# linkedin/spark-tfrecord

Hardware: AMD Instinct MI355X
Metric: rows/sec read+write (1M-row Example round-trip) (higher is better)
Workload: dtype wire(int64/float32/bytes); 1 GPU; model=Example{id:int64, ints:Int64List[8], floats:FloatList[16], tokens:BytesList[2]}, global_batch=1000000, parallelism=dp1, rows_per_rank=1000000, engine=gpu, storage=/dev/shm, crc_verify=True

## Files before the change

csrc/codec_core.h:

```cpp
#pragma once

#include <cstdint>
#include <cstring>

#include "crc32c.h"

namespace tfrec {

using i64 = int64_t;
using u64 = uint64_t;
using u32 = uint32_t;
using u8 = uint8_t;

enum Kind : int32_t { KIND_BYTES = 1, KIND_FLOAT = 2, KIND_INT64 = 3 };

enum RecordFormat : int32_t { FMT_EXAMPLE = 0, FMT_SEQUENCE = 1, FMT_BYTE_ARRAY = 2 };

enum CodecErr : int32_t {
  ERR_OK = 0,
  ERR_TRUNCATED = -1,
  ERR_BAD_VARINT = -2,
  ERR_KIND_MISMATCH = -3,
  ERR_BAD_WIRETYPE = -4,
  ERR_OVERFLOW = -5,
  ERR_NAME_TOO_LONG = -6,
};


TFR_HOSTDEV inline int popcount64(u64 x) { return __builtin_popcountll(x); }

TFR_HOSTDEV inline int ctz64(u64 x) { return __builtin_ctzll(x); }

constexpr u64 kMsbMask = 0x8080808080808080ull;

TFR_HOSTDEV inline const u8* read_varint(const u8* p, const u8* end, u64* out) {
  if (end - p >= 8) {
    u64 w;
    __builtin_memcpy(&w, p, 8);
    u64 stops = ~w & kMsbMask;
    if (stops) {
      int nb = (ctz64(stops) >> 3) + 1;
      u64 v = 0;
      for (int i = 0; i < nb; ++i)
        v |= ((w >> (8 * i)) & 0x7F) << (7 * i);
      *out = v;
      return p + nb;
    }
    u64 v = 0;
    for (int i = 0; i < 8; ++i) v |= ((w >> (8 * i)) & 0x7F) << (7 * i);
    const u8* q = p + 8;
    for (int shift = 56; q < end && shift < 64; shift += 7) {
      u8 b = *q++;
      v |= static_cast<u64>(b & 0x7F) << shift;
      if (!(b & 0x80)) {
        *out = v;
        return q;
      }
    }
    return nullptr;
  }
  u64 v = 0;
  int shift = 0;
  while (p < end) {
    u8 b = *p++;
    v |= static_cast<u64>(b & 0x7F) << shift;
    if (!(b & 0x80)) {
      *out = v;
      return p;
    }
    shift += 7;
    if (shift >= 64) return nullptr;
  }
  return nullptr;
}

TFR_HOSTDEV inline int varint_size(u64 v) {
  int n = 1;
  while (v >= 0x80) {
    v >>= 7;
    ++n;
  }
  return n;
}

TFR_HOSTDEV inline u8* write_varint(u8* p, u64 v) {
  while (v >= 0x80) {
    *p++ = static_cast<u8>(v) | 0x80;
    v >>= 7;
  }
  *p++ = static_cast<u8>(v);
  return p;
}


struct FieldDescRaw {
  int32_t kind;
  int32_t is_seq;
  int32_t name_off;
  int32_t name_len;
};

struct SchemaView {
  int32_t nfields;
  const FieldDescRaw* fields;
  const u8* names;

  TFR_HOSTDEV const u8* name(int f) const { return names + fields[f].name_off; }
  TFR_HOSTDEV int name_len(int f) const { return fields[f].name_len; }
};

TFR_HOSTDEV inline SchemaView schema_view(const u8* blob) {
  SchemaView v;
  int32_t n;
  __builtin_memcpy(&n, blob, 4);
  v.nfields = n;
  v.fields = reinterpret_cast<const FieldDescRaw*>(blob + 4);
  v.names = blob + 4 + n * static_cast<int>(sizeof(FieldDescRaw));
  return v;
}

TFR_HOSTDEV inline bool name_eq(const u8* a, const u8* b, int n) {
  while (n >= 8) {
    u64 x, y;
    __builtin_memcpy(&x, a, 8);
    __builtin_memcpy(&y, b, 8);
    if (x != y) return false;
    a += 8;
    b += 8;
    n -= 8;
  }
  for (int i = 0; i < n; ++i)
    if (a[i] != b[i]) return false;
  return true;
}

TFR_HOSTDEV inline int schema_find(const SchemaView& s, const u8* name, int len,
                                   int want_seq) {
  for (int f = 0; f < s.nfields; ++f) {
    if (s.fields[f].is_seq == want_seq && s.fields[f].name_len == len &&
        name_eq(s.name(f), name, len))
      return f;
  }
  return -1;
}


struct FieldStat {
  i64 pos;
  i64 len;
  i64 nvals;
  i64 nbytes;
  i64 nlists;
  int32_t kind_found;
  int32_t err;
};

TFR_HOSTDEV inline void field_stat_clear(FieldStat* st) {
  st->pos = -1;
  st->len = 0;
  st->nvals = 0;
  st->nbytes = 0;
  st->nlists = 0;
  st->kind_found = 0;
  st->err = 0;
}

TFR_HOSTDEV inline const u8* skip_field(const u8* p, const u8* end, u32 wiretype) {
  u64 tmp;
  switch (wiretype) {
    case 0:
      return read_varint(p, end, &tmp);
    case 1:
      return (end - p >= 8) ? p + 8 : nullptr;
    case 2:
      p = read_varint(p, end, &tmp);
      if (!p || static_cast<u64>(end - p) < tmp) return nullptr;
      return p + tmp;
    case 5:
      return (end - p >= 4) ? p + 4 : nullptr;
    default:
      return nullptr;
  }
}

TFR_HOSTDEV inline int32_t count_list_body(const u8* p, const u8* end, int32_t kind,
                                           i64* nvals, i64* nbytes) {
  while (p < end) {
    u64 tag;
    p = read_varint(p, end, &tag);
    if (!p) return ERR_BAD_VARINT;
    u32 fieldno = static_cast<u32>(tag >> 3);
    u32 wt = static_cast<u32>(tag & 7);
    if (fieldno != 1) {
      p = skip_field(p, end, wt);
      if (!p) return ERR_TRUNCATED;
      continue;
    }
    if (kind == KIND_BYTES) {
      if (wt != 2) return ERR_BAD_WIRETYPE;
      u64 len;
      p = read_varint(p, end, &len);
      if (!p || static_cast<u64>(end - p) < len) return ERR_TRUNCATED;
      *nvals += 1;
      *nbytes += static_cast<i64>(len);
      p += len;
    } else if (kind == KIND_FLOAT) {
      if (wt == 2) {
        u64 len;
        p = read_varint(p, end, &len);
        if (!p || static_cast<u64>(end - p) < len) return ERR_TRUNCATED;
        *nvals += static_cast<i64>(len / 4);
        p += len;
      } else if (wt == 5) {
        if (end - p < 4) return ERR_TRUNCATED;
        *nvals += 1;
        p += 4;
      } else {
        return ERR_BAD_WIRETYPE;
      }
    } else {
      if (wt == 2) {
        u64 len;
        p = read_varint(p, end, &len);
        if (!p || static_cast<u64>(end - p) < len) return ERR_TRUNCATED;
        const u8* q = p;
        const u8* qe = p + len;
        if (len && (qe[-1] & 0x80)) return ERR_BAD_VARINT;
        i64 cnt = 0;
        while (qe - q >= 8) {
          u64 w;
          __builtin_memcpy(&w, q, 8);
          cnt += popcount64(~w & kMsbMask);
          q += 8;
        }
        for (; q < qe; ++q) cnt += !(*q & 0x80);
        *nvals += cnt;
        p = qe;
      } else if (wt == 0) {
        u64 v;
        p = read_varint(p, end, &v);
        if (!p) return ERR_BAD_VARINT;
        *nvals += 1;
      } else {
        return ERR_BAD_WIRETYPE;
      }
    }
  }
  return ERR_OK;
}

TFR_HOSTDEV inline int32_t scan_feature_body(const u8* p, const u8* end,
                                             int32_t expect_kind, int32_t* kind_found,
                                             i64* nvals, i64* nbytes) {
  while (p < end) {
    u64 tag;
    p = read_varint(p, end, &tag);
    if (!p) return ERR_BAD_VARINT;
    u32 fieldno = static_cast<u32>(tag >> 3);
    u32 wt = static_cast<u32>(tag & 7);
    if (fieldno >= 1 && fieldno <= 3 && wt == 2) {
      u64 len;
      p = read_varint(p, end, &len);
      if (!p || static_cast<u64>(end - p) < len) return ERR_TRUNCATED;
      *kind_found = static_cast<int32_t>(fieldno);
      if (expect_kind >= 0 && static_cast<int32_t>(fieldno) != expect_kind)
        return ERR_KIND_MISMATCH;
      int32_t rc = count_list_body(p, p + len, static_cast<int32_t>(fieldno), nvals,
                                   nbytes);
      if (rc != ERR_OK) return rc;
      p += len;
    } else {
      p = skip_field(p, end, wt);
      if (!p) return ERR_TRUNCATED;
    }
  }
  return ERR_OK;
}

TFR_HOSTDEV inline int32_t scan_features_body(const u8* p, const u8* end, i64 base,
                                              const SchemaView& schema, int want_seq,
                                              FieldStat* stats) {
  const u8* body_start = p;
  while (p < end) {
    u64 tag;
    p = read_varint(p, end, &tag);
    if (!p) return ERR_BAD_VARINT;
    u32 fieldno = static_cast<u32>(tag >> 3);
    u32 wt = static_cast<u32>(tag & 7);
    if (fieldno != 1 || wt != 2) {
      p = skip_field(p, end, wt);
      if (!p) return ERR_TRUNCATED;
      continue;
    }
    u64 entry_len;
    p = read_varint(p, end, &entry_len);
    if (!p || static_cast<u64>(end - p) < entry_len) return ERR_TRUNCATED;
    const u8* ep = p;
    const u8* ee = p + entry_len;
    p = ee;
    const u8* key = nullptr;
    u64 key_len = 0;
    const u8* val = nullptr;
    u64 val_len = 0;
    while (ep < ee) {
      u64 etag;
      ep = read_varint(ep, ee, &etag);
      if (!ep) return ERR_BAD_VARINT;
      u32 efn = static_cast<u32>(etag >> 3);
      u32 ewt = static_cast<u32>(etag & 7);
      if (efn == 1 && ewt == 2) {
        ep = read_varint(ep, ee, &key_len);
        if (!ep || static_cast<u64>(ee - ep) < key_len) return ERR_TRUNCATED;
        key = ep;
        ep += key_len;
      } else if (efn == 2 && ewt == 2) {
        ep = read_varint(ep, ee, &val_len);
        if (!ep || static_cast<u64>(ee - ep) < val_len) return ERR_TRUNCATED;
        val = ep;
        ep += val_len;
      } else {
        ep = skip_field(ep, ee, ewt);
        if (!ep) return ERR_TRUNCATED;
      }
    }
    if (!key) continue;
    int f = schema_find(schema, key, static_cast<int>(key_len), want_seq);
    if (f < 0) continue;
    FieldStat* st = &stats[f];
    st->nvals = 0;
    st->nbytes = 0;
    st->nlists = 0;
    st->kind_found = 0;
    st->err = 0;
    st->pos = base + (val ? (val - body_start) : 0);
    st->len = static_cast<i64>(val_len);
    if (!want_seq) {
      int32_t rc = scan_feature_body(val, val + val_len, schema.fields[f].kind,
                                     &st->kind_found, &st->nvals, &st->nbytes);
      if (rc != ERR_OK) st->err = rc;
    } else {
      const u8* lp = val;
      const u8* le = val + val_len;
      while (lp < le) {
        u64 ltag;
        lp = read_varint(lp, le, &ltag);
        if (!lp) {
          st->err = ERR_BAD_VARINT;
          break;
        }
        u32 lfn = static_cast<u32>(ltag >> 3);
        u32 lwt = static_cast<u32>(ltag & 7);
        if (lfn == 1 && lwt == 2) {
          u64 flen;
          lp = read_varint(lp, le, &flen);
          if (!lp || static_cast<u64>(le - lp) < flen) {
            st->err = ERR_TRUNCATED;
            break;
          }
          st->nlists += 1;
          int32_t kf = 0;
          int32_t rc = scan_feature_body(lp, lp + flen, schema.fields[f].kind, &kf,
                                         &st->nvals, &st->nbytes);
          if (rc != ERR_OK) {
            st->err = rc;
            break;
          }
          if (kf) st->kind_found = kf;
          lp += flen;
        } else {
          lp = skip_field(lp, le, lwt);
          if (!lp) {
            st->err = ERR_TRUNCATED;
            break;
          }
        }
      }
    }
  }
  return ERR_OK;
}

TFR_HOSTDEV inline int32_t scan_record(const u8* data, i64 abs_off, i64 rec_len,
                                       int32_t fmt, const SchemaView& schema,
                                       FieldStat* stats) {
  const u8* p = data + abs_off;
  const u8* end = p + rec_len;
  while (p < end) {
    u64 tag;
    p = read_varint(p, end, &tag);
    if (!p) return ERR_BAD_VARINT;
    u32 fieldno = static_cast<u32>(tag >> 3);
    u32 wt = static_cast<u32>(tag & 7);
    bool is_features =
        (fmt == FMT_EXAMPLE && fieldno == 1) || (fmt == FMT_SEQUENCE && fieldno == 1);
    bool is_feature_lists = (fmt == FMT_SEQUENCE && fieldno == 2);
    if ((is_features || is_feature_lists) && wt == 2) {
      u64 len;
      p = read_varint(p, end, &len);
      if (!p || static_cast<u64>(end - p) < len) return ERR_TRUNCATED;
      i64 base = (p - data);
      if (is_features) {
        int32_t rc = scan_features_body(p, p + len, base, schema, 0, stats);
        if (rc != ERR_OK) return rc;
      } else {
        int32_t rc = scan_features_body(p, p + len, base, schema, 1, stats);
        if (rc != ERR_OK) return rc;
      }
      p += len;
    } else {
      p = skip_field(p, end, wt);
      if (!p) return ERR_TRUNCATED;
    }
  }
  return ERR_OK;
}


constexpr int32_t ERR_RETRY_UNFUSED = -100;

TFR_HOSTDEV inline u32 crc32c_step8(u32 crc, u64 w, const uint32_t (*tab)[256]) {
  w ^= crc;
  return tab[7][w & 0xFF] ^ tab[6][(w >> 8) & 0xFF] ^ tab[5][(w >> 16) & 0xFF] ^
         tab[4][(w >> 24) & 0xFF] ^ tab[3][(w >> 32) & 0xFF] ^
         tab[2][(w >> 40) & 0xFF] ^ tab[1][(w >> 48) & 0xFF] ^
         tab[0][(w >> 56) & 0xFF];
}

struct ScanCur {
  const u8* base;
  i64 len;
  i64 pos;
  i64 wpos;
  u64 w0, w1;
  u32 crc;
  const uint32_t (*tab)[256];
};

TFR_HOSTDEV inline u64 cur_load(const ScanCur& c, i64 at) {
  if (at + 8 <= c.len) {
    u64 w;
    __builtin_memcpy(&w, c.base + at, 8);
    return w;
  }
  u64 w = 0;
  for (i64 b = at; b < c.len; ++b) w |= (u64)c.base[b] << (8 * (b - at));
  return w;
}

TFR_HOSTDEV inline void cur_init(ScanCur& c, const u8* base, i64 len,
                                 const uint32_t (*tab)[256]) {
  c.base = base;
  c.len = len;
  c.pos = 0;
  c.wpos = 0;
  c.tab = tab;
  c.crc = 0xFFFFFFFFu;
  c.w0 = cur_load(c, 0);
  c.w1 = cur_load(c, 8);
}

TFR_HOSTDEV inline u64 cur_peek(const ScanCur& c) {
  int sh = (int)(c.pos - c.wpos) * 8;
  if (sh == 0) return c.w0;
  if (sh == 64) return c.w1;
  return (c.w0 >> sh) | (c.w1 << (64 - sh));
}

TFR_HOSTDEV inline void cur_advance(ScanCur& c, i64 k) {
  c.pos += k;
  while (c.pos > c.wpos + 8) {
    if (c.wpos + 8 <= c.len) c.crc = crc32c_step8(c.crc, c.w0, c.tab);
    c.w0 = c.w1;
    c.wpos += 8;
    c.w1 = cur_load(c, c.wpos + 8);
  }
}

TFR_HOSTDEV inline u32 cur_finish_crc(ScanCur& c) {
  while (c.wpos + 8 <= c.len) {
    c.crc = crc32c_step8(c.crc, c.w0, c.tab);
    c.w0 = c.w1;
    c.wpos += 8;
    c.w1 = cur_load(c, c.wpos + 8);
  }
  u32 crc = c.crc;
  for (i64 b = c.wpos; b < c.len; ++b)
    crc = c.tab[0][(crc ^ c.base[b]) & 0xFF] ^ (crc >> 8);
  return ~crc;
}

TFR_HOSTDEV inline bool cur_varint(ScanCur& c, i64 end, u64* out) {
  i64 avail = end - c.pos;
  if (avail <= 0) return false;
  u64 w = cur_peek(c);
  u64 stops = ~w & kMsbMask;
  if (stops) {
    int nb = (ctz64(stops) >> 3) + 1;
    if (nb > avail) return false;
    u64 v = 0;
    for (int i = 0; i < nb; ++i) v |= ((w >> (8 * i)) & 0x7F) << (7 * i);
    *out = v;
    cur_advance(c, nb);
    return true;
  }
  if (avail < 9) return false;
  u64 v = 0;
  for (int i = 0; i < 8; ++i) v |= ((w >> (8 * i)) & 0x7F) << (7 * i);
  cur_advance(c, 8);
  for (int shift = 56; shift < 64 && c.pos < end; shift += 7) {
    u8 b = (u8)cur_peek(c);
    v |= (u64)(b & 0x7F) << shift;
    cur_advance(c, 1);
    if (!(b & 0x80)) {
      *out = v;
      return true;
    }
  }
  return false;
}

TFR_HOSTDEV inline int32_t cur_skip_field(ScanCur& c, i64 end, u32 wt) {
  u64 tmp;
  switch (wt) {
    case 0:
      return cur_varint(c, end, &tmp) ? ERR_OK : ERR_BAD_VARINT;
    case 1:
      if (end - c.pos < 8) return ERR_TRUNCATED;
      cur_advance(c, 8);
      return ERR_OK;
    case 2:
      if (!cur_varint(c, end, &tmp)) return ERR_BAD_VARINT;
      if ((u64)(end - c.pos) < tmp) return ERR_TRUNCATED;
      cur_advance(c, (i64)tmp);
      return ERR_OK;
    case 5:
      if (end - c.pos < 4) return ERR_TRUNCATED;
      cur_advance(c, 4);
      return ERR_OK;
    default:
      return ERR_BAD_WIRETYPE;
  }
}

TFR_HOSTDEV inline i64 cur_count_terms(ScanCur& c, i64 n) {
  i64 cnt = 0;
  while (n >= 8) {
    cnt += popcount64(~cur_peek(c) & kMsbMask);
    cur_advance(c, 8);
    n -= 8;
  }
  if (n > 0) {
    u64 mask = kMsbMask >> (8 * (8 - n));
    cnt += popcount64(~cur_peek(c) & mask);
    cur_advance(c, n);
  }
  return cnt;
}

TFR_HOSTDEV inline int32_t cur_count_list_body(ScanCur& c, i64 end, int32_t kind,
                                               i64* nvals, i64* nbytes) {
  while (c.pos < end) {
    u64 tag;
    if (!cur_varint(c, end, &tag)) return ERR_BAD_VARINT;
    u32 fieldno = (u32)(tag >> 3), wt = (u32)(tag & 7);
    if (fieldno != 1) {
      int32_t rc = cur_skip_field(c, end, wt);
      if (rc != ERR_OK) return rc;
      continue;
    }
    if (kind == KIND_BYTES) {
      if (wt != 2) return ERR_BAD_WIRETYPE;
      u64 blen;
      if (!cur_varint(c, end, &blen)) return ERR_BAD_VARINT;
      if ((u64)(end - c.pos) < blen) return ERR_TRUNCATED;
      *nvals += 1;
      *nbytes += (i64)blen;
      cur_advance(c, (i64)blen);
    } else if (kind == KIND_FLOAT) {
      if (wt == 2) {
        u64 blen;
        if (!cur_varint(c, end, &blen)) return ERR_BAD_VARINT;
        if ((u64)(end - c.pos) < blen) return ERR_TRUNCATED;
        *nvals += (i64)(blen / 4);
        cur_advance(c, (i64)blen);
      } else if (wt == 5) {
        if (end - c.pos < 4) return ERR_TRUNCATED;
        *nvals += 1;
        cur_advance(c, 4);
      } else {
        return ERR_BAD_WIRETYPE;
      }
    } else {
      if (wt == 2) {
        u64 blen;
        if (!cur_varint(c, end, &blen)) return ERR_BAD_VARINT;
        if ((u64)(end - c.pos) < blen) return ERR_TRUNCATED;
        if (blen && (c.base[c.pos + (i64)blen - 1] & 0x80))
          return ERR_BAD_VARINT;
        *nvals += cur_count_terms(c, (i64)blen);
      } else if (wt == 0) {
        u64 v;
        if (!cur_varint(c, end, &v)) return ERR_BAD_VARINT;
        *nvals += 1;
      } else {
        return ERR_BAD_WIRETYPE;
      }
    }
  }
  return ERR_OK;
}

TFR_HOSTDEV inline int32_t cur_scan_feature_body(ScanCur& c, i64 end,
                                                 int32_t expect_kind,
                                                 int32_t* kind_found, i64* nvals,
                                                 i64* nbytes) {
  while (c.pos < end) {
    u64 tag;
    if (!cur_varint(c, end, &tag)) return ERR_BAD_VARINT;
    u32 fieldno = (u32)(tag >> 3), wt = (u32)(tag & 7);
    if (fieldno >= 1 && fieldno <= 3 && wt == 2) {
      u64 blen;
      if (!cur_varint(c, end, &blen)) return ERR_BAD_VARINT;
      if ((u64)(end - c.pos) < blen) return ERR_TRUNCATED;
      *kind_found = (int32_t)fieldno;
      if (expect_kind >= 0 && (int32_t)fieldno != expect_kind)
        return ERR_KIND_MISMATCH;
      int32_t rc = cur_count_list_body(c, c.pos + (i64)blen, (int32_t)fieldno,
                                       nvals, nbytes);
      if (rc != ERR_OK) return rc;
    } else {
      int32_t rc = cur_skip_field(c, end, wt);
      if (rc != ERR_OK) return rc;
    }
  }
  return ERR_OK;
}

TFR_HOSTDEV inline int32_t cur_scan_features_body(ScanCur& c, i64 end, i64 data_rel,
                                                  const SchemaView& schema,
                                                  int want_seq, FieldStat* stats) {
  i64 body_start = c.pos;
  while (c.pos < end) {
    u64 tag;
    if (!cur_varint(c, end, &tag)) return ERR_BAD_VARINT;
    u32 fieldno = (u32)(tag >> 3), wt = (u32)(tag & 7);
    if (fieldno != 1 || wt != 2) {
      int32_t rc = cur_skip_field(c, end, wt);
      if (rc != ERR_OK) return rc;
      continue;
    }
    u64 entry_len;
    if (!cur_varint(c, end, &entry_len)) return ERR_BAD_VARINT;
    if ((u64)(end - c.pos) < entry_len) return ERR_TRUNCATED;
    i64 ee = c.pos + (i64)entry_len;
    int f = -1;
    bool key_seen = false;
    bool val_seen = false;
    while (c.pos < ee) {
      u64 etag;
      if (!cur_varint(c, ee, &etag)) return ERR_BAD_VARINT;
      u32 efn = (u32)(etag >> 3), ewt = (u32)(etag & 7);
      if (efn == 1 && ewt == 2) {
        if (val_seen) return ERR_RETRY_UNFUSED;
        u64 klen;
        if (!cur_varint(c, ee, &klen)) return ERR_BAD_VARINT;
        if ((u64)(ee - c.pos) < klen) return ERR_TRUNCATED;
        f = schema_find(schema, c.base + c.pos, (int)klen, want_seq);
        key_seen = true;
        cur_advance(c, (i64)klen);
      } else if (efn == 2 && ewt == 2) {
        if (!key_seen) return ERR_RETRY_UNFUSED;
        val_seen = true;
        u64 vlen;
        if (!cur_varint(c, ee, &vlen)) return ERR_BAD_VARINT;
        if ((u64)(ee - c.pos) < vlen) return ERR_TRUNCATED;
        i64 ve = c.pos + (i64)vlen;
        if (f < 0) {
          cur_advance(c, (i64)vlen);
          continue;
        }
        FieldStat* st = &stats[f];
        st->nvals = 0;
        st->nbytes = 0;
        st->nlists = 0;
        st->kind_found = 0;
        st->err = 0;
        st->pos = data_rel + c.pos;
        st->len = (i64)vlen;
        if (!want_seq) {
          int32_t rc = cur_scan_feature_body(c, ve, schema.fields[f].kind,
                                             &st->kind_found, &st->nvals,
                                             &st->nbytes);
          if (rc == ERR_RETRY_UNFUSED) return rc;
          if (rc != ERR_OK) st->err = rc;
        } else {
          while (c.pos < ve && st->err == ERR_OK) {
            u64 ltag;
            if (!cur_varint(c, ve, &ltag)) {
              st->err = ERR_BAD_VARINT;
              break;
            }
            u32 lfn = (u32)(ltag >> 3), lwt = (u32)(ltag & 7);
            if (lfn == 1 && lwt == 2) {
              u64 flen;
              if (!cur_varint(c, ve, &flen) || (u64)(ve - c.pos) < flen) {
                st->err = ERR_TRUNCATED;
                break;
              }
              st->nlists += 1;
              int32_t kf = 0;
              int32_t rc = cur_scan_feature_body(c, c.pos + (i64)flen,
                                                 schema.fields[f].kind, &kf,
                                                 &st->nvals, &st->nbytes);
              if (rc == ERR_RETRY_UNFUSED) return rc;
              if (rc != ERR_OK) {
                st->err = rc;
                break;
              }
              if (kf) st->kind_found = kf;
            } else {
              int32_t rc = cur_skip_field(c, ve, lwt);
              if (rc != ERR_OK) {
                st->err = ERR_TRUNCATED;
                break;
              }
            }
          }
        }
        if (c.pos < ve) cur_advance(c, ve - c.pos);
      } else {
        int32_t rc = cur_skip_field(c, ee, ewt);
        if (rc != ERR_OK) return rc;
      }
    }
    if (f >= 0 && !val_seen) {
      FieldStat* st = &stats[f];
      st->pos = data_rel + body_start;
      st->len = 0;
      st->nvals = 0;
      st->nbytes = 0;
      st->nlists = 0;
      st->kind_found = 0;
      st->err = 0;
    }
  }
  return ERR_OK;
}

TFR_HOSTDEV inline int32_t scan_record_fused(const u8* data, i64 abs_off,
                                             i64 rec_len, int32_t fmt,
                                             const SchemaView& schema,
                                             FieldStat* stats, u32* crc_out,
                                             const uint32_t (*tab)[256]) {
  ScanCur c;
  cur_init(c, data + abs_off, rec_len, tab);
  while (c.pos < rec_len) {
    u64 tag;
    if (!cur_varint(c, rec_len, &tag)) return ERR_BAD_VARINT;
    u32 fieldno = (u32)(tag >> 3), wt = (u32)(tag & 7);
    bool is_features = fieldno == 1;
    bool is_fl = (fmt == FMT_SEQUENCE && fieldno == 2);
    if ((is_features || is_fl) && wt == 2) {
      u64 blen;
      if (!cur_varint(c, rec_len, &blen)) return ERR_BAD_VARINT;
      if ((u64)(rec_len - c.pos) < blen) return ERR_TRUNCATED;
      int32_t rc = cur_scan_features_body(c, c.pos + (i64)blen, abs_off, schema,
                                          is_fl ? 1 : 0, stats);
      if (rc != ERR_OK) return rc;
    } else {
      int32_t rc = cur_skip_field(c, rec_len, wt);
      if (rc != ERR_OK) return rc;
    }
  }
  *crc_out = cur_finish_crc(c);
  return ERR_OK;
}


struct DecodeDst {
  i64* i64_vals;
  float* f32_vals;
  u8* bytes_data;
  i64* elem_len;
  i64* sub_count;
};

TFR_HOSTDEV inline int32_t extract_list_body(const u8* p, const u8* end, int32_t kind,
                                             const DecodeDst& dst, i64* vi, i64* bi) {
  while (p < end) {
    u64 tag;
    p = read_varint(p, end, &tag);
    if (!p) return ERR_BAD_VARINT;
    u32 fieldno = static_cast<u32>(tag >> 3);
    u32 wt = static_cast<u32>(tag & 7);
    if (fieldno != 1) {
      p = skip_field(p, end, wt);
      if (!p) return ERR_TRUNCATED;
      continue;
    }
    if (kind == KIND_BYTES) {
      u64 len;
      p = read_varint(p, end, &len);
      if (!p || static_cast<u64>(end - p) < len) return ERR_TRUNCATED;
      u8* d = dst.bytes_data + *bi;
      u64 i = 0;
      for (; i + 8 <= len; i += 8) {
        u64 w;
        __builtin_memcpy(&w, p + i, 8);
        __builtin_memcpy(d + i, &w, 8);
      }
      for (; i < len; ++i) d[i] = p[i];
      dst.elem_len[*vi] = static_cast<i64>(len);
      *bi += static_cast<i64>(len);
      *vi += 1;
      p += len;
    } else if (kind == KIND_FLOAT) {
      if (wt == 2) {
        u64 len;
        p = read_varint(p, end, &len);
        if (!p || static_cast<u64>(end - p) < len) return ERR_TRUNCATED;
        u64 n = len / 4;
        __builtin_memcpy(dst.f32_vals + *vi, p, n * 4);
        *vi += static_cast<i64>(n);
        p += len;
      } else {
        if (end - p < 4) return ERR_TRUNCATED;
        float v;
        __builtin_memcpy(&v, p, 4);
        dst.f32_vals[(*vi)++] = v;
        p += 4;
      }
    } else {
      if (wt == 2) {
        u64 len;
        p = read_varint(p, end, &len);
        if (!p || static_cast<u64>(end - p) < len) return ERR_TRUNCATED;
        const u8* q = p;
        const u8* qe = p + len;
        while (q < qe) {
          u64 v;
          q = read_varint(q, qe, &v);
          if (!q) return ERR_BAD_VARINT;
          dst.i64_vals[(*vi)++] = static_cast<i64>(v);
        }
        p = qe;
      } else {
        u64 v;
        p = read_varint(p, end, &v);
        if (!p) return ERR_BAD_VARINT;
        dst.i64_vals[(*vi)++] = static_cast<i64>(v);
      }
    }
  }
  return ERR_OK;
}

TFR_HOSTDEV inline int32_t extract_feature_body(const u8* p, const u8* end,
                                                int32_t kind, const DecodeDst& dst,
                                                i64* vi, i64* bi) {
  while (p < end) {
    u64 tag;
    p = read_varint(p, end, &tag);
    if (!p) return ERR_BAD_VARINT;
    u32 fieldno = static_cast<u32>(tag >> 3);
    u32 wt = static_cast<u32>(tag & 7);
    if (fieldno >= 1 && fieldno <= 3 && wt == 2) {
      u64 len;
      p = read_varint(p, end, &len);
      if (!p || static_cast<u64>(end - p) < len) return ERR_TRUNCATED;
      int32_t rc = extract_list_body(p, p + len, kind, dst, vi, bi);
      if (rc != ERR_OK) return rc;
      p += len;
    } else {
      p = skip_field(p, end, wt);
      if (!p) return ERR_TRUNCATED;
    }
  }
  return ERR_OK;
}

TFR_HOSTDEV inline int32_t extract_field(const u8* data, i64 pos, i64 len,
                                         int32_t kind, int32_t is_seq,
                                         const DecodeDst& dst, i64 val_base,
                                         i64 byte_base, i64 list_base) {
  if (pos < 0) return ERR_OK;
  const u8* p = data + pos;
  const u8* end = p + len;
  i64 vi = val_base;
  i64 bi = byte_base;
  if (!is_seq) return extract_feature_body(p, end, kind, dst, &vi, &bi);
  i64 li = list_base;
  while (p < end) {
    u64 tag;
    p = read_varint(p, end, &tag);
    if (!p) return ERR_BAD_VARINT;
    u32 fieldno = static_cast<u32>(tag >> 3);
    u32 wt = static_cast<u32>(tag & 7);
    if (fieldno == 1 && wt == 2) {
      u64 flen;
      p = read_varint(p, end, &flen);
      if (!p || static_cast<u64>(end - p) < flen) return ERR_TRUNCATED;
      i64 v_before = vi;
      int32_t rc = extract_feature_body(p, p + flen, kind, dst, &vi, &bi);
      if (rc != ERR_OK) return rc;
      dst.sub_count[li++] = vi - v_before;
      p += flen;
    } else {
      p = skip_field(p, end, wt);
      if (!p) return ERR_TRUNCATED;
    }
  }
  return ERR_OK;
}


struct FieldColumn {
  int32_t kind;
  int32_t is_seq;
  const u8* presence;
  const i64* row_off;
  const i64* list_off;
  const i64* sub_off;
  const i64* elem_off;
  const u8* bytes_data;
  const i64* i64_vals;
  const float* f32_vals;
};

TFR_HOSTDEV inline i64 list_body_size(const FieldColumn& c, i64 v0, i64 v1) {
  if (c.kind == KIND_FLOAT) {
    i64 n = v1 - v0;
    return n ? (1 + varint_size(static_cast<u64>(4 * n)) + 4 * n) : 0;
  }
  if (c.kind == KIND_INT64) {
    i64 packed = 0;
    for (i64 v = v0; v < v1; ++v)
      packed += varint_size(static_cast<u64>(c.i64_vals[v]));
    return packed ? (1 + varint_size(static_cast<u64>(packed)) + packed) : 0;
  }
  i64 sz = 0;
  for (i64 v = v0; v < v1; ++v) {
    i64 blen = c.elem_off[v + 1] - c.elem_off[v];
    sz += 1 + varint_size(static_cast<u64>(blen)) + blen;
  }
  return sz;
}

TFR_HOSTDEV inline i64 feature_body_size(const FieldColumn& c, i64 v0, i64 v1) {
  i64 body = list_body_size(c, v0, v1);
  return 1 + varint_size(static_cast<u64>(body)) + body;
}

TFR_HOSTDEV inline u8* emit_list_body(u8* o, const FieldColumn& c, i64 v0, i64 v1) {
  if (c.kind == KIND_FLOAT) {
    i64 n = v1 - v0;
    if (n) {
      *o++ = 0x0A;
      o = write_varint(o, static_cast<u64>(4 * n));
      __builtin_memcpy(o, c.f32_vals + v0, static_cast<size_t>(4 * n));
      o += 4 * n;
    }
  } else if (c.kind == KIND_INT64) {
    i64 packed = 0;
    for (i64 v = v0; v < v1; ++v)
      packed += varint_size(static_cast<u64>(c.i64_vals[v]));
    if (packed) {
      *o++ = 0x0A;
      o = write_varint(o, static_cast<u64>(packed));
      for (i64 v = v0; v < v1; ++v)
        o = write_varint(o, static_cast<u64>(c.i64_vals[v]));
    }
  } else {
    for (i64 v = v0; v < v1; ++v) {
      i64 b0 = c.elem_off[v];
      i64 blen = c.elem_off[v + 1] - b0;
      *o++ = 0x0A;
      o = write_varint(o, static_cast<u64>(blen));
      for (i64 i = 0; i < blen; ++i) o[i] = c.bytes_data[b0 + i];
      o += blen;
    }
  }
  return o;
}

TFR_HOSTDEV inline u8* emit_feature_body(u8* o, const FieldColumn& c, i64 v0, i64 v1) {
  i64 body = list_body_size(c, v0, v1);
  *o++ = static_cast<u8>((c.kind << 3) | 2);
  o = write_varint(o, static_cast<u64>(body));
  return emit_list_body(o, c, v0, v1);
}

TFR_HOSTDEV inline i64 features_entry_size(const FieldColumn& c, const SchemaView& s,
                                           int f, i64 v0, i64 v1) {
  i64 fb = feature_body_size(c, v0, v1);
  i64 klen = s.name_len(f);
  return (1 + varint_size(static_cast<u64>(klen)) + klen) +
         (1 + varint_size(static_cast<u64>(fb)) + fb);
}

TFR_HOSTDEV inline u8* emit_features_entry(u8* o, const FieldColumn& c,
                                           const SchemaView& s, int f, i64 v0, i64 v1) {
  i64 fb = feature_body_size(c, v0, v1);
  i64 klen = s.name_len(f);
  *o++ = 0x0A;
  o = write_varint(o, static_cast<u64>(klen));
  const u8* nm = s.name(f);
  for (i64 i = 0; i < klen; ++i) o[i] = nm[i];
  o += klen;
  *o++ = 0x12;
  o = write_varint(o, static_cast<u64>(fb));
  return emit_feature_body(o, c, v0, v1);
}

TFR_HOSTDEV inline i64 feature_list_body_size(const FieldColumn& c, i64 r) {
  i64 sz = 0;
  for (i64 j = c.list_off[r]; j < c.list_off[r + 1]; ++j) {
    i64 fb = feature_body_size(c, c.sub_off[j], c.sub_off[j + 1]);
    sz += 1 + varint_size(static_cast<u64>(fb)) + fb;
  }
  return sz;
}

TFR_HOSTDEV inline u8* emit_feature_list_body(u8* o, const FieldColumn& c, i64 r) {
  for (i64 j = c.list_off[r]; j < c.list_off[r + 1]; ++j) {
    i64 fb = feature_body_size(c, c.sub_off[j], c.sub_off[j + 1]);
    *o++ = 0x0A;
    o = write_varint(o, static_cast<u64>(fb));
    o = emit_feature_body(o, c, c.sub_off[j], c.sub_off[j + 1]);
  }
  return o;
}

TFR_HOSTDEV inline i64 feature_lists_entry_size(const FieldColumn& c,
                                                const SchemaView& s, int f, i64 r) {
  i64 flb = feature_list_body_size(c, r);
  i64 klen = s.name_len(f);
  return (1 + varint_size(static_cast<u64>(klen)) + klen) +
         (1 + varint_size(static_cast<u64>(flb)) + flb);
}

TFR_HOSTDEV inline u8* emit_feature_lists_entry(u8* o, const FieldColumn& c,
                                                const SchemaView& s, int f, i64 r) {
  i64 flb = feature_list_body_size(c, r);
  i64 klen = s.name_len(f);
  *o++ = 0x0A;
  o = write_varint(o, static_cast<u64>(klen));
  const u8* nm = s.name(f);
  for (i64 i = 0; i < klen; ++i) o[i] = nm[i];
  o += klen;
  *o++ = 0x12;
  o = write_varint(o, static_cast<u64>(flb));
  return emit_feature_list_body(o, c, r);
}

TFR_HOSTDEV inline i64 record_payload_size(const FieldColumn* cols,
                                           const SchemaView& s, int32_t fmt, i64 r) {
  i64 ctx_body = 0;
  i64 fl_body = 0;
  for (int f = 0; f < s.nfields; ++f) {
    const FieldColumn& c = cols[f];
    if (!c.presence[r]) continue;
    if (!c.is_seq) {
      i64 e = features_entry_size(c, s, f, c.row_off[r], c.row_off[r + 1]);
      ctx_body += 1 + varint_size(static_cast<u64>(e)) + e;
    } else {
      i64 e = feature_lists_entry_size(c, s, f, r);
      fl_body += 1 + varint_size(static_cast<u64>(e)) + e;
    }
  }
  i64 total = 0;
  if (fmt == FMT_EXAMPLE) {
    total += 1 + varint_size(static_cast<u64>(ctx_body)) + ctx_body;
  } else {
    if (ctx_body) total += 1 + varint_size(static_cast<u64>(ctx_body)) + ctx_body;
    total += 1 + varint_size(static_cast<u64>(fl_body)) + fl_body;
  }
  return total;
}

TFR_HOSTDEV inline u8* emit_record_payload(u8* o, const FieldColumn* cols,
                                           const SchemaView& s, int32_t fmt, i64 r) {
  i64 ctx_body = 0, fl_body = 0;
  for (int f = 0; f < s.nfields; ++f) {
    const FieldColumn& c = cols[f];
    if (!c.presence[r]) continue;
    if (!c.is_seq) {
      i64 e = features_entry_size(c, s, f, c.row_off[r], c.row_off[r + 1]);
      ctx_body += 1 + varint_size(static_cast<u64>(e)) + e;
    } else {
      i64 e = feature_lists_entry_size(c, s, f, r);
      fl_body += 1 + varint_size(static_cast<u64>(e)) + e;
    }
  }
  auto emit_ctx = [&](u8* oo) {
    for (int f = 0; f < s.nfields; ++f) {
      const FieldColumn& c = cols[f];
      if (!c.presence[r] || c.is_seq) continue;
      i64 e = features_entry_size(c, s, f, c.row_off[r], c.row_off[r + 1]);
      *oo++ = 0x0A;
      oo = write_varint(oo, static_cast<u64>(e));
      oo = emit_features_entry(oo, c, s, f, c.row_off[r], c.row_off[r + 1]);
    }
    return oo;
  };
  auto emit_fl = [&](u8* oo) {
    for (int f = 0; f < s.nfields; ++f) {
      const FieldColumn& c = cols[f];
      if (!c.presence[r] || !c.is_seq) continue;
      i64 e = feature_lists_entry_size(c, s, f, r);
      *oo++ = 0x0A;
      oo = write_varint(oo, static_cast<u64>(e));
      oo = emit_feature_lists_entry(oo, c, s, f, r);
    }
    return oo;
  };
  if (fmt == FMT_EXAMPLE) {
    *o++ = 0x0A;
    o = write_varint(o, static_cast<u64>(ctx_body));
    o = emit_ctx(o);
  } else {
    if (ctx_body) {
      *o++ = 0x0A;
      o = write_varint(o, static_cast<u64>(ctx_body));
      o = emit_ctx(o);
    }
    *o++ = 0x12;
    o = write_varint(o, static_cast<u64>(fl_body));
    o = emit_fl(o);
  }
  return o;
}



struct WriteCur {
  u8* base;
  i64 pos;
  i64 wpos;
  u64 win;
  u32 crc;
  const uint32_t (*tab)[256];
};

TFR_HOSTDEV inline void wcur_init(WriteCur& w, u8* base,
                                  const uint32_t (*tab)[256]) {
  w.base = base;
  w.pos = 0;
  w.wpos = 0;
  w.win = 0;
  w.crc = 0xFFFFFFFFu;
  w.tab = tab;
}

TFR_HOSTDEV inline void wcur_flush8(WriteCur& w) {
  __builtin_memcpy(w.base + w.wpos, &w.win, 8);
  w.crc = crc32c_step8(w.crc, w.win, w.tab);
  w.wpos += 8;
  w.win = 0;
}

TFR_HOSTDEV inline void wcur_put(WriteCur& w, u8 b) {
  w.win |= (u64)b << (8 * (w.pos - w.wpos));
  if (++w.pos - w.wpos == 8) wcur_flush8(w);
}

TFR_HOSTDEV inline void wcur_varint(WriteCur& w, u64 v) {
  while (v >= 0x80) {
    wcur_put(w, (u8)(v | 0x80));
    v >>= 7;
  }
  wcur_put(w, (u8)v);
}

TFR_HOSTDEV inline void wcur_bytes(WriteCur& w, const u8* src, i64 n) {
  while (n > 0 && (w.pos - w.wpos) != 0) {
    wcur_put(w, *src++);
    --n;
  }
  while (n >= 8) {
    __builtin_memcpy(&w.win, src, 8);
    w.pos += 8;
    wcur_flush8(w);
    src += 8;
    n -= 8;
  }
  while (n-- > 0) wcur_put(w, *src++);
}

TFR_HOSTDEV inline u32 wcur_finish(WriteCur& w) {
  int rem = (int)(w.pos - w.wpos);
  if (!rem) return ~w.crc;
  __builtin_memcpy(w.base + w.wpos, &w.win, (size_t)rem);
  u32 crc = w.crc;
  for (int i = 0; i < rem; ++i)
    crc = w.tab[0][(crc ^ (u8)(w.win >> (8 * i))) & 0xFF] ^ (crc >> 8);
  return ~crc;
}

TFR_HOSTDEV inline void wcur_list_body(WriteCur& w, const FieldColumn& c,
                                       i64 v0, i64 v1) {
  if (c.kind == KIND_FLOAT) {
    i64 n = v1 - v0;
    if (n) {
      wcur_put(w, 0x0A);
      wcur_varint(w, (u64)(4 * n));
      wcur_bytes(w, (const u8*)(c.f32_vals + v0), 4 * n);
    }
  } else if (c.kind == KIND_INT64) {
    i64 packed = 0;
    for (i64 v = v0; v < v1; ++v)
      packed += varint_size((u64)c.i64_vals[v]);
    if (packed) {
      wcur_put(w, 0x0A);
      wcur_varint(w, (u64)packed);
      for (i64 v = v0; v < v1; ++v) wcur_varint(w, (u64)c.i64_vals[v]);
    }
  } else {
    for (i64 v = v0; v < v1; ++v) {
      i64 b0 = c.elem_off[v];
      i64 blen = c.elem_off[v + 1] - b0;
      wcur_put(w, 0x0A);
      wcur_varint(w, (u64)blen);
      wcur_bytes(w, c.bytes_data + b0, blen);
    }
  }
}

TFR_HOSTDEV inline void wcur_feature_body(WriteCur& w, const FieldColumn& c,
                                          i64 v0, i64 v1) {
  i64 body = list_body_size(c, v0, v1);
  wcur_put(w, (u8)((c.kind << 3) | 2));
  wcur_varint(w, (u64)body);
  wcur_list_body(w, c, v0, v1);
}

TFR_HOSTDEV inline void wcur_features_entry(WriteCur& w, const FieldColumn& c,
                                            const SchemaView& s, int f, i64 v0,
                                            i64 v1) {
  i64 fb = feature_body_size(c, v0, v1);
  i64 klen = s.name_len(f);
  wcur_put(w, 0x0A);
  wcur_varint(w, (u64)klen);
  wcur_bytes(w, s.name(f), klen);
  wcur_put(w, 0x12);
  wcur_varint(w, (u64)fb);
  wcur_feature_body(w, c, v0, v1);
}

TFR_HOSTDEV inline void wcur_feature_list_body(WriteCur& w,
                                               const FieldColumn& c, i64 r) {
  for (i64 j = c.list_off[r]; j < c.list_off[r + 1]; ++j) {
    i64 fb = feature_body_size(c, c.sub_off[j], c.sub_off[j + 1]);
    wcur_put(w, 0x0A);
    wcur_varint(w, (u64)fb);
    wcur_feature_body(w, c, c.sub_off[j], c.sub_off[j + 1]);
  }
}

TFR_HOSTDEV inline void wcur_feature_lists_entry(WriteCur& w,
                                                 const FieldColumn& c,
                                                 const SchemaView& s, int f,
                                                 i64 r) {
  i64 flb = feature_list_body_size(c, r);
  i64 klen = s.name_len(f);
  wcur_put(w, 0x0A);
  wcur_varint(w, (u64)klen);
  wcur_bytes(w, s.name(f), klen);
  wcur_put(w, 0x12);
  wcur_varint(w, (u64)flb);
  wcur_feature_list_body(w, c, r);
}

TFR_HOSTDEV inline i64 emit_record_payload_fused(u8* o, const FieldColumn* cols,
                                                 const SchemaView& s, int32_t fmt,
                                                 i64 r, u32* crc_out,
                                                 const uint32_t (*tab)[256]) {
  i64 ctx_body = 0, fl_body = 0;
  for (int f = 0; f < s.nfields; ++f) {
    const FieldColumn& c = cols[f];
    if (!c.presence[r]) continue;
    if (!c.is_seq) {
      i64 e = features_entry_size(c, s, f, c.row_off[r], c.row_off[r + 1]);
      ctx_body += 1 + varint_size((u64)e) + e;
    } else {
      i64 e = feature_lists_entry_size(c, s, f, r);
      fl_body += 1 + varint_size((u64)e) + e;
    }
  }
  WriteCur w;
  wcur_init(w, o, tab);
  auto emit_ctx = [&]() {
    for (int f = 0; f < s.nfields; ++f) {
      const FieldColumn& c = cols[f];
      if (!c.presence[r] || c.is_seq) continue;
      i64 e = features_entry_size(c, s, f, c.row_off[r], c.row_off[r + 1]);
      wcur_put(w, 0x0A);
      wcur_varint(w, (u64)e);
      wcur_features_entry(w, c, s, f, c.row_off[r], c.row_off[r + 1]);
    }
  };
  auto emit_fl = [&]() {
    for (int f = 0; f < s.nfields; ++f) {
      const FieldColumn& c = cols[f];
      if (!c.presence[r] || !c.is_seq) continue;
      i64 e = feature_lists_entry_size(c, s, f, r);
      wcur_put(w, 0x0A);
      wcur_varint(w, (u64)e);
      wcur_feature_lists_entry(w, c, s, f, r);
    }
  };
  if (fmt == FMT_EXAMPLE) {
    wcur_put(w, 0x0A);
    wcur_varint(w, (u64)ctx_body);
    emit_ctx();
  } else {
    if (ctx_body) {
      wcur_put(w, 0x0A);
      wcur_varint(w, (u64)ctx_body);
      emit_ctx();
    }
    wcur_put(w, 0x12);
    wcur_varint(w, (u64)fl_body);
    emit_fl();
  }
  *crc_out = wcur_finish(w);
  return w.pos;
}

constexpr i64 kFrameOverhead = 16;

TFR_HOSTDEV inline void write_frame_header_footer(u8* file, i64 frame_off,
                                                  i64 payload_len,
                                                  const u32 (*tab)[256]) {
  u8* h = file + frame_off;
  u64 len_le = static_cast<u64>(payload_len);
  __builtin_memcpy(h, &len_le, 8);
  u32 lc = mask_crc(crc32c_sw(h, 8, 0, tab));
  __builtin_memcpy(h + 8, &lc, 4);
  u32 dc = mask_crc(crc32c_sw(h + 12, static_cast<size_t>(payload_len), 0, tab));
  __builtin_memcpy(h + 12 + payload_len, &dc, 4);
}

TFR_HOSTDEV inline void write_frame_header_footer_crc(u8* file, i64 frame_off,
                                                      i64 payload_len,
                                                      u32 payload_crc,
                                                      const u32 (*tab)[256]) {
  u8* h = file + frame_off;
  u64 len_le = static_cast<u64>(payload_len);
  __builtin_memcpy(h, &len_le, 8);
  u32 lc = mask_crc(crc32c_sw(h, 8, 0, tab));
  __builtin_memcpy(h + 8, &lc, 4);
  u32 dc = mask_crc(payload_crc);
  __builtin_memcpy(h + 12 + payload_len, &dc, 4);
}

}
```

csrc/hip/kernels.hip:

```cpp

#include <hip/hip_runtime.h>
#include <pybind11/pybind11.h>
#include <pybind11/stl.h>
#include <rocprim/rocprim.hpp>

#include <fcntl.h>
#include <sys/mman.h>
#include <sys/stat.h>
#include <unistd.h>

#include <cstdint>
#include <map>
#include <mutex>
#include <stdexcept>
#include <string>
#include <vector>

#include "../codec_core.h"

namespace py = pybind11;
using namespace tfrec;

#define HIP_CHECK(expr)                                                          \
  do {                                                                           \
    hipError_t _e = (expr);                                                      \
    if (_e != hipSuccess)                                                        \
      throw std::runtime_error(std::string("HIP error: ") +                      \
                               hipGetErrorString(_e) + " at " __FILE__ ":" +     \
                               std::to_string(__LINE__));                        \
  } while (0)

namespace {

constexpr int kBlock = 256;

__device__ inline void stage_crc_tables(uint32_t (*lds)[256]) {
  const uint32_t* src = &kCrcTables.t[0][0];
  uint32_t* dst = &lds[0][0];
  for (int i = threadIdx.x; i < 8 * 256; i += blockDim.x) dst[i] = src[i];
  __syncthreads();
}

__device__ inline void set_err(int32_t* err, int32_t code, i64 r) {
  err[0] = code;
  i64 v = r + 1;
  atomicMax(&err[1], v > 0x7FFFFFFF ? (int32_t)0x7FFFFFFF : (int32_t)v);
}


__global__ void crc_verify_kernel(const u8* __restrict__ data,
                                  const i64* __restrict__ off,
                                  const i64* __restrict__ len, i64 R,
                                  unsigned long long* err_out) {
  __shared__ uint32_t tab[8][256];
  stage_crc_tables(tab);
  for (i64 r = blockIdx.x * (i64)blockDim.x + threadIdx.x; r < R;
       r += (i64)gridDim.x * blockDim.x) {
    const u8* h = data + off[r] - 12;
    u32 len_crc, data_crc;
    __builtin_memcpy(&len_crc, h + 8, 4);
    __builtin_memcpy(&data_crc, h + 12 + len[r], 4);
    bool ok = mask_crc(crc32c_sw(h, 8, 0, tab)) == len_crc &&
              mask_crc(crc32c_sw(h + 12, (size_t)len[r], 0, tab)) == data_crc;
    if (!ok) atomicMin(err_out, (unsigned long long)(r + 1));
  }
}


static_assert(sizeof(FieldStat) == 48, "FieldStat layout shared with Python");

__global__ void scan_records_kernel(const u8* __restrict__ data,
                                    const i64* __restrict__ off,
                                    const i64* __restrict__ len, i64 R, int32_t fmt,
                                    const u8* __restrict__ schema_blob, int F,
                                    FieldStat* __restrict__ stats,
                                    int32_t* __restrict__ err,
                                    unsigned long long* crc_err,
                                    i64 rec_base) {
  __shared__ uint32_t tab[8][256];
  if (crc_err) stage_crc_tables(tab);
  SchemaView schema = schema_view(schema_blob);
  for (i64 r = blockIdx.x * (i64)blockDim.x + threadIdx.x; r < R;
       r += (i64)gridDim.x * blockDim.x) {
    FieldStat* st = stats + r * F;
    for (int f = 0; f < F; ++f) field_stat_clear(&st[f]);
    int32_t rc;
    if (crc_err) {
      u32 payload_crc = 0;
      rc = scan_record_fused(data, off[r], len[r], fmt, schema, st,
                             &payload_crc, tab);
      if (rc == ERR_RETRY_UNFUSED) {
        for (int f = 0; f < F; ++f) field_stat_clear(&st[f]);
        rc = scan_record(data, off[r], len[r], fmt, schema, st);
        payload_crc = crc32c_sw(data + off[r], (size_t)len[r], 0, tab);
      }
      if (rc != ERR_OK)
        payload_crc = crc32c_sw(data + off[r], (size_t)len[r], 0, tab);
      const u8* h = data + off[r] - 12;
      u32 len_crc, data_crc;
      __builtin_memcpy(&len_crc, h + 8, 4);
      __builtin_memcpy(&data_crc, h + 12 + len[r], 4);
      bool ok = mask_crc(crc32c_sw(h, 8, 0, tab)) == len_crc &&
                mask_crc(payload_crc) == data_crc;
      if (!ok) atomicMin(crc_err, (unsigned long long)(rec_base + r + 1));
    } else {
      rc = scan_record(data, off[r], len[r], fmt, schema, st);
    }
    if (rc != ERR_OK) set_err(err, rc, rec_base + r);
    for (int f = 0; f < F; ++f)
      if (st[f].err != ERR_OK) set_err(err, st[f].err, rec_base + r);
  }
}


struct DevFieldDst {
  int32_t kind;
  int32_t is_seq;
  i64* i64_vals;
  float* f32_vals;
  u8* bytes_data;
  i64* elem_len;
  i64* sub_count;
  const i64* val_base;
  const i64* byte_base;
  const i64* list_base;
};

__global__ void extract_fields_kernel(const u8* __restrict__ data, i64 R, int F,
                                      const FieldStat* __restrict__ stats,
                                      const DevFieldDst* __restrict__ metas,
                                      int32_t* __restrict__ err, i64 r0) {
  i64 total = R * F;
  for (i64 idx = blockIdx.x * (i64)blockDim.x + threadIdx.x; idx < total;
       idx += (i64)gridDim.x * blockDim.x) {
    i64 q = idx / F;
    int f = (int)(idx - q * F);
    i64 r = r0 + q;
    const DevFieldDst& m = metas[f];
    const FieldStat& st = stats[r * F + f];
    DecodeDst dst{m.i64_vals, m.f32_vals, m.bytes_data, m.elem_len, m.sub_count};
    int32_t rc = extract_field(data, st.pos, st.len, m.kind, m.is_seq, dst,
                               m.val_base ? m.val_base[r] : 0,
                               m.byte_base ? m.byte_base[r] : 0,
                               m.list_base ? m.list_base[r] : 0);
    if (rc != ERR_OK) set_err(err, rc, r);
  }
}



__global__ void size_records_kernel(const FieldColumn* __restrict__ cols,
                                    const u8* __restrict__ schema_blob, int32_t fmt,
                                    i64 R, i64* __restrict__ psize) {
  SchemaView schema = schema_view(schema_blob);
  for (i64 r = blockIdx.x * (i64)blockDim.x + threadIdx.x; r < R;
       r += (i64)gridDim.x * blockDim.x) {
    psize[r] = record_payload_size(cols, schema, fmt, r) + kFrameOverhead;
  }
}

__global__ void emit_records_kernel(const FieldColumn* __restrict__ cols,
                                    const u8* __restrict__ schema_blob, int32_t fmt,
                                    i64 r0, i64 R, const i64* __restrict__ frame_off,
                                    u8* __restrict__ file,
                                    int32_t* __restrict__ err) {
  __shared__ uint32_t tab[8][256];
  stage_crc_tables(tab);
  SchemaView schema = schema_view(schema_blob);
  for (i64 r = r0 + blockIdx.x * (i64)blockDim.x + threadIdx.x; r < R;
       r += (i64)gridDim.x * blockDim.x) {
    i64 payload = (frame_off[r + 1] - frame_off[r]) - kFrameOverhead;
    u8* o = file + frame_off[r] + 12;
    u32 crc = 0;
    i64 emitted = emit_record_payload_fused(o, cols, schema, fmt, r, &crc,
                                            tab);
    if (emitted != payload) set_err(err, ERR_OVERFLOW, r);
    write_frame_header_footer_crc(file, frame_off[r], payload, crc, tab);
  }
}


constexpr i64 kWaveRecordBytes = 8 << 10;

__device__ inline u32 crc32c_wave(const u8* p, i64 n,
                                  const uint32_t (*tab)[256]) {
  int lane = threadIdx.x & 63;
  i64 chunk = (n + 63) / 64;
  if (chunk < 64) chunk = 64;
  i64 s = (i64)lane * chunk;
  i64 e = s + chunk < n ? s + chunk : n;
  u32 my = (s < e) ? crc32c_sw(p + s, (size_t)(e - s), 0, tab) : 0;
  u32 acc = __shfl(my, 0);
  if (chunk < n) {
    u32 op = crc32c_shift_elem((u64)chunk);
    for (int i = 1; i < 64; ++i) {
      i64 si = (i64)i * chunk;
      if (si >= n) break;
      u32 ci = __shfl(my, i);
      i64 li = (si + chunk < n ? chunk : n - si);
      acc = (li == chunk) ? (crc_gfmul(acc, op) ^ ci)
                          : crc32c_combine_fast(acc, ci, (u64)li);
    }
  }
  return acc;
}

__device__ inline void copy_wave(u8* d, const u8* s, i64 n) {
  int lane = threadIdx.x & 63;
  i64 i = (i64)lane * 8;
  for (; i + 8 <= n; i += 64 * 8) {
    u64 w;
    __builtin_memcpy(&w, s + i, 8);
    __builtin_memcpy(d + i, &w, 8);
  }
  i64 tail = n & ~((i64)7);
  for (i64 b = tail + lane; b < n; b += 64) d[b] = s[b];
}

__global__ void crc_verify_wave_kernel(const u8* __restrict__ data,
                                       const i64* __restrict__ off,
                                       const i64* __restrict__ len, i64 R,
                                       unsigned long long* err_out) {
  __shared__ uint32_t tab[8][256];
  stage_crc_tables(tab);
  i64 wave = (blockIdx.x * (i64)blockDim.x + threadIdx.x) / 64;
  i64 nwaves = ((i64)gridDim.x * blockDim.x) / 64;
  for (i64 r = wave; r < R; r += nwaves) {
    const u8* h = data + off[r] - 12;
    u32 payload = crc32c_wave(h + 12, len[r], tab);
    if ((threadIdx.x & 63) == 0) {
      u32 len_crc, data_crc;
      __builtin_memcpy(&len_crc, h + 8, 4);
      __builtin_memcpy(&data_crc, h + 12 + len[r], 4);
      bool ok = mask_crc(crc32c_sw(h, 8, 0, tab)) == len_crc &&
                mask_crc(payload) == data_crc;
      if (!ok) atomicMin(err_out, (unsigned long long)(r + 1));
    }
  }
}

__global__ void frame_bytes_wave_kernel(const u8* __restrict__ src,
                                        const i64* __restrict__ elem_off,
                                        const i64* __restrict__ frame_off, i64 R,
                                        u8* __restrict__ file) {
  __shared__ uint32_t tab[8][256];
  stage_crc_tables(tab);
  i64 wave = (blockIdx.x * (i64)blockDim.x + threadIdx.x) / 64;
  i64 nwaves = ((i64)gridDim.x * blockDim.x) / 64;
  for (i64 r = wave; r < R; r += nwaves) {
    i64 n = elem_off[r + 1] - elem_off[r];
    const u8* s = src + elem_off[r];
    u8* d = file + frame_off[r] + 12;
    copy_wave(d, s, n);
    u32 crc = crc32c_wave(s, n, tab);
    if ((threadIdx.x & 63) == 0)
      write_frame_header_footer_crc(file, frame_off[r], n, crc, tab);
  }
}

__global__ void gather_payloads_wave_kernel(const u8* __restrict__ data,
                                            const i64* __restrict__ off,
                                            const i64* __restrict__ len,
                                            const i64* __restrict__ dst_off,
                                            i64 R, u8* __restrict__ out) {
  i64 wave = (blockIdx.x * (i64)blockDim.x + threadIdx.x) / 64;
  i64 nwaves = ((i64)gridDim.x * blockDim.x) / 64;
  for (i64 r = wave; r < R; r += nwaves)
    copy_wave(out + dst_off[r], data + off[r], len[r]);
}


__device__ inline i64 wave_incl_scan(i64 v) {
  int lane = threadIdx.x & 63;
  for (int d = 1; d < 64; d <<= 1) {
    i64 y = __shfl_up(v, d);
    if (lane >= d) v += y;
  }
  return v;
}

__device__ inline i64 wave_extract_i64_packed(const u8* __restrict__ p, i64 n,
                                              i64* __restrict__ out, i64 base) {
  int lane = threadIdx.x & 63;
  i64 chunk = (n + 63) / 64;
  i64 lo = (i64)lane * chunk;
  i64 hi = lo + chunk < n ? lo + chunk : n;
  i64 cnt = 0;
  for (i64 i = lo; i < hi; ++i) cnt += !(p[i] & 0x80);
  i64 incl = wave_incl_scan(cnt);
  i64 excl = incl - cnt;
  i64 total = __shfl(incl, 63);
  i64 q = lo;
  i64 pre = 0;
  if (lo > 0 && lo < hi) {
    if (p[lo - 1] & 0x80) {
      while (q < hi && (p[q] & 0x80)) ++q;
      if (q < hi) {
        ++q;
        pre = 1;
      }
    }
  }
  i64 idx = base + excl + pre;
  while (q < hi) {
    u64 v = 0;
    int shift = 0;
    i64 j = q;
    while (j < n && shift < 70) {
      u8 b = p[j++];
      v |= (u64)(b & 0x7F) << shift;
      shift += 7;
      if (!(b & 0x80)) break;
    }
    out[idx++] = (i64)v;
    q = j;
  }
  return total;
}

__device__ inline int32_t extract_list_body_wave(const u8* __restrict__ p,
                                                 const u8* end, int32_t kind,
                                                 const DecodeDst& dst, i64* vi,
                                                 i64* bi) {
  int lane = threadIdx.x & 63;
  while (p < end) {
    u64 tag;
    p = read_varint(p, end, &tag);
    if (!p) return ERR_BAD_VARINT;
    u32 fieldno = (u32)(tag >> 3), wt = (u32)(tag & 7);
    if (fieldno != 1) {
      p = skip_field(p, end, wt);
      if (!p) return ERR_TRUNCATED;
      continue;
    }
    if (kind == KIND_BYTES) {
      u64 len;
      p = read_varint(p, end, &len);
      if (!p || (u64)(end - p) < len) return ERR_TRUNCATED;
      copy_wave(dst.bytes_data + *bi, p, (i64)len);
      if (lane == 0) dst.elem_len[*vi] = (i64)len;
      *bi += (i64)len;
      *vi += 1;
      p += len;
    } else if (kind == KIND_FLOAT) {
      if (wt == 2) {
        u64 len;
        p = read_varint(p, end, &len);
        if (!p || (u64)(end - p) < len) return ERR_TRUNCATED;
        u64 nv = len / 4;
        copy_wave((u8*)(dst.f32_vals + *vi), p, (i64)(nv * 4));
        *vi += (i64)nv;
        p += len;
      } else {
        if (end - p < 4) return ERR_TRUNCATED;
        if (lane == 0) {
          float v;
          __builtin_memcpy(&v, p, 4);
          dst.f32_vals[*vi] = v;
        }
        (*vi)++;
        p += 4;
      }
    } else {
      if (wt == 2) {
        u64 len;
        p = read_varint(p, end, &len);
        if (!p || (u64)(end - p) < len) return ERR_TRUNCATED;
        *vi += wave_extract_i64_packed(p, (i64)len, dst.i64_vals, *vi);
        p += len;
      } else {
        u64 v;
        p = read_varint(p, end, &v);
        if (!p) return ERR_BAD_VARINT;
        if (lane == 0) dst.i64_vals[*vi] = (i64)v;
        (*vi)++;
      }
    }
  }
  return ERR_OK;
}

__device__ inline int32_t extract_feature_body_wave(const u8* __restrict__ p,
                                                    const u8* end, int32_t kind,
                                                    const DecodeDst& dst,
                                                    i64* vi, i64* bi) {
  while (p < end) {
    u64 tag;
    p = read_varint(p, end, &tag);
    if (!p) return ERR_BAD_VARINT;
    u32 fieldno = (u32)(tag >> 3), wt = (u32)(tag & 7);
    if (fieldno >= 1 && fieldno <= 3 && wt == 2) {
      u64 len;
      p = read_varint(p, end, &len);
      if (!p || (u64)(end - p) < len) return ERR_TRUNCATED;
      int32_t rc = extract_list_body_wave(p, p + len, kind, dst, vi, bi);
      if (rc != ERR_OK) return rc;
      p += len;
    } else {
      p = skip_field(p, end, wt);
      if (!p) return ERR_TRUNCATED;
    }
  }
  return ERR_OK;
}

__device__ inline int32_t extract_field_wave(const u8* __restrict__ data,
                                             i64 pos, i64 len, int32_t kind,
                                             int32_t is_seq, const DecodeDst& dst,
                                             i64 val_base, i64 byte_base,
                                             i64 list_base) {
  if (pos < 0) return ERR_OK;
  int lane = threadIdx.x & 63;
  const u8* p = data + pos;
  const u8* end = p + len;
  i64 vi = val_base;
  i64 bi = byte_base;
  if (!is_seq) return extract_feature_body_wave(p, end, kind, dst, &vi, &bi);
  i64 li = list_base;
  while (p < end) {
    u64 tag;
    p = read_varint(p, end, &tag);
    if (!p) return ERR_BAD_VARINT;
    u32 fieldno = (u32)(tag >> 3), wt = (u32)(tag & 7);
    if (fieldno == 1 && wt == 2) {
      u64 flen;
      p = read_varint(p, end, &flen);
      if (!p || (u64)(end - p) < flen) return ERR_TRUNCATED;
      i64 v_before = vi;
      int32_t rc = extract_feature_body_wave(p, p + flen, kind, dst, &vi, &bi);
      if (rc != ERR_OK) return rc;
      if (lane == 0) dst.sub_count[li] = vi - v_before;
      ++li;
      p += flen;
    } else {
      p = skip_field(p, end, wt);
      if (!p) return ERR_TRUNCATED;
    }
  }
  return ERR_OK;
}

__global__ void scan_records_wave_kernel(const u8* __restrict__ data,
                                         const i64* __restrict__ off,
                                         const i64* __restrict__ len, i64 R,
                                         int32_t fmt,
                                         const u8* __restrict__ schema_blob,
                                         int F, FieldStat* __restrict__ stats,
                                         int32_t* __restrict__ err,
                                         unsigned long long* crc_err,
                                         i64 rec_base) {
  __shared__ uint32_t tab[8][256];
  stage_crc_tables(tab);
  SchemaView schema = schema_view(schema_blob);
  i64 wave = (blockIdx.x * (i64)blockDim.x + threadIdx.x) / 64;
  i64 nwaves = ((i64)gridDim.x * blockDim.x) / 64;
  int lane = threadIdx.x & 63;
  for (i64 r = wave; r < R; r += nwaves) {
    if (lane == 0) {
      FieldStat* st = stats + r * F;
      for (int f = 0; f < F; ++f) field_stat_clear(&st[f]);
      int32_t rc = scan_record(data, off[r], len[r], fmt, schema, st);
      if (rc != ERR_OK) set_err(err, rc, rec_base + r);
      for (int f = 0; f < F; ++f)
        if (st[f].err != ERR_OK) set_err(err, st[f].err, rec_base + r);
    }
    if (crc_err) {
      const u8* h = data + off[r] - 12;
      u32 payload = crc32c_wave(h + 12, len[r], tab);
      if (lane == 0) {
        u32 len_crc, data_crc;
        __builtin_memcpy(&len_crc, h + 8, 4);
        __builtin_memcpy(&data_crc, h + 12 + len[r], 4);
        bool ok = mask_crc(crc32c_sw(h, 8, 0, tab)) == len_crc &&
                  mask_crc(payload) == data_crc;
        if (!ok) atomicMin(crc_err, (unsigned long long)(rec_base + r + 1));
      }
    }
  }
}

__global__ void extract_fields_wave_kernel(const u8* __restrict__ data, i64 R,
                                           int F,
                                           const FieldStat* __restrict__ stats,
                                           const DevFieldDst* __restrict__ metas,
                                           int32_t* __restrict__ err, i64 r0) {
  i64 total = R * F;
  i64 wave = (blockIdx.x * (i64)blockDim.x + threadIdx.x) / 64;
  i64 nwaves = ((i64)gridDim.x * blockDim.x) / 64;
  for (i64 idx = wave; idx < total; idx += nwaves) {
    i64 q = idx / F;
    int f = (int)(idx - q * F);
    i64 r = r0 + q;
    const DevFieldDst& m = metas[f];
    const FieldStat& st = stats[r * F + f];
    DecodeDst dst{m.i64_vals, m.f32_vals, m.bytes_data, m.elem_len, m.sub_count};
    int32_t rc = extract_field_wave(data, st.pos, st.len, m.kind, m.is_seq, dst,
                                    m.val_base ? m.val_base[r] : 0,
                                    m.byte_base ? m.byte_base[r] : 0,
                                    m.list_base ? m.list_base[r] : 0);
    if (rc != ERR_OK && (threadIdx.x & 63) == 0) set_err(err, rc, r);
  }
}


__device__ inline i64 wave_emit_i64_packed(u8* __restrict__ o,
                                           const i64* __restrict__ vals,
                                           i64 v0, i64 v1) {
  int lane = threadIdx.x & 63;
  i64 n = v1 - v0;
  i64 chunk = (n + 63) / 64;
  i64 lo = v0 + (i64)lane * chunk;
  i64 hi = lo + chunk < v1 ? lo + chunk : v1;
  i64 sz = 0;
  for (i64 v = lo; v < hi; ++v) sz += varint_size((u64)vals[v]);
  i64 incl = wave_incl_scan(sz);
  u8* q = o + (incl - sz);
  for (i64 v = lo; v < hi; ++v) q = write_varint(q, (u64)vals[v]);
  return __shfl(incl, 63);
}

struct WaveCur {
  u8* base;
  i64 pos;
};

__device__ inline void wvc_put(WaveCur& w, u8 b) {
  if ((threadIdx.x & 63) == 0) w.base[w.pos] = b;
  w.pos += 1;
}

__device__ inline void wvc_varint(WaveCur& w, u64 v) {
  if ((threadIdx.x & 63) == 0) write_varint(w.base + w.pos, v);
  w.pos += varint_size(v);
}

__device__ inline void wvc_bytes(WaveCur& w, const u8* s, i64 n) {
  copy_wave(w.base + w.pos, s, n);
  w.pos += n;
}

__device__ inline void wvc_list_body(WaveCur& w, const FieldColumn& c, i64 v0,
                                     i64 v1) {
  if (c.kind == KIND_FLOAT) {
    i64 n = v1 - v0;
    if (n) {
      wvc_put(w, 0x0A);
      wvc_varint(w, (u64)(4 * n));
      wvc_bytes(w, (const u8*)(c.f32_vals + v0), 4 * n);
    }
  } else if (c.kind == KIND_INT64) {
    i64 packed = 0;
    for (i64 v = v0; v < v1; ++v) packed += varint_size((u64)c.i64_vals[v]);
    if (packed) {
      wvc_put(w, 0x0A);
      wvc_varint(w, (u64)packed);
      w.pos += wave_emit_i64_packed(w.base + w.pos, c.i64_vals, v0, v1);
    }
  } else {
    for (i64 v = v0; v < v1; ++v) {
      i64 b0 = c.elem_off[v];
      i64 blen = c.elem_off[v + 1] - b0;
      wvc_put(w, 0x0A);
      wvc_varint(w, (u64)blen);
      wvc_bytes(w, c.bytes_data + b0, blen);
    }
  }
}

__device__ inline void wvc_feature_body(WaveCur& w, const FieldColumn& c,
                                        i64 v0, i64 v1) {
  i64 body = list_body_size(c, v0, v1);
  wvc_put(w, (u8)((c.kind << 3) | 2));
  wvc_varint(w, (u64)body);
  wvc_list_body(w, c, v0, v1);
}

__device__ inline void wvc_features_entry(WaveCur& w, const FieldColumn& c,
                                          const SchemaView& s, int f, i64 v0,
                                          i64 v1) {
  i64 fb = feature_body_size(c, v0, v1);
  i64 klen = s.name_len(f);
  wvc_put(w, 0x0A);
  wvc_varint(w, (u64)klen);
  wvc_bytes(w, s.name(f), klen);
  wvc_put(w, 0x12);
  wvc_varint(w, (u64)fb);
  wvc_feature_body(w, c, v0, v1);
}

__device__ inline void wvc_feature_lists_entry(WaveCur& w, const FieldColumn& c,
                                               const SchemaView& s, int f,
                                               i64 r) {
  i64 flb = feature_list_body_size(c, r);
  i64 klen = s.name_len(f);
  wvc_put(w, 0x0A);
  wvc_varint(w, (u64)klen);
  wvc_bytes(w, s.name(f), klen);
  wvc_put(w, 0x12);
  wvc_varint(w, (u64)flb);
  for (i64 j = c.list_off[r]; j < c.list_off[r + 1]; ++j) {
    i64 fb = feature_body_size(c, c.sub_off[j], c.sub_off[j + 1]);
    wvc_put(w, 0x0A);
    wvc_varint(w, (u64)fb);
    wvc_feature_body(w, c, c.sub_off[j], c.sub_off[j + 1]);
  }
}

__device__ inline i64 emit_record_payload_wave(u8* o, const FieldColumn* cols,
                                               const SchemaView& s, int32_t fmt,
                                               i64 r) {
  i64 ctx_body = 0, fl_body = 0;
  for (int f = 0; f < s.nfields; ++f) {
    const FieldColumn& c = cols[f];
    if (!c.presence[r]) continue;
    if (!c.is_seq) {
      i64 e = features_entry_size(c, s, f, c.row_off[r], c.row_off[r + 1]);
      ctx_body += 1 + varint_size((u64)e) + e;
    } else {
      i64 e = feature_lists_entry_size(c, s, f, r);
      fl_body += 1 + varint_size((u64)e) + e;
    }
  }
  WaveCur w{o, 0};
  auto emit_ctx = [&]() {
    for (int f = 0; f < s.nfields; ++f) {
      const FieldColumn& c = cols[f];
      if (!c.presence[r] || c.is_seq) continue;
      i64 e = features_entry_size(c, s, f, c.row_off[r], c.row_off[r + 1]);
      wvc_put(w, 0x0A);
      wvc_varint(w, (u64)e);
      wvc_features_entry(w, c, s, f, c.row_off[r], c.row_off[r + 1]);
    }
  };
  auto emit_fl = [&]() {
    for (int f = 0; f < s.nfields; ++f) {
      const FieldColumn& c = cols[f];
      if (!c.presence[r] || !c.is_seq) continue;
      i64 e = feature_lists_entry_size(c, s, f, r);
      wvc_put(w, 0x0A);
      wvc_varint(w, (u64)e);
      wvc_feature_lists_entry(w, c, s, f, r);
    }
  };
  if (fmt == FMT_EXAMPLE) {
    wvc_put(w, 0x0A);
    wvc_varint(w, (u64)ctx_body);
    emit_ctx();
  } else {
    if (ctx_body) {
      wvc_put(w, 0x0A);
      wvc_varint(w, (u64)ctx_body);
      emit_ctx();
    }
    wvc_put(w, 0x12);
    wvc_varint(w, (u64)fl_body);
    emit_fl();
  }
  return w.pos;
}

__global__ void emit_records_wave_kernel(const FieldColumn* __restrict__ cols,
                                         const u8* __restrict__ schema_blob,
                                         int32_t fmt, i64 r0, i64 R,
                                         const i64* __restrict__ frame_off,
                                         u8* __restrict__ file,
                                         int32_t* __restrict__ err) {
  __shared__ uint32_t tab[8][256];
  stage_crc_tables(tab);
  SchemaView schema = schema_view(schema_blob);
  i64 wave = (blockIdx.x * (i64)blockDim.x + threadIdx.x) / 64;
  i64 nwaves = ((i64)gridDim.x * blockDim.x) / 64;
  int lane = threadIdx.x & 63;
  for (i64 r = r0 + wave; r < R; r += nwaves) {
    i64 payload = (frame_off[r + 1] - frame_off[r]) - kFrameOverhead;
    u8* o = file + frame_off[r] + 12;
    i64 emitted = emit_record_payload_wave(o, cols, schema, fmt, r);
    if (emitted != payload && lane == 0) set_err(err, ERR_OVERFLOW, r);
    __threadfence_block();
    u32 crc = crc32c_wave(o, payload, tab);
    if (lane == 0)
      write_frame_header_footer_crc(file, frame_off[r], payload, crc, tab);
  }
}

__global__ void frame_bytes_kernel(const u8* __restrict__ src,
                                   const i64* __restrict__ elem_off,
                                   const i64* __restrict__ frame_off, i64 R,
                                   u8* __restrict__ file) {
  __shared__ uint32_t tab[8][256];
  stage_crc_tables(tab);
  for (i64 r = blockIdx.x * (i64)blockDim.x + threadIdx.x; r < R;
       r += (i64)gridDim.x * blockDim.x) {
    i64 n = elem_off[r + 1] - elem_off[r];
    WriteCur w;
    wcur_init(w, file + frame_off[r] + 12, tab);
    wcur_bytes(w, src + elem_off[r], n);
    u32 crc = wcur_finish(w);
    write_frame_header_footer_crc(file, frame_off[r], n, crc, tab);
  }
}

__device__ inline u32 crc8b_reg(u64 w, const uint32_t (*tab)[256]) {
  w ^= 0xFFFFFFFFull;
  u32 c = tab[7][w & 0xFF] ^ tab[6][(w >> 8) & 0xFF] ^ tab[5][(w >> 16) & 0xFF] ^
          tab[4][(w >> 24) & 0xFF] ^ tab[3][(w >> 32) & 0xFF] ^
          tab[2][(w >> 40) & 0xFF] ^ tab[1][(w >> 48) & 0xFF] ^
          tab[0][(w >> 56) & 0xFF];
  return ~c;
}

constexpr int kPosPerLane = 16;

template <typename F>
__device__ inline void eval_frame_chunk(const u8* __restrict__ data,
                                        const u64* __restrict__ wdata, i64 N,
                                        i64 c, i64 pos_start, i64 pos_end,
                                        const uint32_t (*tab)[256], F&& f) {
  i64 p0 = c * kPosPerLane;
  i64 w0 = p0 >> 3;
  u64 w[4];
  if (p0 + 32 <= N) {
#pragma unroll
    for (int j = 0; j < 4; ++j) w[j] = wdata[w0 + j];
  } else {
#pragma unroll
    for (int j = 0; j < 4; ++j) {
      u64 v = 0;
      i64 boff = (w0 + j) * 8;
      for (int b = 0; b < 8 && boff + b < N; ++b)
        v |= (u64)data[boff + b] << (8 * b);
      w[j] = v;
    }
  }
#pragma unroll
  for (int k = 0; k < kPosPerLane; ++k) {
    i64 i = p0 + k;
    if (i + 16 > N || i >= pos_end) break;
    if (i < pos_start) continue;
    constexpr int _ppl = kPosPerLane;
    static_assert(_ppl == 16, "index math below assumes 16 positions");
    const int wi = k >> 3;
    const int sh = (k & 7) * 8;
    u64 len = (sh == 0) ? w[wi] : (w[wi] >> sh) | (w[wi + 1] << (64 - sh));
    if (len > (u64)(N - i) - 16) continue;
    const int wi2 = (k + 8) >> 3;
    const int sh2 = sh;
    u64 hi = (sh2 == 0) ? w[wi2]
                        : (w[wi2] >> sh2) | (w[wi2 + 1] << (64 - sh2));
    u32 want = (u32)hi;
    if (mask_crc(crc8b_reg(len, tab)) != want) continue;
    f(i, (i64)len);
  }
}

template <bool EMIT>
__global__ void frame_scan_pass_kernel(const u8* __restrict__ data, i64 N,
                                       i64 pos_start, i64 pos_end,
                                       i64 block_base,
                                       i64* __restrict__ block_data,
                                       i64* __restrict__ cand_pos,
                                       i64* __restrict__ cand_len) {
  __shared__ uint32_t tab[8][256];
  __shared__ unsigned int cnt[256];
  stage_crc_tables(tab);
  const u64* wdata = reinterpret_cast<const u64*>(data);
  i64 c_lo = pos_start / kPosPerLane;
  i64 c_hi = (pos_end + kPosPerLane - 1) / kPosPerLane;
  i64 c = c_lo + (i64)blockIdx.x * blockDim.x + threadIdx.x;
  unsigned int my = 0;
  if (c < c_hi)
    eval_frame_chunk(data, wdata, N, c, pos_start, pos_end, tab,
                     [&](i64, i64) { ++my; });
  cnt[threadIdx.x] = my;
  __syncthreads();
  if (!EMIT) {
    for (int off = blockDim.x / 2; off; off >>= 1) {
      if ((int)threadIdx.x < off) cnt[threadIdx.x] += cnt[threadIdx.x + off];
      __syncthreads();
    }
    if (threadIdx.x == 0) block_data[block_base + blockIdx.x] = (i64)cnt[0];
    return;
  }
  for (int off = 1; off < (int)blockDim.x; off <<= 1) {
    unsigned int v = (int)threadIdx.x >= off ? cnt[threadIdx.x - off] : 0;
    __syncthreads();
    cnt[threadIdx.x] += v;
    __syncthreads();
  }
  i64 slot = block_data[block_base + blockIdx.x] + (i64)(cnt[threadIdx.x] - my);
  if (c < c_hi)
    eval_frame_chunk(data, wdata, N, c, pos_start, pos_end, tab,
                     [&](i64 i, i64 len) {
                       cand_pos[slot] = i;
                       cand_len[slot] = len;
                       ++slot;
                     });
}

__global__ void frame_chain_kernel(const i64* __restrict__ pos,
                                   const i64* __restrict__ len, i64 C,
                                   const i64* __restrict__ carry_in,
                                   i64* __restrict__ carry_out,
                                   i64* __restrict__ off,
                                   i64* __restrict__ broken) {
  for (i64 k = blockIdx.x * (i64)blockDim.x + threadIdx.x; k < C;
       k += (i64)gridDim.x * blockDim.x) {
    i64 p = pos[k];
    i64 want = k == 0 ? *carry_in : pos[k - 1] + 16 + len[k - 1];
    if (p != want) *broken = 1;
    off[k] = p + 12;
    if (k == C - 1) *carry_out = p + 16 + len[k];
  }
}


struct InferSlot {
  unsigned long long hash;
  long long nameref;
  long long code;
};
static_assert(sizeof(InferSlot) == 24, "layout shared with Python [S,3] i64");

__device__ inline u64 fnv1a64(const u8* s, u64 n) {
  u64 h = 1469598103934665603ull;
  for (u64 i = 0; i < n; ++i) h = (h ^ s[i]) * 1099511628211ull;
  return h ? h : 1ull;
}

constexpr int kLdsInfer = 64;

struct LdsInferSlot {
  unsigned long long hash;
  long long nameref;
  unsigned int code;
};

__device__ inline bool lds_infer_merge(LdsInferSlot* ltab, u64 hash,
                                       long long nameref, int code) {
  int idx = (int)(hash % (u64)kLdsInfer);
  for (int probe = 0; probe < kLdsInfer; ++probe) {
    LdsInferSlot& s = ltab[idx];
    unsigned long long seen =
        atomicCAS(&s.hash, 0ull, (unsigned long long)hash);
    if (seen == 0ull) s.nameref = nameref;
    if (seen == 0ull || seen == hash) {
      atomicMax(&s.code, (unsigned int)code);
      return true;
    }
    idx = (idx + 1) % kLdsInfer;
  }
  return false;
}

__device__ inline bool infer_slot_merge(InferSlot* table, int lo, int half,
                                        u64 hash, long long nameref, int code) {
  int idx = lo + (int)(hash % (u64)half);
  for (int probe = 0; probe < half; ++probe) {
    InferSlot& s = table[idx];
    unsigned long long seen =
        atomicCAS(&s.hash, 0ull, (unsigned long long)hash);
    if (seen == 0ull) s.nameref = nameref;
    if (seen == 0ull || seen == hash) {
      atomicMax((unsigned long long*)&s.code, (unsigned long long)code);
      return true;
    }
    idx = (idx + 1 - lo) % half + lo;
  }
  return false;
}

__device__ inline int32_t infer_features_body_dev(const u8* data, const u8* p,
                                                  const u8* end, bool seq,
                                                  LdsInferSlot* ltab,
                                                  InferSlot* table, int nslots) {
  int half = nslots / 2;
  int lo = seq ? half : 0;
  while (p < end) {
    u64 tag;
    p = read_varint(p, end, &tag);
    if (!p) return ERR_BAD_VARINT;
    u32 fieldno = (u32)(tag >> 3), wt = (u32)(tag & 7);
    if (fieldno != 1 || wt != 2) {
      p = skip_field(p, end, wt);
      if (!p) return ERR_TRUNCATED;
      continue;
    }
    u64 entry_len;
    p = read_varint(p, end, &entry_len);
    if (!p || (u64)(end - p) < entry_len) return ERR_TRUNCATED;
    const u8* ep = p;
    const u8* ee = p + entry_len;
    p = ee;
    const u8* key = nullptr;
    u64 key_len = 0;
    const u8* val = nullptr;
    u64 val_len = 0;
    while (ep < ee) {
      u64 etag;
      ep = read_varint(ep, ee, &etag);
      if (!ep) return ERR_BAD_VARINT;
      u32 efn = (u32)(etag >> 3), ewt = (u32)(etag & 7);
      if (efn == 1 && ewt == 2) {
        ep = read_varint(ep, ee, &key_len);
        if (!ep || (u64)(ee - ep) < key_len) return ERR_TRUNCATED;
        key = ep;
        ep += key_len;
      } else if (efn == 2 && ewt == 2) {
        ep = read_varint(ep, ee, &val_len);
        if (!ep || (u64)(ee - ep) < val_len) return ERR_TRUNCATED;
        val = ep;
        ep += val_len;
      } else {
        ep = skip_field(ep, ee, ewt);
        if (!ep) return ERR_TRUNCATED;
      }
    }
    if (!key) continue;
    int code = 0;
    if (val) {
      if (!seq) {
        int32_t kf = 0;
        i64 nvals = 0, nbytes = 0;
        int32_t rc = scan_feature_body(val, val + val_len, -1, &kf, &nvals, &nbytes);
        if (rc != ERR_OK) return rc;
        if (kf != 0 && nvals > 0) code = (4 - kf) + (nvals > 1 ? 3 : 0);
      } else {
        const u8* lp = val;
        const u8* le = val + val_len;
        int kind_seen = 0;
        while (lp < le) {
          u64 ltag;
          lp = read_varint(lp, le, &ltag);
          if (!lp) return ERR_BAD_VARINT;
          u32 lfn = (u32)(ltag >> 3), lwt = (u32)(ltag & 7);
          if (lfn == 1 && lwt == 2) {
            u64 flen;
            lp = read_varint(lp, le, &flen);
            if (!lp || (u64)(le - lp) < flen) return ERR_TRUNCATED;
            int32_t kf = 0;
            i64 nvals = 0, nbytes = 0;
            int32_t rc = scan_feature_body(lp, lp + flen, -1, &kf, &nvals, &nbytes);
            if (rc != ERR_OK) return rc;
            if (kf) {
              int r = 4 - kf;
              kind_seen = kind_seen > r ? kind_seen : r;
            }
            lp += flen;
          } else {
            lp = skip_field(lp, le, lwt);
            if (!lp) return ERR_TRUNCATED;
          }
        }
        if (kind_seen) code = 6 + kind_seen;
      }
    }
    if (key_len > 0xFFFF) return ERR_NAME_TOO_LONG;
    long long nameref = ((long long)(key - data) << 16) | (long long)key_len;
    u64 hash = fnv1a64(key, key_len);
    if (!lds_infer_merge(ltab, hash, nameref, code) &&
        !infer_slot_merge(table, lo, half, hash, nameref, code))
      return ERR_OVERFLOW;
  }
  return ERR_OK;
}

__global__ void infer_codes_kernel(const u8* __restrict__ data,
                                   const i64* __restrict__ off,
                                   const i64* __restrict__ len, i64 R, int32_t fmt,
                                   InferSlot* __restrict__ table, int nslots,
                                   int32_t* __restrict__ err) {
  __shared__ LdsInferSlot lctx[kLdsInfer];
  __shared__ LdsInferSlot lseq[kLdsInfer];
  for (int i = threadIdx.x; i < kLdsInfer; i += blockDim.x) {
    lctx[i].hash = 0;
    lctx[i].code = 0;
    lseq[i].hash = 0;
    lseq[i].code = 0;
  }
  __syncthreads();
  for (i64 r = blockIdx.x * (i64)blockDim.x + threadIdx.x; r < R;
       r += (i64)gridDim.x * blockDim.x) {
    const u8* p = data + off[r];
    const u8* end = p + len[r];
    while (p < end) {
      u64 tag;
      const u8* np = read_varint(p, end, &tag);
      if (!np) {
        set_err(err, ERR_BAD_VARINT, r);
        break;
      }
      p = np;
      u32 fieldno = (u32)(tag >> 3), wt = (u32)(tag & 7);
      bool is_features = fieldno == 1;
      bool is_fl = (fmt == FMT_SEQUENCE && fieldno == 2);
      if ((is_features || is_fl) && wt == 2) {
        u64 blen;
        p = read_varint(p, end, &blen);
        if (!p || (u64)(end - p) < blen) {
          set_err(err, ERR_TRUNCATED, r);
          break;
        }
        int32_t rc = infer_features_body_dev(data, p, p + blen, is_fl,
                                             is_fl ? lseq : lctx, table, nslots);
        if (rc != ERR_OK) {
          set_err(err, rc, r);
          break;
        }
        p += blen;
      } else {
        p = skip_field(p, end, wt);
        if (!p) {
          set_err(err, ERR_TRUNCATED, r);
          break;
        }
      }
    }
  }
  __syncthreads();
  int half = nslots / 2;
  for (int i = threadIdx.x; i < kLdsInfer; i += blockDim.x) {
    if (lctx[i].hash &&
        !infer_slot_merge(table, 0, half, lctx[i].hash, lctx[i].nameref,
                          (int)lctx[i].code))
      err[0] = ERR_OVERFLOW;
    if (lseq[i].hash &&
        !infer_slot_merge(table, half, half, lseq[i].hash, lseq[i].nameref,
                          (int)lseq[i].code))
      err[0] = ERR_OVERFLOW;
  }
}

__global__ void gather_payloads_kernel(const u8* __restrict__ data,
                                       const i64* __restrict__ off,
                                       const i64* __restrict__ len,
                                       const i64* __restrict__ dst_off, i64 R,
                                       u8* __restrict__ out) {
  for (i64 r = blockIdx.x * (i64)blockDim.x + threadIdx.x; r < R;
       r += (i64)gridDim.x * blockDim.x) {
    const u8* s = data + off[r];
    u8* d = out + dst_off[r];
    i64 n = len[r];
    i64 i = 0;
    for (; i + 8 <= n; i += 8) {
      u64 w;
      __builtin_memcpy(&w, s + i, 8);
      __builtin_memcpy(d + i, &w, 8);
    }
    for (; i < n; ++i) d[i] = s[i];
  }
}


inline int grid_for(i64 n, i64 max_blocks = 0) {
  i64 blocks = (n + kBlock - 1) / kBlock;
  i64 cap = max_blocks > 0 && max_blocks < 8192 ? max_blocks : 8192;
  if (blocks > cap) blocks = cap;
  if (blocks < 1) blocks = 1;
  return (int)blocks;
}

void gpu_crc_verify(uintptr_t data, uintptr_t off, uintptr_t len, i64 R,
                    uintptr_t err_out, uintptr_t stream, i64 avg_bytes) {
  if (avg_bytes > kWaveRecordBytes) {
    hipLaunchKernelGGL(crc_verify_wave_kernel, dim3(grid_for(R * 64)),
                       dim3(kBlock), 0, (hipStream_t)stream, (const u8*)data,
                       (const i64*)off, (const i64*)len, R,
                       (unsigned long long*)err_out);
  } else {
    hipLaunchKernelGGL(crc_verify_kernel, dim3(grid_for(R)), dim3(kBlock), 0,
                       (hipStream_t)stream, (const u8*)data, (const i64*)off,
                       (const i64*)len, R, (unsigned long long*)err_out);
  }
  HIP_CHECK(hipGetLastError());
}

void gpu_scan_records(uintptr_t data, uintptr_t off, uintptr_t len, i64 R,
                      int32_t fmt, uintptr_t schema_blob, int F, uintptr_t stats,
                      uintptr_t err, uintptr_t crc_err, uintptr_t stream,
                      i64 avg_bytes, i64 rec_base, i64 max_blocks) {
  if (R <= 0) return;
  if (avg_bytes > kWaveRecordBytes) {
    hipLaunchKernelGGL(scan_records_wave_kernel,
                       dim3(grid_for(R * 64, max_blocks)), dim3(kBlock), 0,
                       (hipStream_t)stream, (const u8*)data, (const i64*)off,
                       (const i64*)len, R, fmt, (const u8*)schema_blob, F,
                       (FieldStat*)stats, (int32_t*)err,
                       (unsigned long long*)crc_err, rec_base);
  } else {
    hipLaunchKernelGGL(scan_records_kernel, dim3(grid_for(R, max_blocks)),
                       dim3(kBlock), 0, (hipStream_t)stream, (const u8*)data,
                       (const i64*)off, (const i64*)len, R, fmt,
                       (const u8*)schema_blob, F, (FieldStat*)stats,
                       (int32_t*)err, (unsigned long long*)crc_err, rec_base);
  }
  HIP_CHECK(hipGetLastError());
}

void gpu_extract_fields(uintptr_t data, i64 R, int F, uintptr_t stats,
                        py::list metas, uintptr_t meta_dev, uintptr_t err,
                        uintptr_t stream, i64 avg_bytes, i64 r0,
                        i64 max_blocks) {
  if (R <= 0 || F <= 0) return;
  std::vector<DevFieldDst> host_metas(F);
  for (int f = 0; f < F; ++f) {
    py::dict d = metas[f].cast<py::dict>();
    DevFieldDst& m = host_metas[f];
    m.kind = d["kind"].cast<int32_t>();
    m.is_seq = d["is_seq"].cast<int32_t>();
    m.i64_vals = (i64*)d["i64_vals"].cast<uintptr_t>();
    m.f32_vals = (float*)d["f32_vals"].cast<uintptr_t>();
    m.bytes_data = (u8*)d["bytes_data"].cast<uintptr_t>();
    m.elem_len = (i64*)d["elem_len"].cast<uintptr_t>();
    m.sub_count = (i64*)d["sub_count"].cast<uintptr_t>();
    m.val_base = (const i64*)d["val_base"].cast<uintptr_t>();
    m.byte_base = (const i64*)d["byte_base"].cast<uintptr_t>();
    m.list_base = (const i64*)d["list_base"].cast<uintptr_t>();
  }
  HIP_CHECK(hipMemcpyAsync((void*)meta_dev, host_metas.data(),
                           sizeof(DevFieldDst) * F, hipMemcpyHostToDevice,
                           (hipStream_t)stream));
  if (avg_bytes > kWaveRecordBytes) {
    hipLaunchKernelGGL(extract_fields_wave_kernel,
                       dim3(grid_for(R * F * 64, max_blocks)), dim3(kBlock), 0,
                       (hipStream_t)stream, (const u8*)data, R, F,
                       (const FieldStat*)stats, (const DevFieldDst*)meta_dev,
                       (int32_t*)err, r0);
  } else {
    hipLaunchKernelGGL(extract_fields_kernel,
                       dim3(grid_for(R * F, max_blocks)), dim3(kBlock), 0,
                       (hipStream_t)stream, (const u8*)data, R, F,
                       (const FieldStat*)stats, (const DevFieldDst*)meta_dev,
                       (int32_t*)err, r0);
  }
  HIP_CHECK(hipGetLastError());
}

size_t gpu_devcols_bytes(int F) { return sizeof(FieldColumn) * (size_t)F; }

void fill_devcols(py::list cols, std::vector<FieldColumn>& out) {
  int F = (int)cols.size();
  out.resize(F);
  for (int f = 0; f < F; ++f) {
    py::dict d = cols[f].cast<py::dict>();
    FieldColumn& c = out[f];
    c.kind = d["kind"].cast<int32_t>();
    c.is_seq = d["is_seq"].cast<int32_t>();
    c.presence = (const u8*)d["presence"].cast<uintptr_t>();
    c.row_off = (const i64*)d["row_off"].cast<uintptr_t>();
    c.list_off = (const i64*)d["list_off"].cast<uintptr_t>();
    c.sub_off = (const i64*)d["sub_off"].cast<uintptr_t>();
    c.elem_off = (const i64*)d["elem_off"].cast<uintptr_t>();
    c.bytes_data = (const u8*)d["values_bytes"].cast<uintptr_t>();
    c.i64_vals = (const i64*)d["values_i64"].cast<uintptr_t>();
    c.f32_vals = (const float*)d["values_f32"].cast<uintptr_t>();
  }
}

void gpu_size_records(py::list cols, uintptr_t cols_dev, uintptr_t schema_blob,
                      int32_t fmt, i64 R, uintptr_t psize, uintptr_t stream) {
  static thread_local std::vector<FieldColumn> host_cols;
  fill_devcols(cols, host_cols);
  HIP_CHECK(hipMemcpyAsync((void*)cols_dev, host_cols.data(),
                           sizeof(FieldColumn) * host_cols.size(),
                           hipMemcpyHostToDevice, (hipStream_t)stream));
  hipLaunchKernelGGL(size_records_kernel, dim3(grid_for(R)), dim3(kBlock), 0,
                     (hipStream_t)stream, (const FieldColumn*)cols_dev,
                     (const u8*)schema_blob, fmt, R, (i64*)psize);
  HIP_CHECK(hipGetLastError());
}

void gpu_emit_records(uintptr_t cols_dev, uintptr_t schema_blob, int32_t fmt,
                      i64 r0, i64 R, uintptr_t frame_off, uintptr_t file,
                      uintptr_t err, uintptr_t stream, i64 avg_bytes) {
  if (avg_bytes > kWaveRecordBytes) {
    hipLaunchKernelGGL(emit_records_wave_kernel, dim3(grid_for((R - r0) * 64)),
                       dim3(kBlock), 0, (hipStream_t)stream,
                       (const FieldColumn*)cols_dev, (const u8*)schema_blob,
                       fmt, r0, R, (const i64*)frame_off, (u8*)file,
                       (int32_t*)err);
  } else {
    hipLaunchKernelGGL(emit_records_kernel, dim3(grid_for(R - r0)),
                       dim3(kBlock), 0, (hipStream_t)stream,
                       (const FieldColumn*)cols_dev, (const u8*)schema_blob,
                       fmt, r0, R, (const i64*)frame_off, (u8*)file,
                       (int32_t*)err);
  }
  HIP_CHECK(hipGetLastError());
}

void gpu_frame_bytes(uintptr_t src, uintptr_t elem_off, uintptr_t frame_off, i64 R,
                     uintptr_t file, uintptr_t stream, i64 avg_bytes) {
  if (avg_bytes > kWaveRecordBytes) {
    hipLaunchKernelGGL(frame_bytes_wave_kernel, dim3(grid_for(R * 64)),
                       dim3(kBlock), 0, (hipStream_t)stream, (const u8*)src,
                       (const i64*)elem_off, (const i64*)frame_off, R,
                       (u8*)file);
  } else {
    hipLaunchKernelGGL(frame_bytes_kernel, dim3(grid_for(R)), dim3(kBlock), 0,
                       (hipStream_t)stream, (const u8*)src, (const i64*)elem_off,
                       (const i64*)frame_off, R, (u8*)file);
  }
  HIP_CHECK(hipGetLastError());
}

i64 gpu_frame_scan_blocks(i64 pos_start, i64 pos_end) {
  i64 c_lo = pos_start / kPosPerLane;
  i64 c_hi = (pos_end + kPosPerLane - 1) / kPosPerLane;
  i64 n = c_hi - c_lo;
  return (n + kBlock - 1) / kBlock;
}

void gpu_frame_scan_count(uintptr_t data, i64 N, i64 pos_start, i64 pos_end,
                          i64 block_base, uintptr_t block_counts,
                          uintptr_t stream) {
  i64 B = gpu_frame_scan_blocks(pos_start, pos_end);
  if (B <= 0) return;
  hipLaunchKernelGGL(frame_scan_pass_kernel<false>, dim3((uint32_t)B),
                     dim3(kBlock), 0, (hipStream_t)stream, (const u8*)data, N,
                     pos_start, pos_end, block_base, (i64*)block_counts,
                     nullptr, nullptr);
  HIP_CHECK(hipGetLastError());
}

void gpu_frame_scan_emit(uintptr_t data, i64 N, i64 pos_start, i64 pos_end,
                         i64 block_base, uintptr_t block_off,
                         uintptr_t cand_pos, uintptr_t cand_len,
                         uintptr_t stream) {
  i64 B = gpu_frame_scan_blocks(pos_start, pos_end);
  if (B <= 0) return;
  hipLaunchKernelGGL(frame_scan_pass_kernel<true>, dim3((uint32_t)B),
                     dim3(kBlock), 0, (hipStream_t)stream, (const u8*)data, N,
                     pos_start, pos_end, block_base, (i64*)block_off,
                     (i64*)cand_pos, (i64*)cand_len);
  HIP_CHECK(hipGetLastError());
}

void gpu_frame_chain(uintptr_t pos, uintptr_t len, i64 C, uintptr_t carry_in,
                     uintptr_t carry_out, uintptr_t off, uintptr_t broken,
                     uintptr_t stream) {
  if (C <= 0) return;
  hipLaunchKernelGGL(frame_chain_kernel, dim3(grid_for(C)), dim3(kBlock), 0,
                     (hipStream_t)stream, (const i64*)pos, (const i64*)len, C,
                     (const i64*)carry_in, (i64*)carry_out, (i64*)off,
                     (i64*)broken);
  HIP_CHECK(hipGetLastError());
}

void gpu_infer_codes(uintptr_t data, uintptr_t off, uintptr_t len, i64 R,
                     int32_t fmt, uintptr_t table, int nslots, uintptr_t err,
                     uintptr_t stream) {
  hipLaunchKernelGGL(infer_codes_kernel, dim3(grid_for(R)), dim3(kBlock), 0,
                     (hipStream_t)stream, (const u8*)data, (const i64*)off,
                     (const i64*)len, R, fmt, (InferSlot*)table, nslots,
                     (int32_t*)err);
  HIP_CHECK(hipGetLastError());
}

void gpu_gather_payloads(uintptr_t data, uintptr_t off, uintptr_t len,
                         uintptr_t dst_off, i64 R, uintptr_t out,
                         uintptr_t stream, i64 avg_bytes) {
  if (avg_bytes > kWaveRecordBytes) {
    hipLaunchKernelGGL(gather_payloads_wave_kernel, dim3(grid_for(R * 64)),
                       dim3(kBlock), 0, (hipStream_t)stream, (const u8*)data,
                       (const i64*)off, (const i64*)len, (const i64*)dst_off,
                       R, (u8*)out);
  } else {
    hipLaunchKernelGGL(gather_payloads_kernel, dim3(grid_for(R)), dim3(kBlock),
                       0, (hipStream_t)stream, (const u8*)data,
                       (const i64*)off, (const i64*)len, (const i64*)dst_off,
                       R, (u8*)out);
  }
  HIP_CHECK(hipGetLastError());
}


struct StridedLoadI64 {
  const i64* p;
  i64 stride;
  __host__ __device__ i64 operator()(i64 i) const { return p[i * stride]; }
};

size_t gpu_scan_temp_bytes(i64 n) {
  size_t bytes = 0;
  auto it = rocprim::make_transform_iterator(
      rocprim::make_counting_iterator<i64>(0), StridedLoadI64{nullptr, 1});
  (void)rocprim::inclusive_scan(nullptr, bytes, it, (i64*)nullptr, (size_t)n,
                                rocprim::plus<i64>());
  return bytes;
}


struct Seg3 {
  i64 v0, v1, v2;
  u32 flag;
};

struct Seg3Combine {
  __host__ __device__ Seg3 operator()(const Seg3& a, const Seg3& b) const {
    if (b.flag) return b;
    return Seg3{a.v0 + b.v0, a.v1 + b.v1, a.v2 + b.v2, a.flag};
  }
};

struct Seg3Load {
  const i64* stats;
  i64 n;
  int F;
  i64 r0;
  i64 stride;
  const i64* b0;
  const i64* b1;
  const i64* b2;
  __host__ __device__ Seg3 operator()(i64 idx) const {
    i64 f = idx / n;
    i64 q = idx - f * n;
    const i64* st = stats + ((r0 + q) * F + f) * 6;
    if (q != 0) return Seg3{st[2], st[3], st[4], 0u};
    i64 at = f * stride + r0;
    return Seg3{st[2] + b0[at], st[3] + b1[at], st[4] + b2[at], 1u};
  }
};

struct Seg3OutRef {
  i64* o0;
  i64* o1;
  i64* o2;
  __host__ __device__ Seg3OutRef& operator=(const Seg3& v) {
    *o0 = v.v0;
    *o1 = v.v1;
    *o2 = v.v2;
    return *this;
  }
};

struct Seg3OutIt {
  using value_type = Seg3;
  using reference = Seg3OutRef;
  using pointer = Seg3OutRef*;
  using difference_type = i64;
  using iterator_category = std::random_access_iterator_tag;
  i64* b0;
  i64* b1;
  i64* b2;
  i64 n;
  i64 r0;
  i64 stride;
  i64 pos;
  __host__ __device__ Seg3OutRef operator*() const { return (*this)[0]; }
  __host__ __device__ Seg3OutRef operator[](i64 k) const {
    i64 idx = pos + k;
    i64 f = idx / n;
    i64 q = idx - f * n;
    i64 at = f * stride + r0 + q + 1;
    return Seg3OutRef{b0 + at, b1 + at, b2 + at};
  }
  __host__ __device__ Seg3OutIt operator+(i64 k) const {
    return Seg3OutIt{b0, b1, b2, n, r0, stride, pos + k};
  }
  __host__ __device__ Seg3OutIt& operator+=(i64 k) {
    pos += k;
    return *this;
  }
  __host__ __device__ Seg3OutIt& operator++() {
    ++pos;
    return *this;
  }
};

size_t gpu_stat_scan_temp_bytes(i64 R, int F) {
  size_t bytes = 0;
  auto in = rocprim::make_transform_iterator(
      rocprim::make_counting_iterator<i64>(0),
      Seg3Load{nullptr, R, F, 0, R + 1, nullptr, nullptr, nullptr});
  Seg3OutIt out{nullptr, nullptr, nullptr, R, 0, R + 1, 0};
  (void)rocprim::inclusive_scan(nullptr, bytes, in, out, (size_t)(R * F),
                                Seg3Combine());
  return bytes;
}

void gpu_stat_scans(uintptr_t temp, size_t temp_bytes, uintptr_t stats, i64 R,
                    int F, uintptr_t val_base, uintptr_t byte_base,
                    uintptr_t list_base, uintptr_t stream, i64 r0, i64 r1,
                    i64 stride) {
  auto s = (hipStream_t)stream;
  if (r1 < 0) r1 = R;
  if (stride <= 0) stride = R + 1;
  if (r0 < 0 || r1 > R || r1 >= stride)
    throw std::runtime_error("gpu_stat_scans: range outside the planes");
  i64 n = r1 - r0;
  if (n <= 0 || F <= 0) return;
  auto in = rocprim::make_transform_iterator(
      rocprim::make_counting_iterator<i64>(0),
      Seg3Load{(const i64*)stats, n, F, r0, stride, (const i64*)val_base,
               (const i64*)byte_base, (const i64*)list_base});
  Seg3OutIt out{(i64*)val_base, (i64*)byte_base, (i64*)list_base, n, r0,
                stride, 0};
  size_t tb = temp_bytes;
  HIP_CHECK(rocprim::inclusive_scan((void*)temp, tb, in, out,
                                    (size_t)(n * F), Seg3Combine(), s));
}

void gpu_excl_sum_strided(uintptr_t temp, size_t temp_bytes, uintptr_t in,
                          i64 stride, uintptr_t out, i64 n, uintptr_t stream) {
  auto s = (hipStream_t)stream;
  HIP_CHECK(hipMemsetAsync((void*)out, 0, sizeof(i64), s));
  if (n <= 0) return;
  auto it = rocprim::make_transform_iterator(
      rocprim::make_counting_iterator<i64>(0), StridedLoadI64{(const i64*)in, stride});
  size_t tb = temp_bytes;
  hipError_t e = rocprim::inclusive_scan((void*)temp, tb, it, (i64*)out + 1,
                                         (size_t)n, rocprim::plus<i64>(), s);
  HIP_CHECK(e);
}


struct MappedFile {
  void* ptr = nullptr;
  size_t n = 0;
  dev_t dev = 0;
  ino_t ino = 0;
  bool pinned = false;
  bool writable = false;
};

std::map<std::string, MappedFile> g_mmap_cache;
std::mutex g_mmap_mu;
size_t g_mmap_bytes = 0;
constexpr size_t kMmapCacheCap = 4ull << 30;

void drop_mapping_locked(const std::string& key) {
  auto it = g_mmap_cache.find(key);
  if (it == g_mmap_cache.end()) return;
  if (it->second.pinned) {
    (void)hipDeviceSynchronize();
    (void)hipHostUnregister(it->second.ptr);
  }
  munmap(it->second.ptr, it->second.n);
  g_mmap_bytes -= it->second.n;
  g_mmap_cache.erase(it);
}

void sweep_stale_locked() {
  for (auto it = g_mmap_cache.begin(); it != g_mmap_cache.end();) {
    struct stat st {};
    bool live = stat(it->first.c_str(), &st) == 0 &&
                st.st_dev == it->second.dev && st.st_ino == it->second.ino &&
                (size_t)st.st_size >= it->second.n;
    if (live) {
      ++it;
    } else {
      auto key = it->first;
      ++it;
      drop_mapping_locked(key);
    }
  }
}

py::tuple file_mmap_pinned(const std::string& path, i64 n, bool writable) {
  if (n <= 0) return py::make_tuple((uintptr_t)0, true);
  std::lock_guard<std::mutex> lk(g_mmap_mu);
  sweep_stale_locked();
  int flags = writable ? (O_RDWR | O_CREAT) : O_RDWR;
  int fd = ::open(path.c_str(), flags, 0644);
  bool rdonly = false;
  if (fd < 0 && !writable) {
    fd = ::open(path.c_str(), O_RDONLY);
    rdonly = true;
  }
  if (fd < 0)
    throw std::runtime_error("open failed: " + path + ": " + strerror(errno));
  struct stat st {};
  if (fstat(fd, &st) != 0) {
    ::close(fd);
    throw std::runtime_error("stat failed: " + path);
  }
  auto it = g_mmap_cache.find(path);
  if (it != g_mmap_cache.end()) {
    MappedFile& m = it->second;
    if (m.dev == st.st_dev && m.ino == st.st_ino && m.n == (size_t)n &&
        st.st_size >= (off_t)n && (m.writable || !writable)) {
      ::close(fd);
      return py::make_tuple((uintptr_t)m.ptr, m.pinned);
    }
    drop_mapping_locked(path);
  }
  if (writable && st.st_size != (off_t)n && ftruncate(fd, (off_t)n) != 0) {
    int e = errno;
    ::close(fd);
    throw std::runtime_error("ftruncate failed: " + path + ": " + strerror(e));
  }
  if (!writable && st.st_size < (off_t)n) {
    ::close(fd);
    throw std::runtime_error("short file: " + path);
  }
  while (g_mmap_bytes + (size_t)n > kMmapCacheCap && !g_mmap_cache.empty())
    drop_mapping_locked(g_mmap_cache.begin()->first);
  int prot = PROT_READ | ((writable || !rdonly) ? PROT_WRITE : 0);
  void* p = mmap(nullptr, (size_t)n, prot, MAP_SHARED, fd, 0);
  ::close(fd);
  if (p == MAP_FAILED)
    throw std::runtime_error("mmap failed: " + path + ": " + strerror(errno));
  bool pinned = hipHostRegister(p, (size_t)n, hipHostRegisterDefault) == hipSuccess;
  if (!pinned) (void)hipGetLastError();
  MappedFile m{p, (size_t)n, st.st_dev, st.st_ino, pinned,
               writable || !rdonly};
  g_mmap_cache[path] = m;
  g_mmap_bytes += (size_t)n;
  return py::make_tuple((uintptr_t)p, pinned);
}

void file_mmap_drop(const std::string& path) {
  std::lock_guard<std::mutex> lk(g_mmap_mu);
  drop_mapping_locked(path);
}

void file_mmap_sync(const std::string& path) {
  std::lock_guard<std::mutex> lk(g_mmap_mu);
  auto it = g_mmap_cache.find(path);
  if (it != g_mmap_cache.end() && it->second.ptr) {
    if (msync(it->second.ptr, it->second.n, MS_SYNC) != 0)
      throw std::runtime_error("msync failed: " + path + ": " +
                               strerror(errno));
  }
  int fd = ::open(path.c_str(), O_RDONLY);
  if (fd >= 0) {
    (void)fsync(fd);
    ::close(fd);
  }
}


void gpu_memcpy_d2h(uintptr_t dst, uintptr_t src, i64 n, uintptr_t stream) {
  HIP_CHECK(hipMemcpyAsync((void*)dst, (const void*)src, (size_t)n,
                           hipMemcpyDeviceToHost, (hipStream_t)stream));
}

void gpu_memcpy_h2d(uintptr_t dst, uintptr_t src, i64 n, uintptr_t stream) {
  HIP_CHECK(hipMemcpyAsync((void*)dst, (const void*)src, (size_t)n,
                           hipMemcpyHostToDevice, (hipStream_t)stream));
}

}

void register_gpu(py::module_& m) {
  m.def("gpu_device_count", []() {
    int n = 0;
    hipError_t e = hipGetDeviceCount(&n);
    return (e == hipSuccess) ? n : -static_cast<int>(e);
  });
  m.def("gpu_crc_verify", &gpu_crc_verify, py::arg("data"), py::arg("off"),
        py::arg("len"), py::arg("R"), py::arg("err_out"), py::arg("stream"),
        py::arg("avg_bytes") = 0);
  m.def("gpu_scan_records", &gpu_scan_records, py::arg("data"), py::arg("off"),
        py::arg("len"), py::arg("R"), py::arg("fmt"), py::arg("schema_blob"),
        py::arg("F"), py::arg("stats"), py::arg("err"), py::arg("crc_err"),
        py::arg("stream"), py::arg("avg_bytes") = 0, py::arg("rec_base") = 0,
        py::arg("max_blocks") = 0);
  m.def("gpu_extract_fields", &gpu_extract_fields, py::arg("data"),
        py::arg("R"), py::arg("F"), py::arg("stats"), py::arg("metas"),
        py::arg("meta_dev"), py::arg("err"), py::arg("stream"),
        py::arg("avg_bytes") = 0, py::arg("r0") = 0,
        py::arg("max_blocks") = 0);
  m.def("gpu_size_records", &gpu_size_records);
  m.def("gpu_emit_records", &gpu_emit_records, py::arg("cols_dev"),
        py::arg("schema_blob"), py::arg("fmt"), py::arg("r0"), py::arg("R"),
        py::arg("frame_off"), py::arg("file"), py::arg("err"),
        py::arg("stream"), py::arg("avg_bytes") = 0);
  m.def("gpu_frame_bytes", &gpu_frame_bytes, py::arg("src"),
        py::arg("elem_off"), py::arg("frame_off"), py::arg("R"),
        py::arg("file"), py::arg("stream"), py::arg("avg_bytes") = 0);
  m.def("gpu_frame_scan_blocks", &gpu_frame_scan_blocks);
  m.def("gpu_frame_scan_count", &gpu_frame_scan_count);
  m.def("gpu_frame_scan_emit", &gpu_frame_scan_emit);
  m.def("gpu_frame_chain", &gpu_frame_chain);
  m.def("gpu_gather_payloads", &gpu_gather_payloads, py::arg("data"),
        py::arg("off"), py::arg("len"), py::arg("dst_off"), py::arg("R"),
        py::arg("out"), py::arg("stream"), py::arg("avg_bytes") = 0);
  m.def("gpu_infer_codes", &gpu_infer_codes);
  m.def("gpu_scan_temp_bytes", &gpu_scan_temp_bytes);
  m.def("gpu_stat_scan_temp_bytes", &gpu_stat_scan_temp_bytes);
  m.def("gpu_stat_scans", &gpu_stat_scans, py::arg("temp"),
        py::arg("temp_bytes"), py::arg("stats"), py::arg("R"), py::arg("F"),
        py::arg("val_base"), py::arg("byte_base"), py::arg("list_base"),
        py::arg("stream"), py::arg("r0") = 0, py::arg("r1") = -1,
        py::arg("stride") = 0);
  m.def("gpu_excl_sum_strided", &gpu_excl_sum_strided);
  m.def("file_mmap_pinned", &file_mmap_pinned, py::arg("path"), py::arg("n"),
        py::arg("writable"));
  m.def("file_mmap_drop", &file_mmap_drop);
  m.def("file_mmap_sync", &file_mmap_sync);
  m.def("gpu_memcpy_d2h", &gpu_memcpy_d2h);
  m.def("gpu_memcpy_h2d", &gpu_memcpy_h2d);
  m.def("gpu_devcols_bytes", &gpu_devcols_bytes);
  m.def("gpu_devmeta_bytes", []() { return sizeof(DevFieldDst); });
  m.def("gpu_fieldstat_words", []() { return sizeof(FieldStat) / 8; });
}
```

spark_tfrecord_amd/engine/gpu.py:

```python

from __future__ import annotations

import os
import threading
import warnings
from typing import List, Optional

import numpy as np
import torch

from .. import _native
from . import stream_plan
from ..columnar import RecordBatch, WireColumn, schema_blob, wire_fields
from ..schema import KIND_BYTES, KIND_FLOAT, KIND_INT64, StructType, is_sequence_field, wire_kind_of

FMT = {"Example": _native.FMT_EXAMPLE, "SequenceExample": _native.FMT_SEQUENCE}


def _stream() -> int:
    return torch.cuda.current_stream().cuda_stream


def _dev(x, dtype, device="cuda") -> torch.Tensor:
    if isinstance(x, torch.Tensor):
        return x.to(device=device, dtype=dtype).contiguous()
    arr = np.ascontiguousarray(x)
    with warnings.catch_warnings():
        warnings.simplefilter("ignore", UserWarning)
        return torch.as_tensor(arr, dtype=dtype).to(device)


def check_native():
    if not getattr(_native, "HAS_GPU_KERNELS", False):
        raise RuntimeError("_native was built without HIP kernels; rebuild "
                           "with build_native.py before using the GPU engine")



_pinned_tls = threading.local()


def pinned_buffer(tag: str, nbytes: int) -> torch.Tensor:
    pool = getattr(_pinned_tls, "pool", None)
    if pool is None:
        pool = _pinned_tls.pool = {}
    buf = pool.get(tag)
    if buf is None or buf.numel() < nbytes:
        cap = max(nbytes, int((buf.numel() if buf is not None else 1 << 20) * 1.5))
        buf = torch.empty(cap, dtype=torch.uint8, pin_memory=True)
        pool[tag] = buf
    return buf


_CHUNK = 64 << 20
_READ_SLICE = int(os.environ.get("TFREC_READ_SLICE", 32 << 20))
_SPLIT_SLICES = os.environ.get("TFREC_READ_SPLIT", "1") != "0"
_WRITE_SLICES = int(os.environ.get("TFREC_WRITE_SLICES", 8))
_STREAM_DECODE = os.environ.get("TFREC_STREAM_DECODE", "1") != "0"
_STREAM_HEADROOM = float(os.environ.get("TFREC_STREAM_HEADROOM", 1.125))
_STREAM_EXTRACT = os.environ.get("TFREC_STREAM_EXTRACT", "1") != "0"
_SYNC_WRITES = os.environ.get("TFREC_SYNC", "1") != "0"


def read_file_to_device(path: str, device="cuda") -> torch.Tensor:
    n = os.path.getsize(path)
    dev_t = torch.empty(max(n, 1), dtype=torch.uint8, device=device)[:n]
    if n:
        ptr, pinned = _native.file_mmap_pinned(path, n, False)
        if pinned:
            _multi_dma(dev_t.data_ptr(), ptr, n, _native.gpu_memcpy_h2d,
                       after_main=True)
            return dev_t
    return _read_file_staged(path, dev_t)


_copy_streams: Optional[list] = None


def _dma_streams() -> list:
    global _copy_streams
    if _copy_streams is None:
        _copy_streams = [torch.cuda.Stream() for _ in range(2)]
    return _copy_streams


def _multi_dma(dst: int, src: int, n: int, fn, after_main: bool):
    streams = _dma_streams()
    main = torch.cuda.current_stream()
    k = min(len(streams), max(1, n // (16 << 20)))
    span = (n + k - 1) // k
    for i in range(k):
        o = i * span
        m = min(span, n - o)
        s = streams[i]
        s.wait_stream(main)
        fn(dst + o, src + o, m, s.cuda_stream)
    if after_main:
        for i in range(k):
            main.wait_stream(streams[i])
    else:
        for i in range(k):
            streams[i].synchronize()


def _read_file_staged(path: str, dev: torch.Tensor) -> torch.Tensor:
    n = dev.numel()
    buf = pinned_buffer("fread", min(n, 2 * _CHUNK) or 1)
    ev = [torch.cuda.Event(), torch.cuda.Event()]
    fd = os.open(path, os.O_RDONLY)
    try:
        pos = 0
        which = 0
        while pos < n:
            m = min(_CHUNK, n - pos)
            ev[which].synchronize()
            _native.pread_parallel(fd, buf.data_ptr() + which * _CHUNK, m, pos)
            dev[pos:pos + m].copy_(buf[which * _CHUNK:which * _CHUNK + m],
                                   non_blocking=True)
            ev[which].record()
            pos += m
            which ^= 1 if n > _CHUNK else 0
    finally:
        os.close(fd)
    return dev


def device_to_file(img: torch.Tensor, path: str):
    n = img.numel()
    if n == 0:
        open(path, "wb").close()
        return
    ptr, pinned = _native.file_mmap_pinned(path, n, True)
    if pinned:
        _multi_dma(ptr, img.data_ptr(), n, _native.gpu_memcpy_d2h,
                   after_main=False)
        if _SYNC_WRITES:
            _native.file_mmap_sync(path)
        return
    _write_file_staged(img, path)


def _write_file_staged(img: torch.Tensor, path: str):
    n = img.numel()
    buf = pinned_buffer("fwrite", min(n, 2 * _CHUNK) or 1)
    ev = [torch.cuda.Event(), torch.cuda.Event()]
    fd = os.open(path, os.O_RDWR | os.O_CREAT, 0o644)
    try:
        pos = 0
        which = 0
        m0 = min(_CHUNK, n)
        if n:
            buf[0:m0].copy_(img[0:m0], non_blocking=True)
            ev[0].record()
        while pos < n:
            m = min(_CHUNK, n - pos)
            nxt = pos + m
            nwhich = which ^ (1 if n > _CHUNK else 0)
            if nxt < n:
                m2 = min(_CHUNK, n - nxt)
                buf[nwhich * _CHUNK:nwhich * _CHUNK + m2].copy_(
                    img[nxt:nxt + m2], non_blocking=True)
                ev[nwhich].record()
            ev[which].synchronize()
            _native.pwrite_parallel(fd, buf.data_ptr() + which * _CHUNK, m, pos)
            pos = nxt
            which = nwhich
        os.ftruncate(fd, n)
        if _SYNC_WRITES:
            os.fsync(fd)
    finally:
        os.close(fd)



_scan_ws = {}


def _scan_workspace(n: int, device) -> torch.Tensor:
    key = (device.index if hasattr(device, "index") else 0)
    need = _native.gpu_scan_temp_bytes(max(n, 1))
    ws = _scan_ws.get(key)
    if ws is None or ws.numel() < need:
        ws = torch.empty(int(need * 2), dtype=torch.uint8, device=device)
        _scan_ws[key] = ws
    return ws


def _excl_sum_into(out_ptr: int, in_ptr: int, stride: int, n: int, device):
    ws = _scan_workspace(n, device)
    _native.gpu_excl_sum_strided(ws.data_ptr(), ws.numel(), in_ptr, stride,
                                 out_ptr, n, _stream())


def _stat_scan_workspace(R: int, F: int, device) -> torch.Tensor:
    key = ("stat", device.index if hasattr(device, "index") else 0)
    need = _native.gpu_stat_scan_temp_bytes(R, F)
    ws = _scan_ws.get(key)
    if ws is None or ws.numel() < need:
        ws = torch.empty(int(need * 2) or 1, dtype=torch.uint8, device=device)
        _scan_ws[key] = ws
    return ws


def excl_sum(t: torch.Tensor) -> torch.Tensor:
    n = t.numel()
    out = torch.empty(n + 1, dtype=torch.int64, device=t.device)
    _excl_sum_into(out.data_ptr(), t.data_ptr(), 1, n, t.device)
    return out


def device_to_bytes(img: torch.Tensor) -> bytes:
    n = img.numel()
    buf = pinned_buffer("d2h", n)
    buf[:n].copy_(img, non_blocking=True)
    torch.cuda.synchronize()
    return buf.numpy()[:n].tobytes()


def device_to_pinned_view(img: torch.Tensor, tag: str = "d2h_img") -> np.ndarray:
    n = img.numel()
    buf = pinned_buffer(tag, n)
    buf[:n].copy_(img, non_blocking=True)
    torch.cuda.synchronize()
    return buf.numpy()[:n]



def scan_frames_device(data: torch.Tensor):
    check_native()
    N = data.numel()
    device = data.device
    if N == 0:
        z = torch.zeros(0, dtype=torch.int64, device=device)
        return z, z.clone()
    B = _native.gpu_frame_scan_blocks(0, N)
    block_counts = torch.empty(B, dtype=torch.int64, device=device)
    _native.gpu_frame_scan_count(data.data_ptr(), N, 0, N, 0,
                                 block_counts.data_ptr(), _stream())
    off, lens, _ = _emit_and_chain(data, [(0, N)], block_counts, N)
    return off, lens


def _emit_and_chain(data, ranges, block_counts, N):
    device = data.device
    block_off = excl_sum(block_counts)
    C = int(block_off[-1].item())
    if C == 0:
        raise RuntimeError("corrupt TFRecord: no valid frame header found")
    pos = torch.empty(C, dtype=torch.int64, device=device)
    lens = torch.empty(C, dtype=torch.int64, device=device)
    base = 0
    for s, e in ranges:
        _native.gpu_frame_scan_emit(data.data_ptr(), N, s, e, base,
                                    block_off.data_ptr(), pos.data_ptr(),
                                    lens.data_ptr(), _stream())
        base += _native.gpu_frame_scan_blocks(s, e)
    expect_next = pos + 16 + lens
    ok = bool(((pos[0] == 0) & (expect_next[-1] == N)
               & (expect_next[:-1] == pos[1:]).all()).item())
    if not ok:
        pos_h = pos.cpu().numpy()
        len_h = lens.cpu().numpy()
        keep = []
        cur = 0
        pmap = {int(p): i for i, p in enumerate(pos_h)}
        while cur < N:
            i = pmap.get(cur)
            if i is None:
                raise RuntimeError(
                    f"corrupt TFRecord: broken frame chain at offset {cur}")
            keep.append(i)
            cur = int(pos_h[i] + 16 + len_h[i])
        sel = torch.as_tensor(np.asarray(keep, np.int64), device=device)
        pos = pos[sel]
        lens = lens[sel]
    return pos + 12, lens, ok



def crc_verify_device(data: torch.Tensor, off: torch.Tensor, lens: torch.Tensor,
                      avg_bytes: int = 0):
    R = off.numel()
    if R == 0:
        return
    if not avg_bytes:
        avg_bytes = max(0, (data.numel() // R) - 16)
    err = torch.full((1,), -1, dtype=torch.int64, device=data.device)
    _native.gpu_crc_verify(data.data_ptr(), off.data_ptr(), lens.data_ptr(), R,
                           err.data_ptr(), _stream(), avg_bytes)
    bad = int(err.item())
    if bad != -1:
        raise RuntimeError(
            f"corrupt TFRecord: bad CRC in record {bad - 1 if bad > 0 else bad}")


def decode_device(data: torch.Tensor, off: torch.Tensor, lens: torch.Tensor,
                  schema: StructType, record_type: str,
                  verify_crc: bool = True) -> RecordBatch:
    check_native()
    device = data.device
    R = off.numel()
    fields = wire_fields(schema)
    F = len(fields)
    if verify_crc and record_type == "ByteArray":
        crc_verify_device(data, off, lens)

    if record_type == "ByteArray":
        dst_off = excl_sum(lens.contiguous())
        total = int(dst_off[-1].item())
        out = torch.empty(total, dtype=torch.uint8, device=device)
        if R:
            _native.gpu_gather_payloads(data.data_ptr(), off.data_ptr(),
                                        lens.data_ptr(), dst_off.data_ptr(), R,
                                        out.data_ptr(), _stream(), total // R)
        col = WireColumn(kind=KIND_BYTES, is_seq=False,
                         presence=torch.ones(R, dtype=torch.uint8, device=device),
                         row_off=torch.arange(R + 1, dtype=torch.int64, device=device),
                         values=out, elem_off=dst_off)
        return RecordBatch(schema, [col], R)

    if F == 0 or R == 0:
        cols = [WireColumn(wire_kind_of(f.dataType), is_sequence_field(f.dataType),
                           torch.zeros(R, dtype=torch.uint8, device=device),
                           torch.zeros(R + 1, dtype=torch.int64, device=device),
                           torch.zeros(0, dtype=torch.int64, device=device))
                for f in fields]
        return RecordBatch(schema, cols, R)

    blob = _schema_blob_device(schema, device)
    stats = torch.empty((R, F, 6), dtype=torch.int64, device=device)
    err = torch.zeros(2, dtype=torch.int32, device=device)
    crc_err = None
    fuse_crc = verify_crc
    if fuse_crc:
        crc_err = torch.full((1,), -1, dtype=torch.int64, device=device)
    avg_bytes = max(0, (data.numel() // R) - 16) if R else 0
    _native.gpu_scan_records(data.data_ptr(), off.data_ptr(), lens.data_ptr(),
                             R, FMT[record_type], blob.data_ptr(), F,
                             stats.data_ptr(), err.data_ptr(),
                             crc_err.data_ptr() if fuse_crc else 0,
                             _stream(), avg_bytes)

    val_base = torch.empty((F, R + 1), dtype=torch.int64, device=device)
    byte_base = torch.empty((F, R + 1), dtype=torch.int64, device=device)
    list_base = torch.empty((F, R + 1), dtype=torch.int64, device=device)
    val_base[:, 0] = 0
    byte_base[:, 0] = 0
    list_base[:, 0] = 0
    ws = _stat_scan_workspace(R, F, device)
    _native.gpu_stat_scans(ws.data_ptr(), ws.numel(), stats.data_ptr(), R, F,
                           val_base.data_ptr(), byte_base.data_ptr(),
                           list_base.data_ptr(), _stream())
    totals = torch.stack([val_base[:, -1], byte_base[:, -1], list_base[:, -1]])
    totals_h = totals.cpu()
    _raise_scan_errors(int(crc_err.item()) if fuse_crc else -1,
                       int(err[0].item()), int(err[1].item()))
    vals = _FieldValues(fields, data.numel(), device)
    meta_dev = torch.empty(F * _native.gpu_devmeta_bytes(), dtype=torch.uint8,
                           device=device)
    vals.extract(data, stats, (val_base, byte_base, list_base), 0, R, totals_h,
                 data.numel(), meta_dev, err, avg_bytes)
    cols = vals.columns(stats, val_base, list_base, R)
    if int(err[0].item()) != 0:
        _raise_extract_error(int(err[0].item()), int(err[1].item()))
    return RecordBatch(schema, cols, R)


_schema_blobs = {}


def _schema_blob_device(schema: StructType, device) -> torch.Tensor:
    raw = bytes(schema_blob(schema))
    key = (raw, str(torch.device(device)))
    blob = _schema_blobs.get(key)
    if blob is None:
        if len(_schema_blobs) >= 64:
            _schema_blobs.clear()
        blob = torch.frombuffer(bytearray(raw), dtype=torch.uint8).to(device)
        _schema_blobs[key] = blob
    return blob


def _raise_scan_errors(crc_bad: int, rc: int, rec1: int):
    if crc_bad != -1:
        raise RuntimeError(f"corrupt TFRecord: bad CRC in record {crc_bad - 1}")
    if rc != 0:
        rec = rec1 - 1
        where = f" in record {rec}" if rec >= 0 else ""
        raise RuntimeError(f"TFRecord decode failed{where} (native error "
                           f"{rc}; kind mismatch or malformed record)")


def _raise_extract_error(rc: int, rec1: int):
    rec = rec1 - 1
    where = f" (record {rec})" if rec >= 0 else ""
    raise RuntimeError(f"TFRecord decode failed in value extraction"
                       f"{where} (native error {rc})")


class _FieldValues:

    _BUFS = {"i64_vals": (torch.int64, 0, KIND_INT64),
             "f32_vals": (torch.float32, 0, KIND_FLOAT),
             "elem_len": (torch.int64, 0, KIND_BYTES),
             "bytes_data": (torch.uint8, 1, None),
             "sub_count": (torch.int64, 2, None)}

    def __init__(self, fields, total_bytes: int, device):
        self.total_bytes = total_bytes
        self.device = device
        self.kinds = [wire_kind_of(f.dataType) for f in fields]
        self.seqs = [is_sequence_field(f.dataType) for f in fields]
        self.filled = [[0] * len(fields) for _ in range(3)]
        self.bufs = [{k: torch.empty(0, dtype=d, device=device)
                      for k, (d, _, _) in self._BUFS.items()} for _ in fields]

    def _reserve(self, totals, bytes_seen: int):
        for i, bufs in enumerate(self.bufs):
            for name, (_, dim, kind) in self._BUFS.items():
                if kind not in (None, self.kinds[i]):
                    continue
                need = int(totals[dim][i])
                old = bufs[name]
                cap = stream_plan.grown_capacity(
                    old.numel(), need, bytes_seen, self.total_bytes,
                    _STREAM_HEADROOM, min_unit=1)
                if cap == old.numel():
                    continue
                new = torch.empty(cap, dtype=old.dtype, device=self.device)
                k = self.filled[dim][i]
                if k:
                    new[:k].copy_(old[:k])
                if old.numel():
                    last_read["regrows"] = last_read.get("regrows", 0) + 1
                bufs[name] = new

    def extract(self, data, stats, planes, r0: int, r1: int, totals,
                bytes_seen: int, meta_dev, err, avg_bytes: int):
        self._reserve(totals, bytes_seen)
        v, b, l = planes
        metas = []
        for i, bufs in enumerate(self.bufs):
            metas.append({
                "kind": self.kinds[i], "is_seq": 1 if self.seqs[i] else 0,
                **{name: t.data_ptr() for name, t in bufs.items()},
                "val_base": v[i].data_ptr(),
                "byte_base": b[i].data_ptr(),
                "list_base": l[i].data_ptr() if self.seqs[i] else 0,
            })
        _native.gpu_extract_fields(data.data_ptr(), r1 - r0, len(self.bufs),
                                   stats.data_ptr(), metas,
                                   meta_dev.data_ptr(), err.data_ptr(),
                                   _stream(), avg_bytes, r0=r0)
        self.filled = [[int(totals[d][i]) for i in range(len(self.bufs))]
                       for d in range(3)]

    def columns(self, stats, val_base, list_base, R: int) -> List[WireColumn]:
        cols = []
        for i, bufs in enumerate(self.bufs):
            kind, seq = self.kinds[i], self.seqs[i]
            nv, nb, nl = (self.filled[d][i] for d in range(3))
            presence = (stats[:, i, 0] >= 0).to(torch.uint8)
            elem_off = None
            if kind == KIND_BYTES:
                elem_off = excl_sum(bufs["elem_len"][:nv])
            sub_off = None
            if seq:
                sub_off = excl_sum(bufs["sub_count"][:nl])
            values = (bufs["i64_vals"][:nv] if kind == KIND_INT64 else
                      bufs["f32_vals"][:nv] if kind == KIND_FLOAT else
                      bufs["bytes_data"][:nb])
            cols.append(WireColumn(kind, seq, presence, val_base[i][:R + 1],
                                   values, elem_off,
                                   list_base[i][:R + 1] if seq else None,
                                   sub_off))
        return cols


def decode_buffer_device(data_np: np.ndarray, schema: StructType, record_type: str,
                         verify_crc: bool = True, device="cuda") -> RecordBatch:
    data_np = np.ascontiguousarray(data_np, np.uint8)
    n = data_np.size
    stage = pinned_buffer("h2d", n)
    stage.numpy()[:n] = data_np
    data = torch.empty(n, dtype=torch.uint8, device=device)
    data.copy_(stage[:n], non_blocking=True)
    off, lens = scan_frames_device(data)
    return decode_device(data, off, lens, schema, record_type, verify_crc)


def read_file_to_batch(path: str, schema: StructType, record_type: str,
                       verify_crc: bool = True, device="cuda") -> RecordBatch:
    return read_file_to_batch_pipelined(path, schema, record_type, verify_crc,
                                        device)



def _col_ptrs(col: WireColumn) -> dict:
    def p(t):
        return t.data_ptr() if isinstance(t, torch.Tensor) and t.numel() else 0

    return {
        "kind": col.kind, "is_seq": 1 if col.is_seq else 0,
        "presence": p(col.presence), "row_off": p(col.row_off),
        "list_off": p(col.list_off) if col.list_off is not None else 0,
        "sub_off": p(col.sub_off) if col.sub_off is not None else 0,
        "elem_off": p(col.elem_off) if col.elem_off is not None else 0,
        "values_bytes": p(col.values) if col.kind == KIND_BYTES else 0,
        "values_i64": p(col.values) if col.kind == KIND_INT64 else 0,
        "values_f32": p(col.values) if col.kind == KIND_FLOAT else 0,
    }


def _check_emit_err(err: torch.Tensor):
    if int(err[0].item()) != 0:
        rec = int(err[1].item()) - 1
        where = f" in record {rec}" if rec >= 0 else ""
        raise RuntimeError(f"TFRecord encode failed: size/emit mismatch{where}")


def _size_records(batch: RecordBatch, record_type: str, device):
    blob = _schema_blob_device(batch.schema, device)
    col_dicts = [_col_ptrs(c) for c in batch.columns]
    cols_dev = torch.empty(_native.gpu_devcols_bytes(len(col_dicts)),
                           dtype=torch.uint8, device=device)
    psize = torch.empty(batch.num_rows, dtype=torch.int64, device=device)
    _native.gpu_size_records(col_dicts, cols_dev.data_ptr(), blob.data_ptr(),
                             FMT[record_type], batch.num_rows,
                             psize.data_ptr(), _stream())
    return cols_dev, blob, psize, excl_sum(psize)


def encode_device(batch: RecordBatch, record_type: str) -> torch.Tensor:
    check_native()
    R = batch.num_rows
    device = batch.columns[0].presence.device if batch.columns else torch.device("cuda")
    if record_type == "ByteArray":
        col = batch.columns[0]
        lens = col.elem_off[1:] - col.elem_off[:-1]
        frame_off = excl_sum((lens + 16).contiguous())
        total = int(frame_off[-1].item())
        file = torch.empty(total, dtype=torch.uint8, device=device)
        if R:
            _native.gpu_frame_bytes(col.values.data_ptr(), col.elem_off.data_ptr(),
                                    frame_off.data_ptr(), R, file.data_ptr(),
                                    _stream(), (total // R) - 16)
        return file

    cols_dev, blob, _, frame_off = _size_records(batch, record_type, device)
    total = int(frame_off[-1].item())
    file = torch.empty(total, dtype=torch.uint8, device=device)
    err = torch.zeros(2, dtype=torch.int32, device=device)
    _native.gpu_emit_records(cols_dev.data_ptr(), blob.data_ptr(),
                             FMT[record_type], 0, R, frame_off.data_ptr(),
                             file.data_ptr(), err.data_ptr(), _stream(),
                             total // max(R, 1))
    _check_emit_err(err)
    return file


def write_batch_to_file(batch: RecordBatch, path: str,
                        record_type: str = "Example",
                        slices: Optional[int] = None) -> int:
    check_native()
    R = batch.num_rows
    if record_type == "ByteArray" or R == 0:
        img = encode_device(batch, record_type)
        device_to_file(img, path)
        return img.numel()
    device = batch.columns[0].presence.device
    cols_dev, blob, _, frame_off = _size_records(batch, record_type, device)
    S = max(1, min(slices if slices is not None else _WRITE_SLICES, R))
    ridx = [R * s // S for s in range(S + 1)]
    bounds = frame_off[ridx].cpu()
    total = int(bounds[-1])
    file = torch.empty(total, dtype=torch.uint8, device=device)
    err = torch.zeros(2, dtype=torch.int32, device=device)
    ptr, pinned = _native.file_mmap_pinned(path, total, True)
    if not pinned:
        _native.gpu_emit_records(cols_dev.data_ptr(), blob.data_ptr(),
                                 FMT[record_type], 0, R, frame_off.data_ptr(),
                                 file.data_ptr(), err.data_ptr(), _stream(),
                                 total // R)
        _check_emit_err(err)
        _write_file_staged(file, path)
        return total
    main = torch.cuda.current_stream()
    streams = _dma_streams()
    for s in range(S):
        _native.gpu_emit_records(cols_dev.data_ptr(), blob.data_ptr(),
                                 FMT[record_type], ridx[s], ridx[s + 1],
                                 frame_off.data_ptr(), file.data_ptr(),
                                 err.data_ptr(), _stream(), total // R)
        b0, b1 = int(bounds[s]), int(bounds[s + 1])
        if b1 > b0:
            w = streams[s % len(streams)]
            w.wait_stream(main)
            _native.gpu_memcpy_d2h(ptr + b0, file.data_ptr() + b0, b1 - b0,
                                   w.cuda_stream)
    for w in streams:
        w.synchronize()
    if _SYNC_WRITES:
        _native.file_mmap_sync(path)
    _check_emit_err(err)
    return total


last_read = {}

_ST_BROKEN, _ST_CRC, _ST_ERR, _ST_XERR, _ST_CARRY = 0, 1, 2, 3, 4


class _StreamStatus:

    def __init__(self, max_chains: int, device):
        self.words = torch.zeros(_ST_CARRY + 1 + max_chains, dtype=torch.int64,
                                 device=device)
        self.words[_ST_CRC] = -1
        self.err = self.words[_ST_ERR:_ST_ERR + 1].view(torch.int32)
        self.xerr = self.words[_ST_XERR:_ST_XERR + 1].view(torch.int32)

    def addr(self, word: int) -> int:
        return self.words.data_ptr() + word * 8

    def carry_addr(self, k: int) -> int:
        return self.addr(_ST_CARRY + k)

    def head(self) -> torch.Tensor:
        return self.words[:_ST_CARRY]

    @staticmethod
    def chain_end(h, nchain: int) -> Optional[int]:
        return None if int(h[_ST_BROKEN]) != 0 else int(h[_ST_CARRY + nchain])

    @staticmethod
    def scan_error(h):
        pair = h[_ST_ERR:_ST_ERR + 1].view(torch.int32)
        return int(h[_ST_CRC]), int(pair[0]), int(pair[1])


class _StreamRows:

    def __init__(self, total_bytes: int, F: int, device):
        self.total_bytes = total_bytes
        self.F = F
        self.device = device
        self.cap = 0
        self.pos = self.lens = self.off = self.stats = None
        self.planes = None

    def _alloc(self, cap: int):
        i64 = dict(dtype=torch.int64, device=self.device)
        planes = None
        if self.F:
            planes = [torch.empty((self.F, cap + 1), **i64) for _ in range(3)]
            for t in planes:
                t[:, 0] = 0
        return (torch.empty(cap, **i64), torch.empty(cap, **i64),
                torch.empty(cap, **i64),
                torch.empty((cap, self.F, 6), **i64) if self.F else None,
                planes)

    def cand_ptrs(self, c: int):
        return (self.pos.data_ptr() + c * 8, self.lens.data_ptr() + c * 8,
                self.off.data_ptr() + c * 8)

    def row_ptrs(self, r: int):
        return (self.off.data_ptr() + r * 8, self.lens.data_ptr() + r * 8,
                self.stats.data_ptr() + r * self.F * 48)

    def scan_stats(self, r0: int, r1: int):
        ws = _stat_scan_workspace(r1 - r0, self.F, self.device)
        v, b, l = self.planes
        _native.gpu_stat_scans(ws.data_ptr(), ws.numel(),
                               self.stats.data_ptr(), r1, self.F, v.data_ptr(),
                               b.data_ptr(), l.data_ptr(), _stream(), r0=r0,
                               r1=r1, stride=self.cap + 1)

    def totals(self, r: int) -> list:
        return [t[:, r] for t in self.planes]

    def reserve(self, need: int, n_cand: int, n_scanned: int, bytes_seen: int):
        cap = stream_plan.grown_capacity(self.cap, need, bytes_seen,
                                         self.total_bytes, _STREAM_HEADROOM)
        if cap == self.cap:
            return
        pos, lens, off, stats, planes = self._alloc(cap)
        if n_cand:
            pos[:n_cand].copy_(self.pos[:n_cand])
            lens[:n_cand].copy_(self.lens[:n_cand])
            off[:n_cand].copy_(self.off[:n_cand])
        if n_scanned and stats is not None:
            stats[:n_scanned].copy_(self.stats[:n_scanned])
            for new, old in zip(planes, self.planes):
                new[:, :n_scanned + 1].copy_(old[:, :n_scanned + 1])
        self.pos, self.lens, self.off, self.stats = pos, lens, off, stats
        self.planes = planes
        if self.cap:
            last_read["regrows"] = last_read.get("regrows", 0) + 1
        self.cap = cap


class _StreamedRead:

    def __init__(self, data: torch.Tensor, nslices: int, schema: StructType,
                 record_type: str, verify_crc: bool):
        device = data.device
        self.data = data
        self.n = data.numel()
        self.schema = schema
        self.record_type = record_type
        self.verify_crc = verify_crc
        fields = wire_fields(schema)
        F = self.F = len(fields)
        self.do_scan = record_type != "ByteArray" and F > 0
        self.status = _StreamStatus(nslices, device)
        self.rows = _StreamRows(self.n, F if self.do_scan else 0, device)
        if self.do_scan:
            self.blob = _schema_blob_device(schema, device)
            self.vals = _FieldValues(fields, self.n, device)
            self.meta_dev = torch.empty(F * _native.gpu_devmeta_bytes(),
                                        dtype=torch.uint8, device=device)
        self.C = 0
        self.nchain = 0
        self.r_done = 0
        self.x_done = 0
        self.clean = True
        self.avg_bytes = None

    def discover(self, p: stream_plan.SlicePlan, counts: torch.Tensor):
        block_off = excl_sum(counts)
        c_s = int(block_off[-1].item())
        if not c_s:
            return
        self.rows.reserve(self.C + c_s, self.C, self.r_done, p.scan_hi)
        pos, lens, off = self.rows.cand_ptrs(self.C)
        _native.gpu_frame_scan_emit(self.data.data_ptr(), self.n, p.scan_lo,
                                    p.scan_hi, 0, block_off.data_ptr(), pos,
                                    lens, _stream())
        _native.gpu_frame_chain(pos, lens, c_s,
                                self.status.carry_addr(self.nchain),
                                self.status.carry_addr(self.nchain + 1), off,
                                self.status.addr(_ST_BROKEN), _stream())
        self.nchain += 1
        self.C += c_s

    def arrived(self, p: stream_plan.SlicePlan, last: bool):
        if not self.do_scan or self.C == self.r_done:
            return self.r_done, p.b1
        if last:
            return self.C, self.n
        end = self.status.chain_end(self.status.words.cpu(), self.nchain)
        if end is None:
            return None
        avail = stream_plan.arrived_records(self.C, end, p.b1)
        return avail, end if avail == self.C else p.b1

    def scan(self, avail: int, end: int, last: bool):
        r0 = self.r_done
        if avail <= r0:
            return
        if self.avg_bytes is None:
            self.avg_bytes = max(0, end // avail - 16)
        off, lens, stats = self.rows.row_ptrs(r0)
        _native.gpu_scan_records(
            self.data.data_ptr(), off, lens, avail - r0, FMT[self.record_type],
            self.blob.data_ptr(), self.F, stats, self.status.err.data_ptr(),
            self.status.addr(_ST_CRC) if self.verify_crc else 0, _stream(),
            self.avg_bytes, rec_base=r0)
        self.rows.scan_stats(r0, avail)
        self.r_done = avail
        if not _STREAM_EXTRACT or last or not self.clean:
            return
        F = self.F
        h = torch.cat(self.rows.totals(avail) + [self.status.head()]).cpu()
        crc_bad, rc, _ = self.status.scan_error(h[3 * F:])
        if crc_bad != -1 or rc != 0:
            self.clean = False
            return
        self._extract(avail, h[:3 * F].view(3, F), end)

    def _extract(self, r1: int, totals_h, bytes_seen: int):
        self.vals.extract(self.data, self.rows.stats, self.rows.planes,
                          self.x_done, r1, totals_h, bytes_seen, self.meta_dev,
                          self.status.xerr, self.avg_bytes)
        self.x_done = r1

    def finish(self) -> Optional[RecordBatch]:
        R, F, n = self.C, self.F, self.n
        if R == 0:
            return None
        if not self.do_scan:
            if self.status.chain_end(self.status.words.cpu(), self.nchain) != n:
                return None
            return decode_device(self.data, self.rows.off[:R],
                                 self.rows.lens[:R], self.schema,
                                 self.record_type, self.verify_crc)
        packed = torch.cat(self.rows.totals(R) + [self.status.words]).cpu()
        st_h = packed[3 * F:]
        if self.status.chain_end(st_h, self.nchain) != n:
            return None
        crc_bad, rc, rec1 = self.status.scan_error(st_h)
        _raise_scan_errors(crc_bad if self.verify_crc else -1, rc, rec1)
        if not self.clean:
            raise RuntimeError("streamed decode: scan error lost")
        if self.x_done < R:
            self._extract(R, packed[:3 * F].view(3, F), n)
        val_base, _, list_base = self.rows.planes
        cols = self.vals.columns(self.rows.stats[:R], val_base, list_base, R)
        err_h = self.status.xerr.cpu()
        if int(err_h[0]) != 0:
            _raise_extract_error(int(err_h[0]), int(err_h[1]))
        return RecordBatch(self.schema, cols, R)


def _issue_h2d_slices(data: torch.Tensor, ptr: int, plan) -> list:
    main = torch.cuda.current_stream()
    streams = _dma_streams()
    for st in streams:
        st.wait_stream(main)
    events = []
    for s, p in enumerate(plan):
        half = (p.b1 - p.b0) // 2 if _SPLIT_SLICES and len(streams) > 1 else 0
        parts = ([(p.b0, p.b0 + half, 0), (p.b0 + half, p.b1, 1)] if half
                 else [(p.b0, p.b1, s % len(streams))])
        evs = []
        for lo, hi, k in parts:
            st = streams[k]
            _native.gpu_memcpy_h2d(data.data_ptr() + lo, ptr + lo, hi - lo,
                                   st.cuda_stream)
            ev = torch.cuda.Event()
            ev.record(st)
            evs.append(ev)
        events.append(evs)
    for st in streams:
        data.record_stream(st)
    return events


def _scan_blocks(p: stream_plan.SlicePlan) -> int:
    if p.scan_hi <= p.scan_lo:
        return 0
    return int(_native.gpu_frame_scan_blocks(p.scan_lo, p.scan_hi))


def _count_slice(data, p, evs, block_counts, base: int) -> int:
    main = torch.cuda.current_stream()
    for ev in evs:
        main.wait_event(ev)
    nb = _scan_blocks(p)
    if nb:
        _native.gpu_frame_scan_count(data.data_ptr(), data.numel(), p.scan_lo,
                                     p.scan_hi, base, block_counts.data_ptr(),
                                     _stream())
    return nb


def _read_unstreamed(data, plan, block_counts, events, first: int,
                     schema: StructType, record_type: str,
                     verify_crc: bool) -> RecordBatch:
    last_read["path"] = "fallback" if _STREAM_DECODE else "unstreamed"
    base = sum(_scan_blocks(p) for p in plan[:first])
    for p, evs in zip(plan[first:], events[first:]):
        base += _count_slice(data, p, evs, block_counts, base)
    ranges = [(p.scan_lo, p.scan_hi) for p in plan if p.scan_hi > p.scan_lo]
    off, lens, _ = _emit_and_chain(data, ranges, block_counts, data.numel())
    return decode_device(data, off, lens, schema, record_type, verify_crc)


def read_file_to_batch_pipelined(path: str, schema: StructType, record_type: str,
                                 verify_crc: bool = True,
                                 device="cuda") -> RecordBatch:
    check_native()
    n = os.path.getsize(path)
    if n == 0:
        z = torch.zeros(0, dtype=torch.int64, device=device)
        return decode_device(torch.zeros(0, dtype=torch.uint8, device=device),
                             z, z.clone(), schema, record_type, verify_crc)
    ptr, pinned = _native.file_mmap_pinned(path, n, False)
    if not pinned:
        data = _read_file_staged(path, torch.empty(n, dtype=torch.uint8,
                                                   device=device))
        off, lens = scan_frames_device(data)
        return decode_device(data, off, lens, schema, record_type, verify_crc)
    data = torch.empty(n, dtype=torch.uint8, device=device)
    plan = stream_plan.plan_slices(n, _READ_SLICE)
    S = len(plan)
    block_counts = torch.empty(max(sum(_scan_blocks(p) for p in plan), 1),
                               dtype=torch.int64, device=data.device)
    events = _issue_h2d_slices(data, ptr, plan)
    last_read.update(path="streamed", slices=S, regrows=0)
    unstreamed = (data, plan, block_counts, events)
    decode = (schema, record_type, verify_crc)
    if not _STREAM_DECODE:
        return _read_unstreamed(*unstreamed, 0, *decode)

    rd = _StreamedRead(data, S, *decode)
    base = 0
    for s, p in enumerate(plan):
        nb = _count_slice(data, p, events[s], block_counts, base)
        if nb:
            rd.discover(p, block_counts[base:base + nb])
            base += nb
        got = rd.arrived(p, last=s == S - 1)
        if got is None:
            return _read_unstreamed(*unstreamed, s + 1, *decode)
        rd.scan(*got, last=s == S - 1)
    batch = rd.finish()
    if batch is None:
        return _read_unstreamed(*unstreamed, S, *decode)
    return batch


def gz_device_meta(path: str):
    from ..io import paths as P

    if not getattr(_native, "HAS_GPU_KERNELS", False):
        return None
    return P.parse_gz_segments_file(path)


def _device_inflate_group(data: torch.Tensor, gz_items, device) -> bool:
    comp_sizes = [os.path.getsize(p) for p, _, _ in gz_items]
    comp_total = sum(comp_sizes)
    comp = torch.empty(max(comp_total, 1), dtype=torch.uint8,
                       device=device)[:comp_total]
    main = torch.cuda.current_stream()
    streams = _dma_streams()
    in_off = []
    in_len = []
    out_off = []
    out_len = []
    used = []
    coff = 0
    for k, (p, meta, out_base) in enumerate(gz_items):
        body_off, segs, _crc, _isize = meta
        ptr, pinned = _native.file_mmap_pinned(p, comp_sizes[k], False)
        if pinned:
            st = streams[k % len(streams)]
            st.wait_stream(main)
            _native.gpu_memcpy_h2d(comp.data_ptr() + coff, ptr, comp_sizes[k],
                                   st.cuda_stream)
            used.append(st)
        else:
            _read_file_staged(p, comp[coff:coff + comp_sizes[k]])
        so = coff + body_off
        uo = out_base
        for c, u in segs:
            in_off.append(so)
            in_len.append(c)
            out_off.append(uo)
            out_len.append(u)
            so += c
            uo += u
        coff += comp_sizes[k]
    for st in set(used):
        main.wait_stream(st)
    meta_np = np.array([in_off, in_len, out_off, out_len], np.int64)
    force = os.environ.get("TFREC_INFLATE_STREAMS", "")
    spw_lit = 2
    if force in ("1", "2", "4"):
        spw_lit = int(force)
        lit = np.full(meta_np.shape[1], spw_lit > 1)
    else:
        lit = meta_np[1] >= (0.85 * np.maximum(meta_np[3], 1))
    err = torch.full((1,), -1, dtype=torch.int64, device=device)
    for mask, spw in ((lit, spw_lit), (~lit, 1)):
        k = int(mask.sum())
        if k == 0:
            continue
        idx = np.nonzero(mask)[0]
        if spw == 2 and k > 2:
            idx = idx[np.argsort(-meta_np[3, idx], kind="stable")]
        sub = torch.as_tensor(
            np.ascontiguousarray(meta_np[:, idx])).to(device)
        _native.gpu_inflate_segments(
            comp.data_ptr(), sub[0].data_ptr(), sub[1].data_ptr(),
            sub[2].data_ptr(), sub[3].data_ptr(), k,
            data.data_ptr(), err.data_ptr(), _stream(), spw)
    return int(err.item()) == -1


def read_gzip_file_to_device(path: str, device="cuda") -> Optional[torch.Tensor]:
    meta = gz_device_meta(path)
    if meta is None:
        return None
    total_u = sum(u for _, u in meta[1])
    data = torch.empty(max(total_u, 1), dtype=torch.uint8,
                       device=device)[:total_u]
    if not _device_inflate_group(data, [(path, meta, 0)], device):
        return None
    return data


def read_files_to_batch(paths, schema: StructType, record_type: str,
                        verify_crc: bool = True, device="cuda"):
    from ..io import paths as P

    check_native()
    metas = []
    sizes = []
    for p in paths:
        if P.codec_from_path(p) == "gzip":
            meta = P.parse_gz_segments_file(p)
            if meta is None:
                raise ValueError(f"gzip file without segment table: {p} "
                                 "(host path required)")
            metas.append(meta)
            sizes.append(sum(u for _, u in meta[1]))
        else:
            metas.append(None)
            sizes.append(os.path.getsize(p))
    n = sum(sizes)
    if n == 0:
        if schema is None:
            raise ValueError(
                "Could not infer schema: no non-empty TFRecord files found")
        z = torch.zeros(0, dtype=torch.int64, device=device)
        return (decode_device(torch.zeros(0, dtype=torch.uint8, device=device),
                              z, z.clone(), schema, record_type, verify_crc),
                np.zeros(len(paths), np.int64))
    data = torch.empty(n, dtype=torch.uint8, device=device)
    bounds = np.zeros(len(paths) + 1, np.int64)
    np.cumsum(sizes, out=bounds[1:])
    main = torch.cuda.current_stream()
    streams = _dma_streams()
    gz_items = []
    for i, p in enumerate(paths):
        if not sizes[i]:
            continue
        if metas[i] is not None:
            gz_items.append((p, metas[i], int(bounds[i])))
            continue
        ptr, pinned = _native.file_mmap_pinned(p, sizes[i], False)
        if pinned:
            st = streams[i % len(streams)]
            _native.gpu_memcpy_h2d(data.data_ptr() + int(bounds[i]), ptr,
                                   sizes[i], st.cuda_stream)
            main.wait_stream(st)
        else:
            _read_file_staged(p, data[int(bounds[i]):int(bounds[i + 1])])
    if gz_items and not _device_inflate_group(data, gz_items, device):
        import logging

        logging.getLogger(__name__).warning(
            "device inflate rejected a segment; host zlib fallback for "
            "%d gzip file(s)", len(gz_items))
        for p, meta, base in gz_items:
            blob = np.frombuffer(P.decompress_file(p), np.uint8)
            stage = pinned_buffer("gzfb", blob.size)
            stage.numpy()[:blob.size] = blob
            data[base:base + blob.size].copy_(stage[:blob.size],
                                              non_blocking=True)
            torch.cuda.current_stream().synchronize()
    off, lens = scan_frames_device(data)
    frame_start = off - 12
    counts = torch.searchsorted(
        frame_start, torch.as_tensor(bounds, device=device)).cpu().numpy()
    row_counts = np.diff(counts)
    if schema is None:
        from ..infer import byte_array_schema, schema_from_codes

        if record_type == "ByteArray":
            schema = byte_array_schema()
        else:
            i = next((k for k in range(len(paths)) if row_counts[k] > 0), None)
            if i is None:
                raise ValueError(
                    "Could not infer schema: no non-empty TFRecord files found")
            r0, r1 = int(counts[i]), int(counts[i + 1])
            codes = infer_codes_device(data, off[r0:r1].contiguous(),
                                       lens[r0:r1].contiguous(), record_type)
            schema = schema_from_codes(codes)
    batch = decode_device(data, off, lens, schema, record_type, verify_crc)
    return batch, row_counts


def encode_partitions_device(batch: RecordBatch, part_codes: np.ndarray,
                             num_parts: int, record_type: str):
    check_native()
    R = batch.num_rows
    device = batch.columns[0].presence.device if batch.columns else torch.device("cuda")
    cols_dev, blob, psize, frame_off = _size_records(batch, record_type, device)
    total = int(frame_off[-1].item())
    file = torch.empty(total, dtype=torch.uint8, device=device)
    err = torch.zeros(2, dtype=torch.int32, device=device)
    _native.gpu_emit_records(cols_dev.data_ptr(), blob.data_ptr(),
                             FMT[record_type], 0, R, frame_off.data_ptr(),
                             file.data_ptr(), err.data_ptr(), _stream(),
                             total // max(R, 1))
    codes = torch.as_tensor(np.ascontiguousarray(part_codes, np.int64),
                            device=device)
    order = torch.argsort(codes, stable=True)
    sizes = psize[order].contiguous()
    dst_off = excl_sum(sizes)
    src_off = frame_off[:-1][order].contiguous()
    out = torch.empty(total, dtype=torch.uint8, device=device)
    _native.gpu_gather_payloads(file.data_ptr(), src_off.data_ptr(),
                                sizes.data_ptr(), dst_off.data_ptr(), R,
                                out.data_ptr(), _stream(), total // max(R, 1))
    counts = torch.bincount(codes, minlength=num_parts)
    row_bound = torch.nn.functional.pad(torch.cumsum(counts, 0), (1, 0))
    byte_bound = dst_off[row_bound].cpu().numpy()
    _check_emit_err(err)
    ranges = [(p, int(byte_bound[p]), int(byte_bound[p + 1]))
              for p in range(num_parts) if byte_bound[p + 1] > byte_bound[p]]
    return out, ranges



_INFER_SLOTS = 2048
_INFER_SLOTS_MAX = 1 << 21
_ERR_OVERFLOW = -5
_ERR_NAME_TOO_LONG = -6


def infer_codes_device(data: torch.Tensor, off: torch.Tensor,
                       lens: torch.Tensor, record_type: str) -> dict:
    check_native()
    device = data.device
    fmt = FMT["SequenceExample" if record_type == "SequenceExample" else "Example"]
    R = off.numel()
    slots = _INFER_SLOTS
    while True:
        table = torch.zeros((slots, 3), dtype=torch.int64, device=device)
        err = torch.zeros(2, dtype=torch.int32, device=device)
        if R:
            _native.gpu_infer_codes(data.data_ptr(), off.data_ptr(),
                                    lens.data_ptr(), R, fmt, table.data_ptr(),
                                    slots, err.data_ptr(), _stream())
        tab = table.cpu().numpy()
        rc = int(err[0].item())
        if rc == _ERR_OVERFLOW:
            if slots < _INFER_SLOTS_MAX:
                slots *= 4
                continue
            raise RuntimeError(
                "schema inference failed: more than "
                f"{_INFER_SLOTS_MAX // 2} distinct feature names")
        if rc == _ERR_NAME_TOO_LONG:
            raise RuntimeError(
                "schema inference failed: a feature name exceeds 65535 bytes")
        if rc != 0:
            rec = int(err[1].item()) - 1
            where = f" (record {rec})" if rec >= 0 else ""
            raise RuntimeError(f"malformed record during schema inference"
                               f"{where} (native error {rc})")
        break
    used = np.nonzero(tab[:, 0])[0]
    if len(used) == 0:
        return {}
    refs = tab[used, 1]
    offs = (refs >> 16).astype(np.int64)
    nlens = (refs & 0xFFFF).astype(np.int64)
    lo = int(offs.min())
    hi = int((offs + nlens).max())
    codes: dict = {}
    if hi - lo <= (4 << 20):
        blob = data[lo:hi].cpu().numpy().tobytes()
        for o, ln, code in zip(offs, nlens, tab[used, 2]):
            name = blob[o - lo:o - lo + ln].decode("utf-8", errors="replace")
            codes[name] = max(codes.get(name, 0), int(code))
    else:
        for o, ln, code in zip(offs, nlens, tab[used, 2]):
            name = data[o:o + ln].cpu().numpy().tobytes().decode("utf-8", errors="replace")
            codes[name] = max(codes.get(name, 0), int(code))
    return codes


def infer_schema_file(path: str, record_type: str, device="cuda"):
    from ..infer import schema_from_codes

    data = read_file_to_device(path, device)
    off, lens = scan_frames_device(data)
    return schema_from_codes(infer_codes_device(data, off, lens, record_type))


def batch_to_device(batch: RecordBatch, device="cuda") -> RecordBatch:
    cols = []
    for c in batch.columns:
        cols.append(WireColumn(
            c.kind, c.is_seq,
            _dev(c.presence, torch.uint8, device),
            _dev(c.row_off, torch.int64, device),
            _dev(c.values, {KIND_INT64: torch.int64, KIND_FLOAT: torch.float32,
                            KIND_BYTES: torch.uint8}[c.kind], device),
            _dev(c.elem_off, torch.int64, device) if c.elem_off is not None else None,
            _dev(c.list_off, torch.int64, device) if c.list_off is not None else None,
            _dev(c.sub_off, torch.int64, device) if c.sub_off is not None else None,
        ))
    return RecordBatch(batch.schema, cols, batch.num_rows)


def batch_to_host(batch: RecordBatch) -> RecordBatch:
    streams = _dma_streams()
    main = torch.cuda.current_stream()
    state = {"used": False, "k": 0}

    def h(t):
        if not isinstance(t, torch.Tensor):
            return t
        if not t.is_cuda:
            return t.numpy()
        host = torch.empty_like(t, device="cpu", pin_memory=True)
        if not state["used"]:
            for s in streams:
                s.wait_stream(main)
            state["used"] = True
        nbytes = t.numel() * t.element_size()
        if nbytes >= (8 << 20) and t.is_contiguous() and len(streams) > 1:
            flat_d = t.view(-1)
            flat_h = host.view(-1)
            n = flat_d.numel()
            step = (n + len(streams) - 1) // len(streams)
            for i, st in enumerate(streams):
                lo = i * step
                hi = min(n, lo + step)
                if lo >= hi:
                    break
                with torch.cuda.stream(st):
                    flat_h[lo:hi].copy_(flat_d[lo:hi], non_blocking=True)
                t.record_stream(st)
            return host.numpy()
        st = streams[state["k"] % len(streams)]
        state["k"] += 1
        with torch.cuda.stream(st):
            host.copy_(t, non_blocking=True)
        t.record_stream(st)
        return host.numpy()

    cols = [WireColumn(c.kind, c.is_seq, h(c.presence), h(c.row_off), h(c.values),
                       h(c.elem_off) if c.elem_off is not None else None,
                       h(c.list_off) if c.list_off is not None else None,
                       h(c.sub_off) if c.sub_off is not None else None)
            for c in batch.columns]
    if state["used"]:
        for s in streams:
            s.synchronize()
    return RecordBatch(batch.schema, cols, batch.num_rows)



def decode_buffer_to_cpu(data_np: np.ndarray, schema: StructType, record_type: str,
                         verify_crc: bool = True) -> RecordBatch:
    return batch_to_host(decode_buffer_device(data_np, schema, record_type,
                                              verify_crc))


def encode_batch_from_cpu(batch: RecordBatch, record_type: str) -> bytes:
    dev_batch = batch_to_device(batch)
    file = encode_device(dev_batch, record_type)
    return device_to_bytes(file)
```

spark_tfrecord_amd/engine/stream_plan.py:

```python

from __future__ import annotations

from typing import List, NamedTuple

MIN_FRAME = 16
SCAN_LOOKAHEAD = 32


class SlicePlan(NamedTuple):
    b0: int
    b1: int
    scan_lo: int
    scan_hi: int


def plan_slices(n: int, span: int) -> List[SlicePlan]:
    if n <= 0:
        return []
    span = max(1, int(span))
    S = (n + span - 1) // span
    out = []
    scanned = 0
    for s in range(S):
        b0, b1 = s * span, min(n, (s + 1) * span)
        hi = b1 - SCAN_LOOKAHEAD if s < S - 1 else n
        hi = max(hi, scanned)
        out.append(SlicePlan(b0, b1, scanned, hi))
        scanned = hi
    return out


def arrived_records(n_cand: int, last_end: int, arrived: int) -> int:
    if n_cand <= 0:
        return 0
    return n_cand if last_end <= arrived else n_cand - 1


def row_capacity(need: int, bytes_seen: int, total_bytes: int,
                 headroom: float, min_unit: int = MIN_FRAME) -> int:
    need = max(int(need), 0)
    bytes_seen = min(max(int(bytes_seen), 1), max(int(total_bytes), 1))
    est = int(need * (total_bytes / bytes_seen) * max(headroom, 1.0)) + 1
    most = need + max(total_bytes - bytes_seen, 0) // max(min_unit, 1)
    return max(need, min(est, most), 1)


def grown_capacity(cap: int, need: int, bytes_seen: int, total_bytes: int,
                   headroom: float, min_unit: int = MIN_FRAME) -> int:
    if need <= cap:
        return cap
    return row_capacity(need, bytes_seen, total_bytes, headroom, min_unit)
```

Baseline: 114.6 million rows/s.

## Replace per-slice host syncs in streamed read with device-gated kernels and snapshots

Restructures the streamed decode loop so each slice needs only one small snapshot kernel plus an event wait into pinned memory, replacing the several blocking .cpu() copies used before. Scan and extract kernels now take device-side gate flags, so a broken chain, CRC error or overflowed capacity makes them return early with no host round-trip. Extract speculatively runs ahead using reserved capacity and is confirmed one step later. Extraction also writes offsets and presence directly instead of lengths and counts, which removes later scan passes in column assembly. The cost is more complex speculative bookkeeping and possible re-extraction when the size guess is too small.

Result: no change. 116.7 million rows/s (median of 6 runs) (+1.8%).

```diff
diff --git a/csrc/codec_core.h b/csrc/codec_core.h
--- a/csrc/codec_core.h
+++ b/csrc/codec_core.h
@@ -785,6 +785,8 @@
   i64* sub_count;
 };
 
+
+template <bool OFFS = false>
 TFR_HOSTDEV inline int32_t extract_list_body(const u8* p, const u8* end, int32_t kind,
                                              const DecodeDst& dst, i64* vi, i64* bi) {
   while (p < end) {
@@ -810,7 +812,7 @@
         __builtin_memcpy(d + i, &w, 8);
       }
       for (; i < len; ++i) d[i] = p[i];
-      dst.elem_len[*vi] = static_cast<i64>(len);
+      dst.elem_len[*vi] = OFFS ? *bi : static_cast<i64>(len);
       *bi += static_cast<i64>(len);
       *vi += 1;
       p += len;
@@ -855,6 +857,7 @@
   return ERR_OK;
 }
 
+template <bool OFFS = false>
 TFR_HOSTDEV inline int32_t extract_feature_body(const u8* p, const u8* end,
                                                 int32_t kind, const DecodeDst& dst,
                                                 i64* vi, i64* bi) {
@@ -868,7 +871,7 @@
       u64 len;
       p = read_varint(p, end, &len);
       if (!p || static_cast<u64>(end - p) < len) return ERR_TRUNCATED;
-      int32_t rc = extract_list_body(p, p + len, kind, dst, vi, bi);
+      int32_t rc = extract_list_body<OFFS>(p, p + len, kind, dst, vi, bi);
       if (rc != ERR_OK) return rc;
       p += len;
     } else {
@@ -879,6 +882,7 @@
   return ERR_OK;
 }
 
+template <bool OFFS = false>
 TFR_HOSTDEV inline int32_t extract_field(const u8* data, i64 pos, i64 len,
                                          int32_t kind, int32_t is_seq,
                                          const DecodeDst& dst, i64 val_base,
@@ -888,7 +892,8 @@
   const u8* end = p + len;
   i64 vi = val_base;
   i64 bi = byte_base;
-  if (!is_seq) return extract_feature_body(p, end, kind, dst, &vi, &bi);
+  if (!is_seq)
+    return extract_feature_body<OFFS>(p, end, kind, dst, &vi, &bi);
   i64 li = list_base;
   while (p < end) {
     u64 tag;
@@ -901,9 +906,9 @@
       p = read_varint(p, end, &flen);
       if (!p || static_cast<u64>(end - p) < flen) return ERR_TRUNCATED;
       i64 v_before = vi;
-      int32_t rc = extract_feature_body(p, p + flen, kind, dst, &vi, &bi);
+      int32_t rc = extract_feature_body<OFFS>(p, p + flen, kind, dst, &vi, &bi);
       if (rc != ERR_OK) return rc;
-      dst.sub_count[li++] = vi - v_before;
+      dst.sub_count[li++] = OFFS ? v_before : vi - v_before;
       p += flen;
     } else {
       p = skip_field(p, end, wt);
diff --git a/csrc/hip/kernels.hip b/csrc/hip/kernels.hip
--- a/csrc/hip/kernels.hip
+++ b/csrc/hip/kernels.hip
@@ -76,8 +76,9 @@
                                     FieldStat* __restrict__ stats,
                                     int32_t* __restrict__ err,
                                     unsigned long long* crc_err,
-                                    i64 rec_base) {
+                                    i64 rec_base, const i64* gate) {
   __shared__ uint32_t tab[8][256];
+  if (gate && *gate) return;
   if (crc_err) stage_crc_tables(tab);
   SchemaView schema = schema_view(schema_blob);
   for (i64 r = blockIdx.x * (i64)blockDim.x + threadIdx.x; r < R;
@@ -119,17 +120,63 @@
   i64* i64_vals;
   float* f32_vals;
   u8* bytes_data;
-  i64* elem_len;
-  i64* sub_count;
+  i64* elem_off;
+  i64* sub_off;
+  u8* presence;
   const i64* val_base;
   const i64* byte_base;
   const i64* list_base;
+  i64 cap_vals;
+  i64 cap_bytes;
+  i64 cap_elem_off;
+  i64 cap_sub_off;
 };
+
+__device__ inline void store_end_sentinels(const DevFieldDst* __restrict__ metas,
+                                           int F, i64 r_end) {
+  if (blockIdx.x != 0) return;
+  for (int f = threadIdx.x; f < F; f += blockDim.x) {
+    const DevFieldDst& m = metas[f];
+    if (m.kind == KIND_BYTES && m.elem_off && m.val_base && m.byte_base)
+      m.elem_off[m.val_base[r_end]] = m.byte_base[r_end];
+    if (m.is_seq && m.sub_off && m.list_base && m.val_base)
+      m.sub_off[m.list_base[r_end]] = m.val_base[r_end];
+  }
+}
+
+__global__ void extract_gate_kernel(const DevFieldDst* __restrict__ metas, int F,
+                                    i64 r_end, const i64* broken,
+                                    const unsigned long long* crc,
+                                    const int32_t* scan_err, i64* refused) {
+  int bad = 0;
+  if (threadIdx.x == 0) {
+    if (broken && *broken) bad = 1;
+    if (crc && *crc != ~0ULL) bad = 1;
+    if (scan_err && scan_err[0] != 0) bad = 1;
+  }
+  for (int f = threadIdx.x; f < F; f += blockDim.x) {
+    const DevFieldDst& m = metas[f];
+    i64 nv = m.val_base ? m.val_base[r_end] : 0;
+    i64 nb = m.byte_base ? m.byte_base[r_end] : 0;
+    i64 nl = m.list_base ? m.list_base[r_end] : 0;
+    if (m.kind == KIND_BYTES) {
+      if (nb > m.cap_bytes || nv + 1 > m.cap_elem_off) bad = 1;
+    } else if (nv > m.cap_vals) {
+      bad = 1;
+    }
+    if (m.is_seq && nl + 1 > m.cap_sub_off) bad = 1;
+  }
+  int any = __syncthreads_or(bad);
+  if (threadIdx.x == 0) *refused = any ? 1 : 0;
+}
 
 __global__ void extract_fields_kernel(const u8* __restrict__ data, i64 R, int F,
                                       const FieldStat* __restrict__ stats,
                                       const DevFieldDst* __restrict__ metas,
-                                      int32_t* __restrict__ err, i64 r0) {
+                                      int32_t* __restrict__ err, i64 r0,
+                                      const i64* refused) {
+  if (refused && *refused) return;
+  store_end_sentinels(metas, F, r0 + R);
   i64 total = R * F;
   for (i64 idx = blockIdx.x * (i64)blockDim.x + threadIdx.x; idx < total;
        idx += (i64)gridDim.x * blockDim.x) {
@@ -138,11 +185,12 @@
     i64 r = r0 + q;
     const DevFieldDst& m = metas[f];
     const FieldStat& st = stats[r * F + f];
-    DecodeDst dst{m.i64_vals, m.f32_vals, m.bytes_data, m.elem_len, m.sub_count};
-    int32_t rc = extract_field(data, st.pos, st.len, m.kind, m.is_seq, dst,
-                               m.val_base ? m.val_base[r] : 0,
-                               m.byte_base ? m.byte_base[r] : 0,
-                               m.list_base ? m.list_base[r] : 0);
+    DecodeDst dst{m.i64_vals, m.f32_vals, m.bytes_data, m.elem_off, m.sub_off};
+    if (m.presence) m.presence[r] = st.pos >= 0 ? 1 : 0;
+    int32_t rc = extract_field<true>(data, st.pos, st.len, m.kind, m.is_seq,
+                                     dst, m.val_base ? m.val_base[r] : 0,
+                                     m.byte_base ? m.byte_base[r] : 0,
+                                     m.list_base ? m.list_base[r] : 0);
     if (rc != ERR_OK) set_err(err, rc, r);
   }
 }
@@ -338,7 +386,7 @@
       p = read_varint(p, end, &len);
       if (!p || (u64)(end - p) < len) return ERR_TRUNCATED;
       copy_wave(dst.bytes_data + *bi, p, (i64)len);
-      if (lane == 0) dst.elem_len[*vi] = (i64)len;
+      if (lane == 0) dst.elem_len[*vi] = *bi;
       *bi += (i64)len;
       *vi += 1;
       p += len;
@@ -429,7 +477,7 @@
       i64 v_before = vi;
       int32_t rc = extract_feature_body_wave(p, p + flen, kind, dst, &vi, &bi);
       if (rc != ERR_OK) return rc;
-      if (lane == 0) dst.sub_count[li] = vi - v_before;
+      if (lane == 0) dst.sub_count[li] = v_before;
       ++li;
       p += flen;
     } else {
@@ -448,8 +496,9 @@
                                          int F, FieldStat* __restrict__ stats,
                                          int32_t* __restrict__ err,
                                          unsigned long long* crc_err,
-                                         i64 rec_base) {
+                                         i64 rec_base, const i64* gate) {
   __shared__ uint32_t tab[8][256];
+  if (gate && *gate) return;
   stage_crc_tables(tab);
   SchemaView schema = schema_view(schema_blob);
   i64 wave = (blockIdx.x * (i64)blockDim.x + threadIdx.x) / 64;
@@ -483,7 +532,10 @@
                                            int F,
                                            const FieldStat* __restrict__ stats,
                                            const DevFieldDst* __restrict__ metas,
-                                           int32_t* __restrict__ err, i64 r0) {
+                                           int32_t* __restrict__ err, i64 r0,
+                                           const i64* refused) {
+  if (refused && *refused) return;
+  store_end_sentinels(metas, F, r0 + R);
   i64 total = R * F;
   i64 wave = (blockIdx.x * (i64)blockDim.x + threadIdx.x) / 64;
   i64 nwaves = ((i64)gridDim.x * blockDim.x) / 64;
@@ -493,12 +545,14 @@
     i64 r = r0 + q;
     const DevFieldDst& m = metas[f];
     const FieldStat& st = stats[r * F + f];
-    DecodeDst dst{m.i64_vals, m.f32_vals, m.bytes_data, m.elem_len, m.sub_count};
+    DecodeDst dst{m.i64_vals, m.f32_vals, m.bytes_data, m.elem_off, m.sub_off};
+    bool lane0 = (threadIdx.x & 63) == 0;
+    if (lane0 && m.presence) m.presence[r] = st.pos >= 0 ? 1 : 0;
     int32_t rc = extract_field_wave(data, st.pos, st.len, m.kind, m.is_seq, dst,
                                     m.val_base ? m.val_base[r] : 0,
                                     m.byte_base ? m.byte_base[r] : 0,
                                     m.list_base ? m.list_base[r] : 0);
-    if (rc != ERR_OK && (threadIdx.x & 63) == 0) set_err(err, rc, r);
+    if (rc != ERR_OK && lane0) set_err(err, rc, r);
   }
 }
 
@@ -810,6 +864,30 @@
     if (p != want) *broken = 1;
     off[k] = p + 12;
     if (k == C - 1) *carry_out = p + 16 + len[k];
+  }
+}
+
+__global__ void stream_snapshot_kernel(const i64* count, const i64* status,
+                                       int nst, const i64* carry, const i64* v,
+                                       const i64* b, const i64* l, i64 stride,
+                                       int F, i64 r, i64* out) {
+  int n = 2 + nst + (v ? 3 * F : 0);
+  for (int i = threadIdx.x; i < n; i += blockDim.x) {
+    i64 x;
+    if (i == 0) {
+      x = count ? *count : 0;
+    } else if (i <= nst) {
+      x = status[i - 1];
+    } else if (i == nst + 1) {
+      x = carry ? *carry : 0;
+    } else {
+      int k = i - (nst + 2);
+      int plane = k / F;
+      int f = k - plane * F;
+      const i64* src = plane == 0 ? v : plane == 1 ? b : l;
+      x = src[(i64)f * stride + r];
+    }
+    out[i] = x;
   }
 }
 
@@ -1077,7 +1155,8 @@
 void gpu_scan_records(uintptr_t data, uintptr_t off, uintptr_t len, i64 R,
                       int32_t fmt, uintptr_t schema_blob, int F, uintptr_t stats,
                       uintptr_t err, uintptr_t crc_err, uintptr_t stream,
-                      i64 avg_bytes, i64 rec_base, i64 max_blocks) {
+                      i64 avg_bytes, i64 rec_base, i64 max_blocks,
+                      uintptr_t gate) {
   if (R <= 0) return;
   if (avg_bytes > kWaveRecordBytes) {
     hipLaunchKernelGGL(scan_records_wave_kernel,
@@ -1085,13 +1164,15 @@
                        (hipStream_t)stream, (const u8*)data, (const i64*)off,
                        (const i64*)len, R, fmt, (const u8*)schema_blob, F,
                        (FieldStat*)stats, (int32_t*)err,
-                       (unsigned long long*)crc_err, rec_base);
+                       (unsigned long long*)crc_err, rec_base,
+                       (const i64*)gate);
   } else {
     hipLaunchKernelGGL(scan_records_kernel, dim3(grid_for(R, max_blocks)),
                        dim3(kBlock), 0, (hipStream_t)stream, (const u8*)data,
                        (const i64*)off, (const i64*)len, R, fmt,
                        (const u8*)schema_blob, F, (FieldStat*)stats,
-                       (int32_t*)err, (unsigned long long*)crc_err, rec_base);
+                       (int32_t*)err, (unsigned long long*)crc_err, rec_base,
+                       (const i64*)gate);
   }
   HIP_CHECK(hipGetLastError());
 }
@@ -1099,40 +1180,100 @@
 void gpu_extract_fields(uintptr_t data, i64 R, int F, uintptr_t stats,
                         py::list metas, uintptr_t meta_dev, uintptr_t err,
                         uintptr_t stream, i64 avg_bytes, i64 r0,
-                        i64 max_blocks) {
+                        i64 max_blocks, bool upload, uintptr_t gate_broken,
+                        uintptr_t gate_crc, uintptr_t gate_err,
+                        uintptr_t gate_out) {
   if (R <= 0 || F <= 0) return;
-  std::vector<DevFieldDst> host_metas(F);
-  for (int f = 0; f < F; ++f) {
-    py::dict d = metas[f].cast<py::dict>();
-    DevFieldDst& m = host_metas[f];
-    m.kind = d["kind"].cast<int32_t>();
-    m.is_seq = d["is_seq"].cast<int32_t>();
-    m.i64_vals = (i64*)d["i64_vals"].cast<uintptr_t>();
-    m.f32_vals = (float*)d["f32_vals"].cast<uintptr_t>();
-    m.bytes_data = (u8*)d["bytes_data"].cast<uintptr_t>();
-    m.elem_len = (i64*)d["elem_len"].cast<uintptr_t>();
-    m.sub_count = (i64*)d["sub_count"].cast<uintptr_t>();
-    m.val_base = (const i64*)d["val_base"].cast<uintptr_t>();
-    m.byte_base = (const i64*)d["byte_base"].cast<uintptr_t>();
-    m.list_base = (const i64*)d["list_base"].cast<uintptr_t>();
-  }
-  HIP_CHECK(hipMemcpyAsync((void*)meta_dev, host_metas.data(),
-                           sizeof(DevFieldDst) * F, hipMemcpyHostToDevice,
-                           (hipStream_t)stream));
+  if (upload) {
+    std::vector<DevFieldDst> host_metas(F);
+    for (int f = 0; f < F; ++f) {
+      py::dict d = metas[f].cast<py::dict>();
+      auto ptr = [&](const char* k) {
+        return d.contains(k) ? d[k].cast<uintptr_t>() : (uintptr_t)0;
+      };
+      auto cap = [&](const char* k) {
+        return d.contains(k) ? d[k].cast<i64>() : (i64)0;
+      };
+      DevFieldDst& m = host_metas[f];
+      m.kind = d["kind"].cast<int32_t>();
+      m.is_seq = d["is_seq"].cast<int32_t>();
+      m.i64_vals = (i64*)ptr("i64_vals");
+      m.f32_vals = (float*)ptr("f32_vals");
+      m.bytes_data = (u8*)ptr("bytes_data");
+      m.elem_off = (i64*)ptr("elem_off");
+      m.sub_off = (i64*)ptr("sub_off");
+      m.presence = (u8*)ptr("presence");
+      m.val_base = (const i64*)ptr("val_base");
+      m.byte_base = (const i64*)ptr("byte_base");
+      m.list_base = (const i64*)ptr("list_base");
+      m.cap_vals = cap("cap_vals");
+      m.cap_bytes = cap("cap_bytes");
+      m.cap_elem_off = cap("cap_elem_off");
+      m.cap_sub_off = cap("cap_sub_off");
+    }
+    HIP_CHECK(hipMemcpyAsync((void*)meta_dev, host_metas.data(),
+                             sizeof(DevFieldDst) * F, hipMemcpyHostToDevice,
+                             (hipStream_t)stream));
+  }
+  if (gate_out) {
+    hipLaunchKernelGGL(extract_gate_kernel, dim3(1), dim3(kBlock), 0,
+                       (hipStream_t)stream, (const DevFieldDst*)meta_dev, F,
+                       r0 + R, (const i64*)gate_broken,
+                       (const unsigned long long*)gate_crc,
+                       (const int32_t*)gate_err, (i64*)gate_out);
+  }
   if (avg_bytes > kWaveRecordBytes) {
     hipLaunchKernelGGL(extract_fields_wave_kernel,
                        dim3(grid_for(R * F * 64, max_blocks)), dim3(kBlock), 0,
                        (hipStream_t)stream, (const u8*)data, R, F,
                        (const FieldStat*)stats, (const DevFieldDst*)meta_dev,
-                       (int32_t*)err, r0);
+                       (int32_t*)err, r0, (const i64*)gate_out);
   } else {
     hipLaunchKernelGGL(extract_fields_kernel,
                        dim3(grid_for(R * F, max_blocks)), dim3(kBlock), 0,
                        (hipStream_t)stream, (const u8*)data, R, F,
                        (const FieldStat*)stats, (const DevFieldDst*)meta_dev,
-                       (int32_t*)err, r0);
+                       (int32_t*)err, r0, (const i64*)gate_out);
   }
   HIP_CHECK(hipGetLastError());
+}
+
+struct SnapshotEvent {
+  int device = -1;
+  hipEvent_t ev = nullptr;
+};
+thread_local SnapshotEvent snapshot_event;
+
+void gpu_stream_snapshot(uintptr_t count, uintptr_t status, int nst,
+                         uintptr_t carry, uintptr_t v, uintptr_t b, uintptr_t l,
+                         i64 stride, int F, i64 r, uintptr_t out_host,
+                         uintptr_t stream) {
+  int dev = 0;
+  HIP_CHECK(hipGetDevice(&dev));
+  SnapshotEvent& se = snapshot_event;
+  if (se.device != dev) {
+    if (se.ev) (void)hipEventDestroy(se.ev);
+    se.ev = nullptr;
+    HIP_CHECK(hipEventCreateWithFlags(&se.ev, hipEventDisableTiming));
+    se.device = dev;
+  }
+  void* out_dev = nullptr;
+  HIP_CHECK(hipHostGetDevicePointer(&out_dev, (void*)out_host, 0));
+  hipLaunchKernelGGL(stream_snapshot_kernel, dim3(1), dim3(kBlock), 0,
+                     (hipStream_t)stream, (const i64*)count,
+                     (const i64*)status, nst, (const i64*)carry, (const i64*)v,
+                     (const i64*)b, (const i64*)l, stride, v ? F : 0, r,
+                     (i64*)out_dev);
+  HIP_CHECK(hipGetLastError());
+  HIP_CHECK(hipEventRecord(se.ev, (hipStream_t)stream));
+}
+
+void gpu_stream_snapshot_wait() {
+  SnapshotEvent& se = snapshot_event;
+  if (!se.ev)
+    throw std::runtime_error("gpu_stream_snapshot_wait: no snapshot taken");
+  py::gil_scoped_release rel;
+  HIP_CHECK(hipEventSynchronize(se.ev));
 }
 
 size_t gpu_devcols_bytes(int F) { return sizeof(FieldColumn) * (size_t)F; }
@@ -1555,12 +1696,19 @@
         py::arg("len"), py::arg("R"), py::arg("fmt"), py::arg("schema_blob"),
         py::arg("F"), py::arg("stats"), py::arg("err"), py::arg("crc_err"),
         py::arg("stream"), py::arg("avg_bytes") = 0, py::arg("rec_base") = 0,
-        py::arg("max_blocks") = 0);
+        py::arg("max_blocks") = 0, py::arg("gate") = 0);
   m.def("gpu_extract_fields", &gpu_extract_fields, py::arg("data"),
         py::arg("R"), py::arg("F"), py::arg("stats"), py::arg("metas"),
         py::arg("meta_dev"), py::arg("err"), py::arg("stream"),
         py::arg("avg_bytes") = 0, py::arg("r0") = 0,
-        py::arg("max_blocks") = 0);
+        py::arg("max_blocks") = 0, py::arg("upload") = true,
+        py::arg("gate_broken") = 0, py::arg("gate_crc") = 0,
+        py::arg("gate_err") = 0, py::arg("gate_out") = 0);
+  m.def("gpu_stream_snapshot", &gpu_stream_snapshot, py::arg("count"),
+        py::arg("status"), py::arg("nst"), py::arg("carry"), py::arg("v"),
+        py::arg("b"), py::arg("l"), py::arg("stride"), py::arg("F"),
+        py::arg("r"), py::arg("out_host"), py::arg("stream"));
+  m.def("gpu_stream_snapshot_wait", &gpu_stream_snapshot_wait);
   m.def("gpu_size_records", &gpu_size_records);
   m.def("gpu_emit_records", &gpu_emit_records, py::arg("cols_dev"),
         py::arg("schema_blob"), py::arg("fmt"), py::arg("r0"), py::arg("R"),
diff --git a/exp/trace_tail.py b/exp/trace_tail.py
--- /dev/null
+++ b/exp/trace_tail.py
@@ -0,0 +1,138 @@
+#!/usr/bin/env python3
+
+import argparse
+import csv
+import glob
+import os
+
+SLICE_COPY_MS = 0.1
+READ_GAP_MS = 2.0
+MIN_SLICE_COPIES = 4
+
+
+def _rows(out_dir, suffix):
+    rows = []
+    for path in sorted(glob.glob(os.path.join(out_dir, "**", "*" + suffix),
+                                 recursive=True)):
+        with open(path, newline="") as f:
+            rows += list(csv.DictReader(f))
+    return rows
+
+
+def load(out_dir):
+    kernels = [(int(r["Start_Timestamp"]) / 1e6, int(r["End_Timestamp"]) / 1e6,
+                r["Kernel_Name"]) for r in _rows(out_dir, "kernel_trace.csv")]
+    copies = [(int(r["Start_Timestamp"]) / 1e6, int(r["End_Timestamp"]) / 1e6,
+               r.get("Direction", "")) for r in
+              _rows(out_dir, "memory_copy_trace.csv")]
+    return sorted(kernels), sorted(copies)
+
+
+def find_reads(kernels, copies):
+    big = [c for c in copies if "HOST_TO_DEVICE" in c[2]
+           and c[1] - c[0] > SLICE_COPY_MS]
+    groups = []
+    for c in big:
+        if groups and c[0] - groups[-1][-1][1] < READ_GAP_MS:
+            groups[-1].append(c)
+        else:
+            groups.append([c])
+    writes = [k[0] for k in kernels if "size_records" in k[2]]
+    reads = []
+    for i, g in enumerate(groups):
+        t0 = g[0][0]
+        t1 = min([w for w in writes if w > t0] +
+                 [groups[i + 1][0][0] if i + 1 < len(groups) else float("inf")])
+        if len(g) >= MIN_SLICE_COPIES:
+            reads.append((g, [k for k in kernels if t0 <= k[0] < t1]))
+    return reads
+
+
+def landings(slice_copies, split=True):
+    if not split:
+        return sorted(c[1] for c in slice_copies)
+    lanes = [[], []]
+    for c in sorted(slice_copies):
+        idle = [ln for ln in lanes if not ln or ln[-1][1] <= c[0] + 0.005]
+        if idle:
+            lane = max(idle, key=lambda ln: ln[-1][1] if ln else float("-inf"))
+        else:
+            lane = min(lanes, key=lambda ln: ln[-1][1])
+        lane.append(c)
+    n = min(len(lanes[0]), len(lanes[1]))
+    out = [max(lanes[0][k][1], lanes[1][k][1]) for k in range(n)]
+    out += [c[1] for ln in lanes for c in ln[n:]]
+    return sorted(out)
+
+
+def busy(spans):
+    total, cur_s, cur_e = 0.0, None, None
+    for s, e in sorted(spans):
+        if cur_e is None or s > cur_e:
+            if cur_e is not None:
+                total += cur_e - cur_s
+            cur_s, cur_e = s, e
+        else:
+            cur_e = max(cur_e, e)
+    if cur_e is not None:
+        total += cur_e - cur_s
+    return total
+
+
+def report(idx, slice_copies, ks, detail, split):
+    t0 = slice_copies[0][0]
+    last_copy = max(c[1] for c in slice_copies)
+    last_kernel = max((k[1] for k in ks), default=last_copy)
+    after = [k for k in ks if k[1] > last_copy]
+    print(f"read {idx}: {len(slice_copies)} slice copies, last lands at "
+          f"{last_copy - t0:.3f} ms, last decode kernel ends at "
+          f"{last_kernel - t0:.3f} ms: tail {last_kernel - last_copy:.3f} ms; "
+          f"{len(after)} kernels end after the last copy, busy "
+          f"{busy([(max(k[0], last_copy), k[1]) for k in after]):.3f} ms")
+    if not detail:
+        return
+    print("  copies (start, end) ms from first issue:",
+          [(round(c[0] - t0, 3), round(c[1] - t0, 3)) for c in slice_copies])
+    print("  kernels (start, end, name) from first copy issue:")
+    for s, e, name in ks:
+        mark = " *" if e > last_copy else "  "
+        print(f"  {mark}{s - t0:9.3f} {e - t0:8.3f}  {name[:72]}")
+    print("  (* ends after the last copy)")
+    counts = [i for i, k in enumerate(ks) if "frame_scan_pass_kernel<false>" in k[2]]
+    land = landings(slice_copies, split)
+    print("  slice: landed, period to the next landing, chain wall, chain busy")
+    for n, i in enumerate(counts):
+        j = counts[n + 1] if n + 1 < len(counts) else len(ks)
+        chain = ks[i:j]
+        wall = max(k[1] for k in chain) - chain[0][0]
+        period = (f"{land[n + 1] - land[n]:.3f}" if n + 1 < len(land)
+                  else "  -  ")
+        landed = f"{land[n] - t0:.3f}" if n < len(land) else "  ?  "
+        print(f"  {n:5d}  {landed:>7}  {period:>7}  {wall:7.3f}  "
+              f"{busy([(k[0], k[1]) for k in chain]):7.3f}   "
+              f"(COUNT starts {chain[0][0] - t0:.3f})")
+
+
+def main():
+    ap = argparse.ArgumentParser(description=__doc__.split("\n\n")[0])
+    ap.add_argument("out_dir")
+    ap.add_argument("--read", type=int, default=-1,
+                    help="read to print in detail (default: the last)")
+    ap.add_argument("--whole-slices", action="store_true",
+                    help="the run had TFREC_READ_SPLIT=0: one copy per slice")
+    args = ap.parse_args()
+    kernels, copies = load(args.out_dir)
+    dirs = {}
+    for c in copies:
+        dirs[c[2]] = dirs.get(c[2], 0) + 1
+    print("copy directions:", dirs)
+    reads = find_reads(kernels, copies)
+    if not reads:
+        raise SystemExit("no slice copies found in the trace")
+    detail = args.read % len(reads)
+    for i, (g, ks) in enumerate(reads):
+        report(i, g, ks, i == detail, not args.whole_slices)
+
+
+if __name__ == "__main__":
+    main()
diff --git a/spark_tfrecord_amd/engine/gpu.py b/spark_tfrecord_amd/engine/gpu.py
--- a/spark_tfrecord_amd/engine/gpu.py
+++ b/spark_tfrecord_amd/engine/gpu.py
@@ -356,11 +356,12 @@
     _raise_scan_errors(int(crc_err.item()) if fuse_crc else -1,
                        int(err[0].item()), int(err[1].item()))
     vals = _FieldValues(fields, data.numel(), device)
-    meta_dev = torch.empty(F * _native.gpu_devmeta_bytes(), dtype=torch.uint8,
-                           device=device)
-    vals.extract(data, stats, (val_base, byte_base, list_base), 0, R, totals_h,
-                 data.numel(), meta_dev, err, avg_bytes)
-    cols = vals.columns(stats, val_base, list_base, R)
+    vals.reserve(totals_h, data.numel())
+    presence = torch.empty((F, R), dtype=torch.uint8, device=device)
+    vals.extract(data, stats, (val_base, byte_base, list_base), presence, 0, R,
+                 _MetaTable(F, device), err, avg_bytes)
+    vals.confirm(totals_h)
+    cols = vals.columns(presence, val_base, list_base, R)
     if int(err[0].item()) != 0:
         _raise_extract_error(int(err[0].item()), int(err[1].item()))
     return RecordBatch(schema, cols, R)
@@ -398,13 +399,28 @@
                        f"{where} (native error {rc})")
 
 
+class _MetaTable:
+
+    def __init__(self, F: int, device):
+        self.dev = torch.empty(F * _native.gpu_devmeta_bytes(),
+                               dtype=torch.uint8, device=device)
+        self.last = None
+
+    def changed(self, metas) -> bool:
+        key = [tuple(m.items()) for m in metas]
+        if key == self.last:
+            return False
+        self.last = key
+        return True
+
+
 class _FieldValues:
 
-    _BUFS = {"i64_vals": (torch.int64, 0, KIND_INT64),
-             "f32_vals": (torch.float32, 0, KIND_FLOAT),
-             "elem_len": (torch.int64, 0, KIND_BYTES),
-             "bytes_data": (torch.uint8, 1, None),
-             "sub_count": (torch.int64, 2, None)}
+    _BUFS = {"i64_vals": (torch.int64, 0, 0, lambda k, seq: k == KIND_INT64),
+             "f32_vals": (torch.float32, 0, 0, lambda k, seq: k == KIND_FLOAT),
+             "elem_off": (torch.int64, 0, 1, lambda k, seq: k == KIND_BYTES),
+             "bytes_data": (torch.uint8, 1, 0, lambda k, seq: k == KIND_BYTES),
+             "sub_off": (torch.int64, 2, 1, lambda k, seq: seq)}
 
     def __init__(self, fields, total_bytes: int, device):
         self.total_bytes = total_bytes
@@ -413,14 +429,14 @@
         self.seqs = [is_sequence_field(f.dataType) for f in fields]
         self.filled = [[0] * len(fields) for _ in range(3)]
         self.bufs = [{k: torch.empty(0, dtype=d, device=device)
-                      for k, (d, _, _) in self._BUFS.items()} for _ in fields]
-
-    def _reserve(self, totals, bytes_seen: int):
+                      for k, (d, _, _, _) in self._BUFS.items()} for _ in fields]
+
+    def reserve(self, totals, bytes_seen: int):
         for i, bufs in enumerate(self.bufs):
-            for name, (_, dim, kind) in self._BUFS.items():
-                if kind not in (None, self.kinds[i]):
+            for name, (_, dim, extra, fills) in self._BUFS.items():
+                if not fills(self.kinds[i], self.seqs[i]):
                     continue
-                need = int(totals[dim][i])
+                need = int(totals[dim][i]) + extra
                 old = bufs[name]
                 cap = stream_plan.grown_capacity(
                     old.numel(), need, bytes_seen, self.total_bytes,
@@ -428,52 +444,57 @@
                 if cap == old.numel():
                     continue
                 new = torch.empty(cap, dtype=old.dtype, device=self.device)
-                k = self.filled[dim][i]
+                k = min(self.filled[dim][i] + extra, old.numel())
                 if k:
                     new[:k].copy_(old[:k])
                 if old.numel():
                     last_read["regrows"] = last_read.get("regrows", 0) + 1
                 bufs[name] = new
 
-    def extract(self, data, stats, planes, r0: int, r1: int, totals,
-                bytes_seen: int, meta_dev, err, avg_bytes: int):
-        self._reserve(totals, bytes_seen)
+    def confirm(self, totals):
+        self.filled = [[int(totals[d][i]) for i in range(len(self.bufs))]
+                       for d in range(3)]
+
+    def extract(self, data, stats, planes, presence, r0: int, r1: int,
+                meta: _MetaTable, err, avg_bytes: int, gate=None):
         v, b, l = planes
         metas = []
         for i, bufs in enumerate(self.bufs):
+            vals = bufs["i64_vals" if self.kinds[i] == KIND_INT64 else "f32_vals"]
             metas.append({
                 "kind": self.kinds[i], "is_seq": 1 if self.seqs[i] else 0,
                 **{name: t.data_ptr() for name, t in bufs.items()},
+                "presence": presence[i].data_ptr(),
                 "val_base": v[i].data_ptr(),
                 "byte_base": b[i].data_ptr(),
                 "list_base": l[i].data_ptr() if self.seqs[i] else 0,
+                "cap_vals": vals.numel(),
+                "cap_bytes": bufs["bytes_data"].numel(),
+                "cap_elem_off": bufs["elem_off"].numel(),
+                "cap_sub_off": bufs["sub_off"].numel(),
             })
+        g_broken, g_crc, g_err, g_out = gate or (0, 0, 0, 0)
         _native.gpu_extract_fields(data.data_ptr(), r1 - r0, len(self.bufs),
                                    stats.data_ptr(), metas,
-                                   meta_dev.data_ptr(), err.data_ptr(),
-                                   _stream(), avg_bytes, r0=r0)
-        self.filled = [[int(totals[d][i]) for i in range(len(self.bufs))]
-                       for d in range(3)]
-
-    def columns(self, stats, val_base, list_base, R: int) -> List[WireColumn]:
+                                   meta.dev.data_ptr(), err.data_ptr(),
+                                   _stream(), avg_bytes, r0=r0,
+                                   upload=meta.changed(metas),
+                                   gate_broken=g_broken, gate_crc=g_crc,
+                                   gate_err=g_err, gate_out=g_out)
+
+    def columns(self, presence, val_base, list_base, R: int) -> List[WireColumn]:
         cols = []
         for i, bufs in enumerate(self.bufs):
             kind, seq = self.kinds[i], self.seqs[i]
             nv, nb, nl = (self.filled[d][i] for d in range(3))
-            presence = (stats[:, i, 0] >= 0).to(torch.uint8)
-            elem_off = None
-            if kind == KIND_BYTES:
-                elem_off = excl_sum(bufs["elem_len"][:nv])
-            sub_off = None
-            if seq:
-                sub_off = excl_sum(bufs["sub_count"][:nl])
             values = (bufs["i64_vals"][:nv] if kind == KIND_INT64 else
                       bufs["f32_vals"][:nv] if kind == KIND_FLOAT else
                       bufs["bytes_data"][:nb])
-            cols.append(WireColumn(kind, seq, presence, val_base[i][:R + 1],
-                                   values, elem_off,
-                                   list_base[i][:R + 1] if seq else None,
-                                   sub_off))
+            cols.append(WireColumn(
+                kind, seq, presence[i][:R], val_base[i][:R + 1], values,
+                bufs["elem_off"][:nv + 1] if kind == KIND_BYTES else None,
+                list_base[i][:R + 1] if seq else None,
+                bufs["sub_off"][:nl + 1] if seq else None))
         return cols
 
 
@@ -608,7 +629,7 @@
 
 last_read = {}
 
-_ST_BROKEN, _ST_CRC, _ST_ERR, _ST_XERR, _ST_CARRY = 0, 1, 2, 3, 4
+_ST_BROKEN, _ST_CRC, _ST_ERR, _ST_XERR, _ST_NOEXT, _ST_CARRY = 0, 1, 2, 3, 4, 5
 
 
 class _StreamStatus:
@@ -626,17 +647,20 @@
     def carry_addr(self, k: int) -> int:
         return self.addr(_ST_CARRY + k)
 
-    def head(self) -> torch.Tensor:
-        return self.words[:_ST_CARRY]
-
-    @staticmethod
-    def chain_end(h, nchain: int) -> Optional[int]:
-        return None if int(h[_ST_BROKEN]) != 0 else int(h[_ST_CARRY + nchain])
-
-    @staticmethod
-    def scan_error(h):
-        pair = h[_ST_ERR:_ST_ERR + 1].view(torch.int32)
-        return int(h[_ST_CRC]), int(pair[0]), int(pair[1])
+
+class _Snapshot:
+
+    def __init__(self, h: np.ndarray, F: int):
+        self.count = int(h[0])
+        st = h[1:1 + _ST_CARRY]
+        self.broken = int(st[_ST_BROKEN]) != 0
+        pair = st[_ST_ERR:_ST_ERR + 1].view(np.int32)
+        self.scan_error = (int(st[_ST_CRC]), int(pair[0]), int(pair[1]))
+        xpair = st[_ST_XERR:_ST_XERR + 1].view(np.int32)
+        self.xerr = (int(xpair[0]), int(xpair[1]))
+        self.refused = int(st[_ST_NOEXT]) != 0
+        self.chain_end = int(h[1 + _ST_CARRY])
+        self.totals = h[2 + _ST_CARRY:].reshape(3, F) if F else None
 
 
 class _StreamRows:
@@ -648,18 +672,21 @@
         self.cap = 0
         self.pos = self.lens = self.off = self.stats = None
         self.planes = None
+        self.presence = None
 
     def _alloc(self, cap: int):
         i64 = dict(dtype=torch.int64, device=self.device)
-        planes = None
+        planes = presence = None
         if self.F:
             planes = [torch.empty((self.F, cap + 1), **i64) for _ in range(3)]
             for t in planes:
                 t[:, 0] = 0
+            presence = torch.empty((self.F, cap), dtype=torch.uint8,
+                                   device=self.device)
         return (torch.empty(cap, **i64), torch.empty(cap, **i64),
                 torch.empty(cap, **i64),
                 torch.empty((cap, self.F, 6), **i64) if self.F else None,
-                planes)
+                planes, presence)
 
     def cand_ptrs(self, c: int):
         return (self.pos.data_ptr() + c * 8, self.lens.data_ptr() + c * 8,
@@ -677,15 +704,12 @@
                                b.data_ptr(), l.data_ptr(), _stream(), r0=r0,
                                r1=r1, stride=self.cap + 1)
 
-    def totals(self, r: int) -> list:
-        return [t[:, r] for t in self.planes]
-
     def reserve(self, need: int, n_cand: int, n_scanned: int, bytes_seen: int):
         cap = stream_plan.grown_capacity(self.cap, need, bytes_seen,
                                          self.total_bytes, _STREAM_HEADROOM)
         if cap == self.cap:
             return
-        pos, lens, off, stats, planes = self._alloc(cap)
+        pos, lens, off, stats, planes, presence = self._alloc(cap)
         if n_cand:
             pos[:n_cand].copy_(self.pos[:n_cand])
             lens[:n_cand].copy_(self.lens[:n_cand])
@@ -694,8 +718,9 @@
             stats[:n_scanned].copy_(self.stats[:n_scanned])
             for new, old in zip(planes, self.planes):
                 new[:, :n_scanned + 1].copy_(old[:, :n_scanned + 1])
+            presence[:, :n_scanned].copy_(self.presence[:, :n_scanned])
         self.pos, self.lens, self.off, self.stats = pos, lens, off, stats
-        self.planes = planes
+        self.planes, self.presence = planes, presence
         if self.cap:
             last_read["regrows"] = last_read.get("regrows", 0) + 1
         self.cap = cap
@@ -719,98 +744,141 @@
         if self.do_scan:
             self.blob = _schema_blob_device(schema, device)
             self.vals = _FieldValues(fields, self.n, device)
-            self.meta_dev = torch.empty(F * _native.gpu_devmeta_bytes(),
-                                        dtype=torch.uint8, device=device)
+            self.meta = _MetaTable(F, device)
         self.C = 0
         self.nchain = 0
         self.r_done = 0
         self.x_done = 0
+        self.x_pending = None
+        self.sized = False
+        self.bytes_done = 0
         self.clean = True
         self.avg_bytes = None
 
-    def discover(self, p: stream_plan.SlicePlan, counts: torch.Tensor):
-        block_off = excl_sum(counts)
-        c_s = int(block_off[-1].item())
-        if not c_s:
-            return
-        self.rows.reserve(self.C + c_s, self.C, self.r_done, p.scan_hi)
-        pos, lens, off = self.rows.cand_ptrs(self.C)
-        _native.gpu_frame_scan_emit(self.data.data_ptr(), self.n, p.scan_lo,
-                                    p.scan_hi, 0, block_off.data_ptr(), pos,
-                                    lens, _stream())
-        _native.gpu_frame_chain(pos, lens, c_s,
-                                self.status.carry_addr(self.nchain),
-                                self.status.carry_addr(self.nchain + 1), off,
-                                self.status.addr(_ST_BROKEN), _stream())
-        self.nchain += 1
-        self.C += c_s
-
-    def arrived(self, p: stream_plan.SlicePlan, last: bool):
-        if not self.do_scan or self.C == self.r_done:
-            return self.r_done, p.b1
-        if last:
-            return self.C, self.n
-        end = self.status.chain_end(self.status.words.cpu(), self.nchain)
-        if end is None:
-            return None
-        avail = stream_plan.arrived_records(self.C, end, p.b1)
-        return avail, end if avail == self.C else p.b1
-
-    def scan(self, avail: int, end: int, last: bool):
-        r0 = self.r_done
-        if avail <= r0:
-            return
-        if self.avg_bytes is None:
-            self.avg_bytes = max(0, end // avail - 16)
-        off, lens, stats = self.rows.row_ptrs(r0)
-        _native.gpu_scan_records(
-            self.data.data_ptr(), off, lens, avail - r0, FMT[self.record_type],
-            self.blob.data_ptr(), self.F, stats, self.status.err.data_ptr(),
-            self.status.addr(_ST_CRC) if self.verify_crc else 0, _stream(),
-            self.avg_bytes, rec_base=r0)
-        self.rows.scan_stats(r0, avail)
-        self.r_done = avail
-        if not _STREAM_EXTRACT or last or not self.clean:
-            return
-        F = self.F
-        h = torch.cat(self.rows.totals(avail) + [self.status.head()]).cpu()
-        crc_bad, rc, _ = self.status.scan_error(h[3 * F:])
+    def _snapshot(self, count_ptr: int, r: int) -> _Snapshot:
+        F = self.F if self.rows.planes is not None else 0
+        n = 2 + _ST_CARRY + 3 * F
+        buf = pinned_buffer("snapshot", n * 8)
+        v, b, l = ([t.data_ptr() for t in self.rows.planes] if F
+                   else (0, 0, 0))
+        _native.gpu_stream_snapshot(
+            count_ptr, self.status.addr(0), _ST_CARRY,
+            self.status.carry_addr(self.nchain), v, b, l, self.rows.cap + 1,
+            F, r, buf.data_ptr(), _stream())
+        _native.gpu_stream_snapshot_wait()
+        last_read["host_waits"] = last_read.get("host_waits", 0) + 1
+        return _Snapshot(buf.numpy()[:n * 8].view(np.int64).copy(), F)
+
+    def _settle(self, snap: _Snapshot):
+        crc_bad, rc, _ = snap.scan_error
         if crc_bad != -1 or rc != 0:
             self.clean = False
+        if self.x_pending is None:
             return
-        self._extract(avail, h[:3 * F].view(3, F), end)
-
-    def _extract(self, r1: int, totals_h, bytes_seen: int):
+        assert self.x_pending == self.r_done
+        if not snap.refused:
+            self.x_done = self.x_pending
+            self.vals.confirm(snap.totals)
+        elif self.clean:
+            self.vals.reserve(snap.totals, self.bytes_done)
+        self.x_pending = None
+
+    def _extract(self, r1: int, gated: bool):
+        st = self.status
+        gate = (st.addr(_ST_BROKEN), st.addr(_ST_CRC), st.addr(_ST_ERR),
+                st.addr(_ST_NOEXT)) if gated else None
         self.vals.extract(self.data, self.rows.stats, self.rows.planes,
-                          self.x_done, r1, totals_h, bytes_seen, self.meta_dev,
-                          self.status.xerr, self.avg_bytes)
-        self.x_done = r1
+                          self.rows.presence, self.x_done, r1, self.meta,
+                          st.xerr, self.avg_bytes, gate)
+
+    def step(self, p: stream_plan.SlicePlan, counts: Optional[torch.Tensor],
+             last: bool) -> bool:
+        count_ptr = 0
+        if counts is not None:
+            block_off = excl_sum(counts)
+            count_ptr = block_off.data_ptr() + counts.numel() * 8
+        snap = self._snapshot(count_ptr, self.r_done)
+        if snap.broken:
+            return False
+        if self.do_scan:
+            self._settle(snap)
+        c_s = snap.count
+        if c_s:
+            self.rows.reserve(self.C + c_s, self.C, self.r_done, p.scan_hi)
+            pos, lens, off = self.rows.cand_ptrs(self.C)
+            _native.gpu_frame_scan_emit(self.data.data_ptr(), self.n,
+                                        p.scan_lo, p.scan_hi, 0,
+                                        block_off.data_ptr(), pos, lens,
+                                        _stream())
+            _native.gpu_frame_chain(pos, lens, c_s,
+                                    self.status.carry_addr(self.nchain),
+                                    self.status.carry_addr(self.nchain + 1),
+                                    off, self.status.addr(_ST_BROKEN),
+                                    _stream())
+            self.nchain += 1
+            self.C += c_s
+        if not self.do_scan:
+            return True
+        avail = stream_plan.launchable_records(self.C, last)
+        r0 = self.r_done
+        if avail > r0:
+            if self.avg_bytes is None:
+                self.avg_bytes = max(0, p.scan_hi // avail - 16)
+            off, lens, stats = self.rows.row_ptrs(r0)
+            _native.gpu_scan_records(
+                self.data.data_ptr(), off, lens, avail - r0,
+                FMT[self.record_type], self.blob.data_ptr(), self.F, stats,
+                self.status.err.data_ptr(),
+                self.status.addr(_ST_CRC) if self.verify_crc else 0, _stream(),
+                self.avg_bytes, rec_base=r0,
+                gate=self.status.addr(_ST_BROKEN))
+            self.rows.scan_stats(r0, avail)
+            self.r_done = avail
+        self.bytes_done = p.scan_hi
+        if not _STREAM_EXTRACT or not self.clean or avail <= self.x_done:
+            return True
+        if not self.sized:
+            if last:
+                return True
+            snap = self._snapshot(0, avail)
+            if snap.broken:
+                return False
+            self._settle(snap)
+            if not self.clean:
+                return True
+            self.vals.reserve(snap.totals, p.scan_hi)
+            self.sized = True
+        self._extract(avail, gated=True)
+        self.x_pending = avail
+        return True
 
     def finish(self) -> Optional[RecordBatch]:
-        R, F, n = self.C, self.F, self.n
+        R, n = self.C, self.n
         if R == 0:
             return None
+        snap = self._snapshot(0, R)
+        if snap.broken or snap.chain_end != n:
+            return None
         if not self.do_scan:
-            if self.status.chain_end(self.status.words.cpu(), self.nchain) != n:
-                return None
             return decode_device(self.data, self.rows.off[:R],
                                  self.rows.lens[:R], self.schema,
                                  self.record_type, self.verify_crc)
-        packed = torch.cat(self.rows.totals(R) + [self.status.words]).cpu()
-        st_h = packed[3 * F:]
-        if self.status.chain_end(st_h, self.nchain) != n:
-            return None
-        crc_bad, rc, rec1 = self.status.scan_error(st_h)
+        crc_bad, rc, rec1 = snap.scan_error
         _raise_scan_errors(crc_bad if self.verify_crc else -1, rc, rec1)
         if not self.clean:
             raise RuntimeError("streamed decode: scan error lost")
+        self._settle(snap)
+        xerr = snap.xerr
         if self.x_done < R:
-            self._extract(R, packed[:3 * F].view(3, F), n)
+            self.vals.reserve(snap.totals, n)
+            self._extract(R, gated=False)
+            self.x_done = R
+            self.vals.confirm(snap.totals)
+            xerr = self._snapshot(0, R).xerr
         val_base, _, list_base = self.rows.planes
-        cols = self.vals.columns(self.rows.stats[:R], val_base, list_base, R)
-        err_h = self.status.xerr.cpu()
-        if int(err_h[0]) != 0:
-            _raise_extract_error(int(err_h[0]), int(err_h[1]))
+        cols = self.vals.columns(self.rows.presence, val_base, list_base, R)
+        if xerr[0] != 0:
+            _raise_extract_error(*xerr)
         return RecordBatch(self.schema, cols, R)
 
 
@@ -889,7 +957,7 @@
     block_counts = torch.empty(max(sum(_scan_blocks(p) for p in plan), 1),
                                dtype=torch.int64, device=data.device)
     events = _issue_h2d_slices(data, ptr, plan)
-    last_read.update(path="streamed", slices=S, regrows=0)
+    last_read.update(path="streamed", slices=S, regrows=0, host_waits=0)
     unstreamed = (data, plan, block_counts, events)
     decode = (schema, record_type, verify_crc)
     if not _STREAM_DECODE:
@@ -899,13 +967,10 @@
     base = 0
     for s, p in enumerate(plan):
         nb = _count_slice(data, p, events[s], block_counts, base)
-        if nb:
-            rd.discover(p, block_counts[base:base + nb])
-            base += nb
-        got = rd.arrived(p, last=s == S - 1)
-        if got is None:
+        counts = block_counts[base:base + nb] if nb else None
+        base += nb
+        if not rd.step(p, counts, last=s == S - 1):
             return _read_unstreamed(*unstreamed, s + 1, *decode)
-        rd.scan(*got, last=s == S - 1)
     batch = rd.finish()
     if batch is None:
         return _read_unstreamed(*unstreamed, S, *decode)
diff --git a/spark_tfrecord_amd/engine/stream_plan.py b/spark_tfrecord_amd/engine/stream_plan.py
--- a/spark_tfrecord_amd/engine/stream_plan.py
+++ b/spark_tfrecord_amd/engine/stream_plan.py
@@ -36,6 +36,12 @@
     return n_cand if last_end <= arrived else n_cand - 1
 
 
+def launchable_records(n_cand: int, last: bool) -> int:
+    if n_cand <= 0:
+        return 0
+    return n_cand if last else n_cand - 1
+
+
 def row_capacity(need: int, bytes_seen: int, total_bytes: int,
                  headroom: float, min_unit: int = MIN_FRAME) -> int:
     need = max(int(need), 0)
```
